# medivhna/TF_Face_Toolbox

Hardware: AMD Instinct MI355X
Metric: images/sec (whole node), SphereFaceNet-20 112x112 bs512 (higher is better)
Workload: dtype f32; 1 GPU; SphereFaceNet-20 + A-softmax training step, 112x112x3, global batch 512, 10575 classes, Momentum, fp32; global_batch=512, per_gpu_batch=512, parallelism=dp1

## Files before the change

### include/fte.h

```cpp
#ifndef FTE_H_
#define FTE_H_

#include <stddef.h>
#include <stdint.h>

#ifdef __cplusplus
extern "C" {
#endif

#define FTE_OK 0
#define FTE_EINVAL (-1)
#define FTE_EWORKSPACE (-2)

const char* fte_version(void);

#define FTE_MFMA_F32 0
#define FTE_MFMA_BF16 1
int fte_set_mfma_dtype(int dtype);
int fte_get_mfma_dtype(void);

#define FTE_CONV_DIRECT 0
#define FTE_CONV_WINOGRAD 1
#define FTE_CONV_AUTO 2
int fte_set_conv_algo(int algo);
int fte_get_conv_algo(void);
int fte_conv3x3_algo(int n, int h, int wd, int cin, int cout, int stride, int op);
size_t fte_wino_pack_bytes(int n, int h, int wd, int c);

int fte_prof_enable(int on);
int fte_prof_count(void);
int fte_prof_get(int i, int* sig, double* flops, float* ms);
int fte_prof_get_shape(int i, int* mnk, double* bytes);
int fte_prof_get_name(int i, char* buf, int buflen);


int fte_conv3x3_fwd(const float* x, const float* w, const float* bias, const float* alpha,
                    const float* res, float* z, float* y,
                    int n, int h, int wd, int cin, int cout, int stride,
                    void* ws, size_t ws_bytes, void* stream);
size_t fte_conv3x3_fwd_ws_bytes(int n, int h, int wd, int cin, int cout, int stride);
int fte_conv3x3_fwd_keep(const float* x, const float* w, const float* bias, const float* alpha,
                         const float* res, float* z, float* y,
                         int n, int h, int wd, int cin, int cout, int stride, float* vpack,
                         void* ws, size_t ws_bytes, void* stream);

int fte_conv3x3_dgrad(const float* dz, const float* w, const float* addin,
                      const float* zprev, const float* alpha_prev,
                      float* raw, float* dzprev, float* dalpha_prev, float* dbias_prev,
                      int n, int h, int wd, int cin, int cout, int stride,
                      void* ws, size_t ws_bytes, void* stream);
size_t fte_conv3x3_dgrad_ws_bytes(int n, int h, int wd, int cin, int cout, int stride);

int fte_conv3x3_wgrad(const float* x, const float* dz, float* dw,
                      int n, int h, int wd, int cin, int cout, int stride,
                      void* ws, size_t ws_bytes, void* stream);
size_t fte_conv3x3_wgrad_ws_bytes(int n, int h, int wd, int cin, int cout, int stride);
int fte_conv3x3_wgrad_kept(const float* x, const float* dz, float* dw,
                           int n, int h, int wd, int cin, int cout, int stride, const float* vpack,
                           void* ws, size_t ws_bytes, void* stream);


int fte_conv2d_fwd(const float* x, const float* w, const float* bias, const float* alpha, const float* res,
                   float* z, float* y, int n, int h, int wd, int cin, int cout, int ksize, int stride,
                   void* ws, size_t ws_bytes, void* stream);
size_t fte_conv2d_fwd_ws_bytes(int n, int h, int wd, int cin, int cout, int ksize, int stride);
int fte_conv2d_dgrad(const float* dz, const float* w, const float* addin, const float* zprev,
                     const float* alpha_prev, float* raw, float* dzprev, float* dalpha_prev, float* dbias_prev,
                     int n, int h, int wd, int cin, int cout, int ksize, int stride,
                     void* ws, size_t ws_bytes, void* stream);
size_t fte_conv2d_dgrad_ws_bytes(int n, int h, int wd, int cin, int cout, int ksize, int stride);
int fte_conv2d_wgrad(const float* x, const float* dz, float* dw, int n, int h, int wd, int cin, int cout,
                     int ksize, int stride, void* ws, size_t ws_bytes, void* stream);
size_t fte_conv2d_wgrad_ws_bytes(int n, int h, int wd, int cin, int cout, int ksize, int stride);

int fte_im2col_first(const float* x, float* cols, int n, int h, int wd, int cin, int ksize, int stride,
                     int kpad, void* stream);
int fte_im2col_first_s16(const float* x, uint16_t* cols16, int n, int h, int wd, int cin, int ksize, int stride, int kpad, void* stream);

int fte_preprocess_u8(const uint8_t* slots, float* out, int n, long slot_stride, int channels, int in_h, int in_w, int crop_h, int crop_w,
                      void* stream);
int fte_preprocess_u8_aug(const uint8_t* slots, float* out, int n, long slot_stride, int channels, int in_h, int in_w, int crop_h,
                          int crop_w, void* stream);
size_t fte_preprocess_u8_geo_ws_bytes(int n, int channels, int crop_h, int crop_w);
int fte_preprocess_u8_geo(const uint8_t* slots, float* out, int n, long slot_stride, int channels, int in_h, int in_w, int crop_h,
                          int crop_w, const float* affine_table, void* ws, size_t ws_bytes, void* stream);

size_t fte_bn_ws_bytes(int c);
int fte_bn_train_fwd(const float* z, const float* gamma, const float* beta, const float* res, float* y,
                     float* mean, float* rstd, float* scale, float* shift, float* moving_mean, float* moving_var,
                     long rows, int c, float eps, float decay, int relu, void* ws, size_t ws_bytes, void* stream);
int fte_bn_infer_fwd(const float* z, const float* gamma, const float* beta, const float* moving_mean,
                     const float* moving_var, const float* res, float* y, float* scale, float* shift,
                     long rows, int c, float eps, int relu, void* stream);
int fte_bn_train_bwd(const float* dy, const float* ymask, const float* z, const float* gamma, const float* mean,
                     const float* rstd, float* dz, float* dgamma, float* dbeta, long rows, int c,
                     void* ws, size_t ws_bytes, void* stream);
int fte_bn_train_bwd_zmask(const float* dy, const float* z, const float* gamma, const float* mean, const float* rstd,
                           const float* scale, const float* shift, float* dz, float* dgamma, float* dbeta, long rows, int c,
                           void* ws, size_t ws_bytes, void* stream);
int fte_bn_train_bwd_res(const float* dy, const float* y, const float* z, const float* gamma, const float* mean, const float* rstd,
                         float* g_out, float* dz, float* dgamma, float* dbeta, long rows, int c,
                         void* ws, size_t ws_bytes, void* stream);
int fte_bn_train_stats(const float* z, const float* gamma, const float* beta, float* mean, float* rstd, float* scale, float* shift,
                       float* moving_mean, float* moving_var, long rows, int c, float eps, float decay,
                       void* ws, size_t ws_bytes, void* stream);
int fte_bn_infer_coef(const float* gamma, const float* beta, const float* moving_mean, const float* moving_var,
                      float* scale, float* shift, int c, float eps, void* stream);
size_t fte_bn_prelu_ws_bytes(int c);
int fte_bn_prelu_apply(const float* z, const float* scale, const float* shift, const float* alpha, float* y, long rows, int c,
                       void* stream);
int fte_bn_prelu_infer_fwd(const float* z, const float* gamma, const float* beta, const float* moving_mean, const float* moving_var,
                           const float* alpha, float* y, float* scale, float* shift, long rows, int c, float eps, void* stream);
int fte_bn_prelu_train_bwd(const float* dy, const float* z, const float* gamma, const float* mean, const float* rstd,
                           const float* scale, const float* shift, const float* alpha, float* dz, float* dgamma, float* dbeta,
                           float* dalpha, long rows, int c, void* ws, size_t ws_bytes, void* stream);
int fte_relu_bwd(const float* dy, const float* y, float* g, long n, void* stream);

int fte_maxpool3x3s2_fwd(const float* x, float* y, uint8_t* idx, int n, int h, int wd, int c, void* stream);
int fte_maxpool3x3s2_bwd(const float* dy, const uint8_t* idx, float* dx, int n, int h, int wd, int c, void* stream);
int fte_gap_fwd(const float* x, float* y, int n, int hw, int c, void* stream);
int fte_gap_bwd(const float* dy, float* dx, int n, int hw, int c, void* stream);
int fte_dropout_fwd(const float* x, float* mask, float* y, long n, float keep_prob, uint64_t seed, void* stream);
int fte_dropout_bwd(const float* dy, const float* mask, float* dx, long n, float keep_prob, void* stream);

int fte_gconv3x3_fwd(const float* x, const float* w, float* y, int n, int h, int wd, int c, int groups,
                     int stride, void* stream);
int fte_gconv3x3_pack_bf16(const float* w, uint16_t* wpk_fwd, uint16_t* wpk_dgrad, int c, int groups, void* stream);
int fte_gconv3x3_bf16(const float* x, const uint16_t* wpk, float* y, int n, int h, int wd, int c, int stride, int dgrad, void* stream);
size_t fte_gconv3x3_wgrad_bf16_ws_bytes(int n, int h, int wd, int c, int groups, int stride);
int fte_gconv3x3_wgrad_bf16(const float* x, const float* dz, float* dw, int n, int h, int wd, int c, int groups, int stride,
                            void* ws, size_t ws_bytes, void* stream);
int fte_gconv3x3_dgrad(const float* dz, const float* w, float* dx, int n, int h, int wd, int c, int groups,
                       int stride, void* stream);
int fte_gconv3x3_wgrad(const float* x, const float* dz, float* dw, int n, int h, int wd, int c, int groups,
                       int stride, void* ws, size_t ws_bytes, void* stream);
size_t fte_gconv3x3_wgrad_ws_bytes(int n, int h, int wd, int c, int groups, int stride);

int fte_bcast_add(float* dx, const float* v, int n, int hw, int c, float scale, void* stream);
int fte_dense_small(const float* a, const float* w, const float* bias, const float* mask, float* out, int m, int n, int k,
                    int trans_w, int act, void* stream);
int fte_act_fwd(const float* x, float* y, long n, int kind, void* stream);
int fte_act_bwd(const float* dy, const float* y, float* dx, long n, int kind, void* stream);
int fte_channel_scale_fwd(const float* x, const float* gate, float* y, int n, int hw, int c, void* stream);
int fte_channel_scale_bwd(const float* dy, const float* x, const float* gate, float* dx, float* dgate,
                          int n, int hw, int c, int pre_sigmoid, void* stream);

int fte_to_bf16(const float* x, uint16_t* y16, long n, void* stream);
int fte_pack_weights_bf16(const float* w, uint16_t* w16, uint16_t* w16t, int ksize, int cin, int cout, void* stream);
int fte_pack_weights_bf16_table(const float* params, uint16_t* dst, const int32_t* table, int nconv, long total, int transposed, void* stream);
int fte_conv2d_fwd16(const uint16_t* x16, const uint16_t* w16t, const float* bias, const float* alpha, const float* res,
                     float* z, float* y, uint16_t* y16, int n, int h, int wd, int cin, int cout, int ksize, int stride,
                     void* ws, size_t ws_bytes, void* stream);
int fte_conv2d_dgrad16(const uint16_t* dz16, const uint16_t* w16, const float* addin, const float* zprev,
                       const float* alpha_prev, float* raw, float* dzprev, uint16_t* dzprev16, float* dalpha_prev,
                       float* dbias_prev, int n, int h, int wd, int cin, int cout, int ksize, int stride,
                       void* ws, size_t ws_bytes, void* stream);
int fte_conv2d_wgrad16(const uint16_t* x16, const uint16_t* dz16, float* dw, int n, int h, int wd, int cin, int cout,
                       int ksize, int stride, void* ws, size_t ws_bytes, void* stream);

int fte_conv2d_fwd_s16(const uint16_t* x16, const uint16_t* w16t, const float* bias, const float* alpha, const uint16_t* res16,
                       uint16_t* z16, uint16_t* y16, float* z32, float* y32, int n, int h, int wd, int cin, int cout,
                       int ksize, int stride, void* ws, size_t ws_bytes, void* stream);
int fte_conv2d_dgrad_s16(const uint16_t* dz16, const uint16_t* w16, const uint16_t* addin16, const uint16_t* zprev16,
                         const float* alpha_prev, uint16_t* raw16, uint16_t* dzprev16, float* dalpha_prev, float* dbias_prev,
                         int n, int h, int wd, int cin, int cout, int ksize, int stride, void* ws, size_t ws_bytes, void* stream);
int fte_conv3x3_first_fwd_s16(const float* x, const float* w, const float* bias, const float* alpha, uint16_t* z16, uint16_t* y16,
                              int n, int h, int wd, int cin, int cout, int stride, void* stream);
int fte_conv3x3_first_wgrad_s16(const float* x, const uint16_t* dz16, float* dw, int n, int h, int wd, int cin, int cout, int stride,
                                void* ws, size_t ws_bytes, void* stream);

#define FTE_S16_Z 1
#define FTE_S16_A 2
int fte_bn_train_fwd_s16(const void* z, const float* gamma, const float* beta, const void* res, void* y,
                         float* mean, float* rstd, float* scale, float* shift, float* moving_mean, float* moving_var,
                         long rows, int c, float eps, float decay, int relu, int flags, void* ws, size_t ws_bytes, void* stream);
int fte_bn_infer_fwd_s16(const void* z, const float* gamma, const float* beta, const float* moving_mean, const float* moving_var,
                         const void* res, void* y, float* scale, float* shift, long rows, int c, float eps, int relu, int flags, void* stream);
int fte_bn_train_bwd_s16(const void* dy, const void* y, const void* z, const float* gamma, const float* mean, const float* rstd,
                         const float* scale, const float* shift, void* g_out, void* dz, float* dgamma, float* dbeta,
                         long rows, int c, int flags, void* ws, size_t ws_bytes, void* stream);
int fte_relu_bwd_s16(const uint16_t* dy16, const uint16_t* y16, uint16_t* g16, long n, void* stream);
int fte_maxpool3x3s2_fwd_s16(const uint16_t* x16, uint16_t* y16, uint8_t* idx, int n, int h, int wd, int c, void* stream);
int fte_maxpool3x3s2_bwd_s16(const uint16_t* dy16, const uint8_t* idx, uint16_t* dx16, int n, int h, int wd, int c, void* stream);
int fte_gap_fwd_s16(const uint16_t* x16, float* y, int n, int hw, int c, void* stream);
int fte_gap_bwd_s16(const float* dy, uint16_t* dx16, int n, int hw, int c, void* stream);
int fte_gconv3x3_bf16_s16(const uint16_t* x16, const uint16_t* wpk, uint16_t* y16, int n, int h, int wd, int c, int stride, int dgrad, void* stream);
int fte_gconv3x3_wgrad_bf16_s16(const uint16_t* x16, const uint16_t* dz16, float* dw, int n, int h, int wd, int c, int groups, int stride,
                                void* ws, size_t ws_bytes, void* stream);
size_t fte_conv2d_bn_fwd_ws_bytes(int n, int h, int wd, int cin, int cout, int ksize, int stride);
int fte_conv2d_bn_fwd_folds(int n, int h, int wd, int cin, int cout, int ksize, int stride, int s16);
int fte_conv2d_bn_fwd(const void* x, const void* w, void* z, const float* gamma, const float* beta, float* mean, float* rstd,
                      float* scale, float* shift, float* moving_mean, float* moving_var, float eps, float decay,
                      const float* in_scale, const float* in_shift, void* y_side,
                      int n, int h, int wd, int cin, int cout, int ksize, int stride, int s16, void* ws, size_t ws_bytes, void* stream);
size_t fte_conv2d_dgrad_bn_ws_bytes(int n, int h, int wd, int cin, int cout, int ksize, int stride);
int fte_conv2d_dgrad_bn(const void* dz, const void* w, const void* addin, const void* zbn, const void* ybn,
                        const float* gamma, const float* mean, const float* rstd, const float* bn_scale, const float* bn_shift,
// ... 175 lines not shown
```

### tf_face_toolbox_amd/_lib.py

```python
import ctypes
import os
from ctypes import c_char_p, c_float, c_int, c_long, c_size_t, c_uint64, c_void_p

_HERE = os.path.dirname(os.path.abspath(__file__))
LIB_PATH = os.environ.get('FTE_LIB') or os.path.join(_HERE, 'libfte.so')


class FteError(RuntimeError):
    pass


_P = c_void_p
_SIGS = {
    'fte_version': (c_char_p, []),
    'fte_prof_enable': (c_int, [c_int]),
    'fte_prof_count': (c_int, []),
    'fte_prof_get': (c_int, [c_int, _P, _P, _P]),
    'fte_prof_get_shape': (c_int, [c_int, _P, _P]),
    'fte_prof_get_name': (c_int, [c_int, _P, c_int]),
    'fte_conv3x3_fwd': (c_int, [_P] * 7 + [c_int] * 6 + [_P, c_size_t, _P]),
    'fte_conv3x3_fwd_ws_bytes': (c_size_t, [c_int] * 6),
    'fte_conv3x3_dgrad': (c_int, [_P] * 9 + [c_int] * 6 + [_P, c_size_t, _P]),
    'fte_conv3x3_dgrad_ws_bytes': (c_size_t, [c_int] * 6),
    'fte_conv3x3_wgrad': (c_int, [_P] * 3 + [c_int] * 6 + [_P, c_size_t, _P]),
    'fte_conv3x3_wgrad_ws_bytes': (c_size_t, [c_int] * 6),
    'fte_conv2d_fwd': (c_int, [_P] * 7 + [c_int] * 7 + [_P, c_size_t, _P]),
    'fte_conv2d_fwd_ws_bytes': (c_size_t, [c_int] * 7),
    'fte_conv2d_dgrad': (c_int, [_P] * 9 + [c_int] * 7 + [_P, c_size_t, _P]),
    'fte_conv2d_dgrad_ws_bytes': (c_size_t, [c_int] * 7),
    'fte_conv2d_wgrad': (c_int, [_P] * 3 + [c_int] * 7 + [_P, c_size_t, _P]),
    'fte_conv2d_wgrad_ws_bytes': (c_size_t, [c_int] * 7),
    'fte_im2col_first': (c_int, [_P] * 2 + [c_int] * 7 + [_P]),
    'fte_im2col_first_s16': (c_int, [_P] * 2 + [c_int] * 7 + [_P]),
    'fte_preprocess_u8': (c_int, [_P] * 2 + [c_int, c_long] + [c_int] * 5 + [_P]),
    'fte_preprocess_u8_aug': (c_int, [_P] * 2 + [c_int, c_long] + [c_int] * 5 + [_P]),
    'fte_preprocess_u8_geo_ws_bytes': (c_size_t, [c_int] * 4),
    'fte_preprocess_u8_geo': (c_int, [_P] * 2 + [c_int, c_long] + [c_int] * 5 + [_P, _P, c_size_t, _P]),
    'fte_bn_ws_bytes': (c_size_t, [c_int]),
    'fte_bn_train_fwd': (c_int, [_P] * 11 + [c_long, c_int, c_float, c_float, c_int, _P, c_size_t, _P]),
    'fte_bn_infer_fwd': (c_int, [_P] * 9 + [c_long, c_int, c_float, c_int, _P]),
    'fte_bn_train_bwd': (c_int, [_P] * 9 + [c_long, c_int, _P, c_size_t, _P]),
    'fte_bn_train_bwd_zmask': (c_int, [_P] * 10 + [c_long, c_int, _P, c_size_t, _P]),
    'fte_bn_train_bwd_res': (c_int, [_P] * 10 + [c_long, c_int, _P, c_size_t, _P]),
    'fte_bn_train_stats': (c_int, [_P] * 9 + [c_long, c_int, c_float, c_float, _P, c_size_t, _P]),
    'fte_bn_infer_coef': (c_int, [_P] * 6 + [c_int, c_float, _P]),
    'fte_bn_prelu_ws_bytes': (c_size_t, [c_int]),
    'fte_bn_prelu_apply': (c_int, [_P] * 5 + [c_long, c_int, _P]),
    'fte_bn_prelu_infer_fwd': (c_int, [_P] * 9 + [c_long, c_int, c_float, _P]),
    'fte_bn_prelu_train_bwd': (c_int, [_P] * 12 + [c_long, c_int, _P, c_size_t, _P]),
    'fte_relu_bwd': (c_int, [_P] * 3 + [c_long, _P]),
    'fte_maxpool3x3s2_fwd': (c_int, [_P] * 3 + [c_int] * 4 + [_P]),
    'fte_maxpool3x3s2_bwd': (c_int, [_P] * 3 + [c_int] * 4 + [_P]),
    'fte_gap_fwd': (c_int, [_P] * 2 + [c_int] * 3 + [_P]),
    'fte_gap_bwd': (c_int, [_P] * 2 + [c_int] * 3 + [_P]),
    'fte_dropout_fwd': (c_int, [_P] * 3 + [c_long, c_float, c_uint64, _P]),
    'fte_dropout_bwd': (c_int, [_P] * 3 + [c_long, c_float, _P]),
    'fte_gconv3x3_fwd': (c_int, [_P] * 3 + [c_int] * 6 + [_P]),
    'fte_gconv3x3_pack_bf16': (c_int, [_P] * 3 + [c_int, c_int, _P]),
    'fte_gconv3x3_bf16': (c_int, [_P] * 3 + [c_int] * 6 + [_P]),
    'fte_gconv3x3_wgrad_bf16_ws_bytes': (c_size_t, [c_int] * 6),
    'fte_gconv3x3_wgrad_bf16': (c_int, [_P] * 3 + [c_int] * 6 + [_P, c_size_t, _P]),
    'fte_gconv3x3_dgrad': (c_int, [_P] * 3 + [c_int] * 6 + [_P]),
    'fte_gconv3x3_wgrad': (c_int, [_P] * 3 + [c_int] * 6 + [_P, c_size_t, _P]),
    'fte_gconv3x3_wgrad_ws_bytes': (c_size_t, [c_int] * 6),
    'fte_bcast_add': (c_int, [_P] * 2 + [c_int] * 3 + [c_float, _P]),
    'fte_act_fwd': (c_int, [_P] * 2 + [c_long, c_int, _P]),
    'fte_act_bwd': (c_int, [_P] * 3 + [c_long, c_int, _P]),
    'fte_channel_scale_fwd': (c_int, [_P] * 3 + [c_int] * 3 + [_P]),
    'fte_channel_scale_bwd': (c_int, [_P] * 5 + [c_int] * 4 + [_P]),
    'fte_to_bf16': (c_int, [_P, _P, c_long, _P]),
    'fte_pack_weights_bf16': (c_int, [_P, _P, _P, c_int, c_int, c_int, _P]),
    'fte_pack_weights_bf16_table': (c_int, [_P, _P, _P, c_int, c_long, c_int, _P]),
    'fte_conv2d_fwd16': (c_int, [_P] * 8 + [c_int] * 7 + [_P, c_size_t, _P]),
    'fte_conv2d_dgrad16': (c_int, [_P] * 10 + [c_int] * 7 + [_P, c_size_t, _P]),
    'fte_conv2d_wgrad16': (c_int, [_P] * 3 + [c_int] * 7 + [_P, c_size_t, _P]),
    'fte_conv2d_fwd_s16': (c_int, [_P] * 9 + [c_int] * 7 + [_P, c_size_t, _P]),
    'fte_conv2d_dgrad_s16': (c_int, [_P] * 9 + [c_int] * 7 + [_P, c_size_t, _P]),
    'fte_conv3x3_first_fwd_s16': (c_int, [_P] * 6 + [c_int] * 6 + [_P]),
    'fte_conv3x3_first_wgrad_s16': (c_int, [_P] * 3 + [c_int] * 6 + [_P, c_size_t, _P]),
    'fte_bn_train_fwd_s16': (c_int, [_P] * 11 + [c_long, c_int, c_float, c_float, c_int, c_int, _P, c_size_t, _P]),
    'fte_bn_infer_fwd_s16': (c_int, [_P] * 9 + [c_long, c_int, c_float, c_int, c_int, _P]),
    'fte_bn_train_bwd_s16': (c_int, [_P] * 12 + [c_long, c_int, c_int, _P, c_size_t, _P]),
    'fte_relu_bwd_s16': (c_int, [_P] * 3 + [c_long, _P]),
    'fte_maxpool3x3s2_fwd_s16': (c_int, [_P] * 3 + [c_int] * 4 + [_P]),
    'fte_maxpool3x3s2_bwd_s16': (c_int, [_P] * 3 + [c_int] * 4 + [_P]),
    'fte_gap_fwd_s16': (c_int, [_P] * 2 + [c_int] * 3 + [_P]),
    'fte_gap_bwd_s16': (c_int, [_P] * 2 + [c_int] * 3 + [_P]),
    'fte_gconv3x3_bf16_s16': (c_int, [_P] * 3 + [c_int] * 6 + [_P]),
    'fte_gconv3x3_wgrad_bf16_s16': (c_int, [_P] * 3 + [c_int] * 6 + [_P, c_size_t, _P]),
    'fte_channel_scale_fwd_s16': (c_int, [_P] * 3 + [c_int] * 3 + [_P]),
    'fte_channel_scale_bwd_s16': (c_int, [_P] * 4 + [c_int] * 4 + [_P]),
    'fte_channel_scale_bwd_apply_s16': (c_int, [_P] * 4 + [c_int] * 3 + [c_float, _P]),
    'fte_dense_small': (c_int, [_P] * 5 + [c_int] * 5 + [_P]),
    'fte_se_squeeze': (c_int, [_P] * 7 + [c_int] * 4 + [_P]),
    'fte_se_apply_fwd': (c_int, [_P] * 6 + [c_int] * 4 + [_P]),
    'fte_se_bwd_gate': (c_int, [_P] * 12 + [c_int] * 4 + [_P]),
    'fte_se_bn_bwd_coef': (c_int, [_P] * 11 + [c_int] * 3 + [_P]),
    'fte_se_bn_bwd_apply': (c_int, [_P] * 6 + [c_int] * 4 + [_P]),
    'fte_dwconv3x3_fwd_s16': (c_int, [_P] * 3 + [c_int] * 5 + [_P]),
    'fte_dwconv3x3_dgrad_s16': (c_int, [_P] * 3 + [c_int] * 5 + [_P]),
    'fte_dwconv3x3_wgrad_s16': (c_int, [_P] * 3 + [c_int] * 5 + [_P, c_size_t, _P]),
    'fte_channel_gather_s16': (c_int, [_P] * 4 + [c_long] + [c_int] * 3 + [_P]),
    'fte_channel_gather_affine_s16': (c_int, [_P] * 4 + [c_int, _P, _P, c_int, c_long, c_int, c_int, _P, _P, c_int, _P, _P, c_int, _P]),
    'fte_bn_train_stats_s16': (c_int, [_P] * 9 + [c_long, c_int, c_float, c_float, c_int, _P, c_size_t, _P]),
    'fte_conv2d_bn_fwd_ws_bytes': (c_size_t, [c_int] * 7),
    'fte_conv2d_bn_fwd': (c_int, [_P] * 11 + [c_float, c_float] + [_P] * 3 + [c_int] * 8 + [_P, c_size_t, _P]),
    'fte_conv2d_bn_fwd_folds': (c_int, [c_int] * 8),
    'fte_conv2d_dgrad_bn_ws_bytes': (c_size_t, [c_int] * 7),
    'fte_conv2d_dgrad_bn': (c_int, [_P] * 14 + [c_int] * 8 + [_P, c_size_t, _P]),
    'fte_bn_apply': (c_int, [_P] * 5 + [c_long, c_int, c_int, c_int, _P]),
    'fte_bn_bwd_apply': (c_int, [_P] * 4 + [c_long, c_int, c_int, _P]),
    'fte_gconv3x3_bn_ws_bytes': (c_size_t, [c_int] * 5),
    'fte_gconv3x3_bn_fwd_bf16_s16': (c_int, [_P] * 11 + [c_float, c_float] + [_P] * 3 + [c_int] * 5 + [_P, c_size_t, _P]),
    'fte_gconv3x3_dgrad_bn_bf16_s16': (c_int, [_P] * 12 + [c_int] * 5 + [_P, c_size_t, _P]),
    'fte_set_mfma_dtype': (c_int, [c_int]),
    'fte_get_mfma_dtype': (c_int, []),
    'fte_set_conv_algo': (c_int, [c_int]),
    'fte_conv3x3_algo': (c_int, [c_int] * 7),
    'fte_wino_pack_bytes': (c_size_t, [c_int] * 4),
    'fte_conv3x3_fwd_keep': (c_int, [_P] * 7 + [c_int] * 6 + [_P, _P, c_size_t, _P]),
    'fte_conv3x3_wgrad_kept': (c_int, [_P] * 3 + [c_int] * 6 + [_P, _P, c_size_t, _P]),
    'fte_get_conv_algo': (c_int, []),
    'fte_l2_normalize_rows': (c_int, [_P] * 3 + [c_int] * 2 + [_P]),
    'fte_pair_scores': (c_int, [_P] * 4 + [c_int] * 3 + [_P]),
    'fte_topk_search_ws_bytes': (c_size_t, [c_int] * 4),
    'fte_topk_search': (c_int, [_P] * 2 + [c_int] * 7 + [_P] * 3 + [c_size_t, _P]),
    'fte_topk_merge': (c_int, [_P] * 2 + [c_int] * 3 + [_P] * 3),
    'fte_score_histograms': (c_int, [_P, _P, c_int, _P, _P] + [c_int] * 4 + [_P] * 3),
    'fte_template_pool': (c_int, [_P, _P, c_int, c_int, _P, c_int, _P, c_int, _P, c_int, _P, _P]),
    'fte_set_pair_scores': (c_int, [_P, c_int, c_int, _P, c_int, _P, c_int, _P, c_int, _P, _P, c_int, _P, c_int, _P, _P]),
    'fte_megaface_pair_scores': (c_int, [_P, c_int, _P, c_int, c_int, _P, _P, c_int, _P, _P]),
    'fte_megaface_scan_ws_bytes': (c_size_t, [c_int] * 2),
    'fte_megaface_scan': (c_int, [_P, c_int, _P, c_int, c_int, _P, _P, c_int, c_int, _P, _P, _P, c_size_t, _P]),
    'fte_pfc_sample_ws_bytes': (c_size_t, [c_int]),
    'fte_pfc_sample': (c_int, [_P] + [c_int] * 5 + [_P] * 4 + [c_size_t, _P]),
    'fte_pfc_gather_cols': (c_int, [_P] * 3 + [c_int] * 5 + [_P]),
    'fte_pfc_scatter_cols': (c_int, [_P] * 3 + [c_int] * 5 + [_P]),
    'fte_pfc_momentum_update_cols': (c_int, [_P] * 4 + [c_int] * 5 + [c_float] * 4 + [_P]),
    'fte_pfc_adam_update_cols': (c_int, [_P] * 5 + [c_int] * 5 + [c_float] * 6 + [c_int, _P]),
    'fte_knn_links_threshold': (c_int, [_P] * 2 + [c_int] * 2 + [c_float, c_int, _P, _P]),
    'fte_knn_links_rank_order': (c_int, [_P] * 2 + [c_int] * 2 + [c_float] * 2 + [_P, _P]),
    'fte_components': (c_int, [_P] * 2 + [c_int] * 2 + [_P] * 3),
    'fte_dwconv3x3_fwd': (c_int, [_P] * 3 + [c_int] * 5 + [_P]),
    'fte_dwconv3x3_dgrad': (c_int, [_P] * 3 + [c_int] * 5 + [_P]),
    'fte_dwconv3x3_wgrad': (c_int, [_P] * 3 + [c_int] * 5 + [_P, c_size_t, _P]),
    'fte_dwconv3x3_wgrad_ws_bytes': (c_size_t, [c_int] * 5),
    'fte_channel_gather': (c_int, [_P] * 4 + [c_long] + [c_int] * 3 + [_P]),
    'fte_channel_gather_affine': (c_int, [_P] * 4 + [c_int, _P, _P, c_int, c_long, c_int, c_int, _P, _P, c_int, _P, _P, c_int, _P]),
    'fte_conv3x3_first_fwd': (c_int, [_P] * 6 + [c_int] * 6 + [_P]),
    'fte_conv3x3_first_wgrad': (c_int, [_P] * 3 + [c_int] * 6 + [_P, c_size_t, _P]),
    'fte_conv3x3_first_wgrad_ws_bytes': (c_size_t, [c_int] * 6),
    'fte_gemm_nn': (c_int, [_P] * 4 + [c_int] * 3 + [_P, c_size_t, _P]),
    'fte_gemm_nn_act': (c_int, [_P] * 4 + [c_int] * 4 + [_P, c_size_t, _P]),
    'fte_gemm_nt': (c_int, [_P] * 4 + [c_int] + [_P] * 3 + [c_int] * 3 + [_P, c_size_t, _P]),
    'fte_gemm_tn': (c_int, [_P] * 3 + [c_int] * 3 + [_P, c_size_t, _P]),
    'fte_gemm_ws_bytes': (c_size_t, [c_int] * 3),
    'fte_softmax_ce_fwd_bwd': (c_int, [_P] * 4 + [c_int] * 3 + [c_float, _P]),
    'fte_focal_loss_fwd_bwd': (c_int, [_P] * 4 + [c_int] * 3 + [c_float] * 3 + [_P]),
    'fte_asoftmax_fwd_bwd': (c_int, [_P] * 4 + [c_float] + [_P] * 4 + [c_int] * 3 + [c_float, _P]),
    'fte_asoftmax_colcoef': (c_int, [_P] * 4 + [c_int] * 3 + [_P]),
    'fte_margin_softmax_fwd_bwd': (c_int, [_P] * 4 + [c_float] * 3 + [_P] * 4 + [c_int] * 3 + [c_float, _P]),
    'fte_margin_softmax_rows_fwd_bwd': (c_int, [_P] * 4 + [c_float] + [_P] * 6 + [c_int] * 3 + [c_float, _P]),
    'fte_subcenter_margin_softmax_fwd_bwd': (c_int, [_P] * 4 + [c_int] + [c_float] * 3 + [_P] * 4 + [c_int] * 3 + [c_float, _P]),
    'fte_subcenter_colcoef': (c_int, [_P] * 4 + [c_int] * 4 + [_P]),
    'fte_subcenter_assign': (c_int, [_P] * 3 + [c_int] + [_P] * 2 + [c_int] * 3 + [_P]),
    'fte_adaface_margins': (c_int, [_P, c_int] + [c_float] * 3 + [c_int] + [_P] * 4),
    'fte_row_norms': (c_int, [_P] * 2 + [c_int] * 3 + [_P]),
    'fte_col_norms': (c_int, [_P] * 2 + [c_int] * 3 + [_P]),
    'fte_add_scaled_rows_cols': (c_int, [_P] * 4 + [c_int] * 3 + [_P]),
    'fte_flip_width': (c_int, [_P] * 2 + [c_int] * 4 + [_P]),
    'fte_axpby': (c_int, [c_float, _P, c_float, _P, _P, c_long, _P]),
    'fte_center_loss_fwd_bwd_update': (c_int, [_P] * 5 + [c_int] * 3 + [c_float] * 2 + [_P, c_size_t, _P]),
    'fte_center_scatter_update': (c_int, [_P] * 3 + [c_int] * 3 + [c_float, _P]),
    'fte_batch_hard_triplet_fwd_bwd': (c_int, [_P] * 2 + [c_float, c_int, c_float] + [_P] * 2 + [c_int] * 2 + [_P, c_size_t, _P]),
    'fte_reduce_rows': (c_int, [_P] * 3 + [c_int, c_long, c_long, c_int, c_float, _P]),
    'fte_sumsq': (c_int, [_P, c_long, c_float, _P, _P, c_size_t, _P]),
    'fte_sum': (c_int, [_P, c_long, c_float, _P, _P, c_size_t, _P]),
    'fte_momentum_update': (c_int, [_P] * 3 + [c_long] + [c_float] * 4 + [_P]),
    'fte_adam_update': (c_int, [_P] * 4 + [c_long] + [c_float] * 6 + [c_int, _P]),
}

_lib = None


def exported_names():
    return sorted(_SIGS)


_CODES = {-1: 'FTE_EINVAL -- a null pointer, a shape the kernel family does not tile (channel multiples, stride, '
              'ksize) or a tensor of 2 GiB or more (buffer-load range)',
          -2: 'FTE_EWORKSPACE -- workspace missing or smaller than the matching *_ws_bytes() query'}

MFMA_DTYPES = {'f32': 0, 'fp32': 0, 'float32': 0, 'bf16': 1, 'bfloat16': 1, 'bf16s': 1}
_storage16 = False


def load():
    global _lib
    if _lib is not None:
        return _lib
    if not os.path.exists(LIB_PATH):
        raise FteError('libfte.so not found at %s -- build it with `python -c "import __graft_entry__ as g; g.build()"` '
                       '(or tf_face_toolbox_amd/csrc/build.sh). There is no CPU fallback.' % LIB_PATH)
    lib = ctypes.CDLL(LIB_PATH)
    for name, (res, args) in _SIGS.items():
        fn = getattr(lib, name)
        fn.restype = res
        fn.argtypes = args
    _lib = lib
    env = os.environ.get('FTE_MFMA_DTYPE')
    if env:
        if env not in MFMA_DTYPES:
            raise FteError('FTE_MFMA_DTYPE=%r: expected f32, bf16 or bf16s' % env)
        lib.fte_set_mfma_dtype(MFMA_DTYPES[env])
        global _storage16
        _storage16 = env == 'bf16s'
    return lib


def _ptr(t):
    if t is None:
        return None
    if isinstance(t, int):
        return t
    return t.data_ptr()


_FN = {}
_Tensor = None


def call(name, *args):
    global _Tensor
    fn = _FN.get(name)
    if fn is None:
        fn = _FN[name] = getattr(load(), name)
        if _Tensor is None:
            import torch
            _Tensor = torch.Tensor
    T = _Tensor
    r = fn(*[a.data_ptr() if type(a) is T else (a.data_ptr() if hasattr(a, 'data_ptr') else a) for a in args])
    if r != 0:
        what = _CODES.get(r, 'hipError_t %d (see hip_runtime_api.h)' % r if r > 0 else 'unknown')
        raise FteError('%s failed with code %d: %s' % (name, r, what))


def query(name, *args):
    return getattr(load(), name)(*args)


def version():
    return load().fte_version().decode()


def source_stamp():
    v = version()
    return v.split('src:', 1)[1] if 'src:' in v else ''


def set_mfma_dtype(name):
    if name not in MFMA_DTYPES:
        raise ValueError('unknown MFMA dtype %r (f32 | bf16 | bf16s)' % (name,))
    global _storage16
    call('fte_set_mfma_dtype', MFMA_DTYPES[name])
    _storage16 = name == 'bf16s'


def get_mfma_dtype():
    return 'bf16' if query('fte_get_mfma_dtype') == 1 else 'f32'


def bf16_storage():
    return _storage16 and query('fte_get_mfma_dtype') == 1
# ... 32 lines not shown
```

### tf_face_toolbox_amd/csrc/api.hip

```cpp
#include <hip/hip_runtime.h>
#include <stdio.h>
#include <stdlib.h>
#include <string.h>

#include <initializer_list>

#include "../../include/fte.h"
#include "igemm.h"
#include "wgrad16.h"
#include "pw16.h"
#include "kernels.h"
#include "layers.h"
#include "wino.h"
#include "search.h"
#include "partial_fc.h"
#include "cluster.h"
#include "iresnet.h"

namespace {

struct Pads { int out, before; };
inline Pads same_pads(int in, int k, int stride) {
    const int out = (in + stride - 1) / stride;
    int total = (out - 1) * stride + k - in;
// ... 196 lines not shown
    hipError_t e = hipSuccess;
    if (rp.tail_mode == 3) {
        int bm, bn;
        igemm_tile_dims(rp.main_tile, &bm, &bn);
        const long T = rp.main_mtiles * (p.N / bn), iters = T * (p.K / 32);
        p.m_base = 0; p.prow0 = (int)prow0;
        p.sk_workers = rp.sk_workers; p.sk_base = (int)(iters / rp.sk_workers); p.sk_rem = (int)(iters % rp.sk_workers);
        p.SKW = pw; p.SKF = reinterpret_cast<unsigned*>(pw + (size_t)rp.sk_workers * bm * bn);
        return igemm_launch(p, al, bl, epi, rp.main_tile, 1, st);
    }
    if (rp.main_rows > 0) {
        p.m_base = 0; p.M = (int)rp.main_rows; p.prow0 = (int)prow0;
        e = igemm_launch(p, al, bl, epi, rp.main_tile, 1, st);
        if (e != hipSuccess) return e;
    }
    if (rp.tail_mode == 0) return e;
    p.m_base = (int)rp.main_rows; p.M = M; p.prow0 = (int)(prow0 + rp.main_mtiles);
    if (rp.tail_mode == 1) return igemm_launch(p, al, bl, epi, rp.tail_tile, 1, st);
    p.PW = pw; p.kchunk = rp.tail_kchunk;
    e = igemm_launch(p, al, bl, epi, rp.tail_tile, rp.tail_splits, st);
    if (e != hipSuccess) return e;
    return igemm_fixup(p, epi, rp.tail_tile, rp.tail_splits, st);
}

template <class F>
size_t both_modes(F f) {
    size_t a, b, c;
    { PlanMode m(false); a = f(); }
    { PlanMode m(true); b = f(); }
    {
        Plan16 guard;
        PlanS16 storage(true);
        c = f();
    }
    return a > b ? (a > c ? a : c) : (b > c ? b : c);
}

inline int wino_min_c() {
    static const int v = getenv("FTE_WINO_MIN_C") ? atoi(getenv("FTE_WINO_MIN_C")) : 128;
    return v;
}
inline bool wino_fwd_small_tiles() {
    static const int tpb = getenv("FTE_WINO_FWD_TPB") ? atoi(getenv("FTE_WINO_FWD_TPB")) : 256;
    return tpb != 512;
}
inline bool wino_shape_ok(int n, int h, int wd, int cin, int cout, int ksize, int stride) {
    if (ksize != 3 || stride != 1 || cin % 64 || cout % 64 || n <= 0 || h < 2 || wd < 2) return false;
    const size_t lim = (size_t)1 << 31;
    return (size_t)n * h * wd * cin * 4 < lim && (size_t)n * h * wd * cout * 4 < lim;
}
inline bool wino_sized(int n, int h, int wd, int cin, int cout, int ksize, int stride, int op) {
    const int algo = wino_get_algo();
    if (algo == 0 || !wino_shape_ok(n, h, wd, cin, cout, ksize, stride)) return false;
    if (op == 2 && !wino_wgrad_splits(cin, cout)) return false;
    if (algo == 1) return true;
    static const int ops = getenv("FTE_WINO_OPS") ? atoi(getenv("FTE_WINO_OPS")) : 7;
    static const int ops64 = getenv("FTE_WINO_OPS64") ? atoi(getenv("FTE_WINO_OPS64")) : 5;
    const int cmin = cin < cout ? cin : cout;
    if (cmin < wino_min_c()) return cmin >= 64 && (ops64 & (1 << op)) != 0;
    return (ops & (1 << op)) != 0;
}
inline bool wino_wanted(int n, int h, int wd, int cin, int cout, int ksize, int stride, int op) {
    return !plan_bf16() && !g_plan_bn && wino_sized(n, h, wd, cin, cout, ksize, stride, op);
}
inline bool aligned16(std::initializer_list<const void*> ptrs) {
    uintptr_t v = 0;
    for (const void* q : ptrs) v |= (uintptr_t)q;
    return (v & 15) == 0;
}
struct WinoWs { size_t v_off, u_off, slab_off, total; };
inline WinoWs wino_ws(int n, int h, int wd, int cin, int cout, int op, size_t head) {
    const WinoGeom g = wino_geom(n, h, wd);
    WinoWs w;
    w.v_off = align_up(head);
    if (op == 0) {
        w.u_off = w.v_off + align_up(wino_pack_floats(g.M, cin) * 4);
        w.slab_off = w.total = w.u_off + align_up((size_t)16 * cin * cout * 4);
    } else if (op == 1) {
        w.u_off = w.v_off + align_up(wino_pack_floats(g.M, cout) * 4);
        w.slab_off = w.total = w.u_off + align_up((size_t)16 * cin * cout * 4);
    } else {
        w.u_off = w.v_off + align_up(wino_pack_floats(g.M, cin) * 4);
        w.slab_off = w.u_off;
        w.total = w.slab_off + align_up((size_t)wino_wgrad_splits(cin, cout) * 16 * cin * cout * 4);
    }
    return w;
}
}

extern "C" {

#ifndef FTE_SRC_SHA
#define FTE_SRC_SHA "unstamped"
#endif
const char* fte_version(void) { return "fte 0.2 gfx950 fp32-mfma src:" FTE_SRC_SHA; }

int fte_to_bf16(const float* x, uint16_t* y, long n, void* stream) {
    if (!x || !y || n <= 0 || n % 4) return FTE_EINVAL;
    return rc(k_to_bf16(x, y, n, (hipStream_t)stream));
}
int fte_pack_weights_bf16(const float* w, uint16_t* w16, uint16_t* w16t, int ksize, int cin, int cout, void* stream) {
    if (!w || (!w16 && !w16t) || ksize <= 0 || cin <= 0 || cout <= 0) return FTE_EINVAL;
    return rc(k_pack_weights_bf16(w, w16, w16t, ksize * ksize, cin, cout, (hipStream_t)stream));
}

int fte_pack_weights_bf16_table(const float* params, uint16_t* dst, const int32_t* table, int nconv, long total, int transposed, void* stream) {
    if (!params || !dst || !table || nconv <= 0 || nconv > 64 || total <= 0 || total % 4) return FTE_EINVAL;
    return rc(k_pack_weights_table(params, dst, table, nconv, total, transposed, (hipStream_t)stream));
}

int fte_set_mfma_dtype(int dtype) {
    if (dtype != FTE_MFMA_F32 && dtype != FTE_MFMA_BF16) return FTE_EINVAL;
    igemm_set_bf16(dtype == FTE_MFMA_BF16);
    return FTE_OK;
}
int fte_get_mfma_dtype(void) { return igemm_get_bf16() ? FTE_MFMA_BF16 : FTE_MFMA_F32; }

int fte_set_conv_algo(int algo) {
    if (algo < FTE_CONV_DIRECT || algo > FTE_CONV_AUTO) return FTE_EINVAL;
    wino_set_algo(algo);
    return FTE_OK;
}
int fte_get_conv_algo(void) { return wino_get_algo(); }

int fte_prof_enable(int on) { igemm_prof_enable(on != 0, on == 1); return FTE_OK; }
int fte_prof_count(void) { return igemm_prof_count(); }
int fte_prof_get_shape(int i, int* mnk, double* bytes) {
    if (!mnk || !bytes) return FTE_EINVAL;
    return rc(igemm_prof_get_shape(i, mnk, bytes));
}
int fte_prof_get_name(int i, char* buf, int buflen) {
    if (!buf || buflen <= 0) return FTE_EINVAL;
    return rc(igemm_prof_get_name(i, buf, buflen));
}
int fte_prof_get(int i, int* sig, double* flops, float* ms) {
    if (!sig || !flops || !ms) return FTE_EINVAL;
    return rc(igemm_prof_get(i, sig, flops, ms));
}

size_t fte_conv2d_fwd_ws_bytes(int n, int h, int wd, int cin, int cout, int ksize, int stride) {
    if (n <= 0 || cin <= 0 || cin % 32 || cout <= 0 || cout % 64) return 0;
    const Pads ph = same_pads(h, ksize, stride), pw = same_pads(wd, ksize, stride);
    size_t need = both_modes([&] { return plan_rows((long)n * ph.out * pw.out, cout, (long)ksize * ksize * cin, true, false, EPI_FWD).pw_bytes; });
    if (wino_sized(n, h, wd, cin, cout, ksize, stride, 0)) {
        const size_t wn = wino_ws(n, h, wd, cin, cout, 0, 0).total;
        if (wn > need) need = wn;
    }
    return need;
}

static int conv2d_fwd_impl(const void* x, const void* w, bool src16, const float* bias, const float* alpha, const float* res,
                           float* z, float* y, uint16_t* y16, int n, int h, int wd, int cin, int cout, int ksize, int stride,
                           void* ws, size_t ws_bytes, void* stream, const uint16_t* res16 = nullptr, uint16_t* z16 = nullptr,
                           float* stat_part = nullptr, int* stat_rows = nullptr, float* vpack = nullptr) {
    if (!x || !w || (!y && !(src16 && y16)) || n <= 0 || cin % 32 || cout % 64 || (stride != 1 && stride != 2) || (ksize != 1 && ksize != 3))
        return FTE_EINVAL;
    const Pads ph = same_pads(h, ksize, stride), pw = same_pads(wd, ksize, stride);
    IgemmParams p;
    zero_params(&p);
    p.M = n * ph.out * pw.out; p.N = cout; p.K = ksize * ksize * cin; p.kchunk = p.K;
    p.a_OH = ph.out; p.a_OW = pw.out; p.a_IH = h; p.a_IW = wd; p.a_stride = stride;
    p.a_ld = cin; p.a_KC = cin; p.a_NT = ksize * ksize;
    for (int r = 0; r < ksize; ++r)
        for (int s = 0; s < ksize; ++s) { p.a_dh[r * ksize + s] = r - ph.before; p.a_dw[r * ksize + s] = s - pw.before; }
    p.A = (const float*)x;
    p.B = (const float*)w;
    p.c_ld = cout;
    p.Y = y; p.Z = z; p.R = res; p.bias = bias; p.alpha = alpha; p.Y16 = y16;
    p.R16 = res16; p.Z16 = z16;
    int bl = BL_KN;
    if (src16) {
        p.src16 = 1; p.b_ld = cin; bl = BL_NK;
        for (int t = 0; t < ksize * ksize; ++t) p.b_tapoff[t] = t * cout * cin;
    } else {
        p.b_ld = cout;
    }
    if (!set_bytes(&p, (size_t)n * h * wd * cin, (size_t)ksize * ksize * cin * cout, src16 ? 2 : 4)) return FTE_EINVAL;
    if (!src16 && !stat_part && y && wino_wanted(n, h, wd, cin, cout, ksize, stride, 0)) {
        WinoWs wl = wino_ws(n, h, wd, cin, cout, 0, 0);
        if (vpack) { wl.u_off = 0; wl.total = align_up((size_t)16 * cin * cout * 4); }
        if (ws && ws_bytes >= wl.total) {
            if (!aligned16({x, w, bias, alpha, res, z, y, ws, vpack})) return FTE_EINVAL;
            float* V = vpack ? vpack : (float*)((char*)ws + wl.v_off);
            float* U = (float*)((char*)ws + wl.u_off);
            hipError_t e = wino_transform_filter((const float*)w, U, cin, cout, 0, (hipStream_t)stream);
            if (e != hipSuccess) return (int)e;
            e = wino_transform_tiles((const float*)x, V, n, h, wd, cin, 0, (hipStream_t)stream, wino_fwd_small_tiles());
            if (e != hipSuccess) return (int)e;
            WinoMMParams q;
            memset(&q, 0, sizeof(q));
            q.V = V; q.U = U; q.K = cin; q.N = cout; q.g = wino_geom(n, h, wd);
            q.Y = y; q.Z = z; q.R = res; q.bias = bias; q.alpha = alpha;
            return rc(wino_mm(q, EPI_FWD, (hipStream_t)stream));
        }
    }
    if (vpack) return FTE_EWORKSPACE;
    RowPlan rp = plan_rows(p.M, p.N, p.K, ws != nullptr, false, EPI_FWD);
    if (rp.tail_mode >= 2 && ws_bytes < rp.pw_bytes) rp = plan_rows(p.M, p.N, p.K, false);
    if (stat_part) {
        if (rp.tail_mode == 2) return FTE_EINVAL;
        p.SP = stat_part;
        *stat_rows = (int)(rp.main_mtiles + rp.tail_mtiles);
    }
    return rc(launch_rows(p, rp, AL_MK, bl, EPI_FWD, 0, (float*)ws, (hipStream_t)stream));
}
int fte_conv2d_fwd(const float* x, const float* w, const float* bias, const float* alpha, const float* res,
                   float* z, float* y, int n, int h, int wd, int cin, int cout, int ksize, int stride,
                   void* ws, size_t ws_bytes, void* stream) {
    return conv2d_fwd_impl(x, w, false, bias, alpha, res, z, y, nullptr, n, h, wd, cin, cout, ksize, stride, ws, ws_bytes, stream);
}
int fte_conv2d_fwd16(const uint16_t* x16, const uint16_t* w16t, const float* bias, const float* alpha, const float* res,
                     float* z, float* y, uint16_t* y16, int n, int h, int wd, int cin, int cout, int ksize, int stride,
                     void* ws, size_t ws_bytes, void* stream) {
    Plan16 guard;
    return conv2d_fwd_impl(x16, w16t, true, bias, alpha, res, z, y, y16, n, h, wd, cin, cout, ksize, stride, ws, ws_bytes, stream);
}

int fte_conv2d_fwd_s16(const uint16_t* x16, const uint16_t* w16t, const float* bias, const float* alpha, const uint16_t* res16,
                       uint16_t* z16, uint16_t* y16, float* z32, float* y32, int n, int h, int wd, int cin, int cout, int ksize, int stride,
                       void* ws, size_t ws_bytes, void* stream) {
    if (!y16 || (res16 && ((uintptr_t)res16 & 15))) return FTE_EINVAL;
    Plan16 guard;
    PlanS16 storage(!z32 && !y32);
    return conv2d_fwd_impl(x16, w16t, true, bias, alpha, nullptr, z32, y32, y16, n, h, wd, cin, cout, ksize, stride, ws, ws_bytes, stream, res16, z16);
}

size_t fte_conv3x3_fwd_ws_bytes(int n, int h, int wd, int cin, int cout, int stride) {
    return fte_conv2d_fwd_ws_bytes(n, h, wd, cin, cout, 3, stride);
}
int fte_conv3x3_fwd(const float* x, const float* w, const float* bias, const float* alpha, const float* res,
                    float* z, float* y, int n, int h, int wd, int cin, int cout, int stride,
                    void* ws, size_t ws_bytes, void* stream) {
    return fte_conv2d_fwd(x, w, bias, alpha, res, z, y, n, h, wd, cin, cout, 3, stride, ws, ws_bytes, stream);
}
int fte_conv3x3_fwd_keep(const float* x, const float* w, const float* bias, const float* alpha, const float* res,
                         float* z, float* y, int n, int h, int wd, int cin, int cout, int stride, float* vpack,
                         void* ws, size_t ws_bytes, void* stream) {
    if (vpack && ((uintptr_t)vpack & 15)) return FTE_EINVAL;
    return conv2d_fwd_impl(x, w, false, bias, alpha, res, z, y, nullptr, n, h, wd, cin, cout, 3, stride, ws, ws_bytes, stream,
                           nullptr, nullptr, nullptr, nullptr, vpack);
}
int fte_conv3x3_algo(int n, int h, int wd, int cin, int cout, int stride, int op) {
    if (op < 0 || op > 2) return FTE_EINVAL;
    return (!igemm_get_bf16() && wino_sized(n, h, wd, cin, cout, 3, stride, op)) ? FTE_CONV_WINOGRAD : FTE_CONV_DIRECT;
}
size_t fte_wino_pack_bytes(int n, int h, int wd, int c) {
    if (n <= 0 || h < 2 || wd < 2 || c <= 0 || c % 64) return 0;
    return wino_pack_floats(wino_geom(n, h, wd).M, c) * sizeof(float);
}

namespace {
struct DgradClass { int ph, pw, hq, wq, ntap, dh[9], dw[9], wt[9]; RowPlan rp; long mtiles; };
int dgrad_classes(int n, int h, int wd, int cin, int cout, int ksize, int stride, DgradClass* cls) {
    const Pads ph = same_pads(h, ksize, stride), pw = same_pads(wd, ksize, stride);
    int nc = 0;
    for (int a = 0; a < stride; ++a)
        for (int b = 0; b < stride; ++b) {
            DgradClass& c = cls[nc];
            c.ph = a; c.pw = b;
            c.hq = (h - a + stride - 1) / stride;
            c.wq = (wd - b + stride - 1) / stride;
            c.ntap = 0;
            if (c.hq <= 0 || c.wq <= 0) continue;
            for (int r = 0; r < ksize; ++r) {
                if ((a + ph.before - r) % stride) continue;
                for (int s = 0; s < ksize; ++s) {
                    if ((b + pw.before - s) % stride) continue;
                    c.dh[c.ntap] = (a + ph.before - r) / stride;
                    c.dw[c.ntap] = (b + pw.before - s) / stride;
                    c.wt[c.ntap] = r * ksize + s;
                    ++c.ntap;
                }
            }
            const long M = (long)n * c.hq * c.wq;
            static const bool cls_big = getenv("FTE_DGRAD_CLS_BIG") && atoi(getenv("FTE_DGRAD_CLS_BIG")) == 1;
            c.rp = plan_rows(M, cin, (long)c.ntap * cout, true, stride != 1 && !cls_big, EPI_DGRAD);
            c.mtiles = c.rp.main_mtiles + c.rp.tail_mtiles;
            ++nc;
        }
    return nc;
}
static bool dgrad_merged16() {
    static const bool on = getenv("FTE_DGRAD_MERGED16") && atoi(getenv("FTE_DGRAD_MERGED16")) == 1;
    return on && plan_bf16();
}
bool dgrad_mergeable(const DgradClass* cls, int nc, int n, int cin) {
    static const char* mode = getenv("FTE_DGRAD_CLASSES");
    if (nc != 4 || (mode && mode[0] == 's')) return false;
    for (int i = 0; i < nc; ++i)
        if (cls[i].hq != cls[0].hq || cls[i].wq != cls[0].wq || cls[i].ntap < 1) return false;
    if ((mode && mode[0] == 'm') || dgrad_merged16()) return true;
    const long tiles = (((long)n * cls[0].hq * cls[0].wq + 63) / 64) * (cin / 64);
    return tiles < SLOTS;
}
static int dgrad_merged_tile(int cin) {
    if (!dgrad_merged16()) return TILE_64x64;
    return cin % 128 == 0 ? TILE_128x128 : TILE_128x64;
}
long dgrad_merged_rows(const DgradClass* cls, int nc, int n, int cin) {
    if (!dgrad_mergeable(cls, nc, n, cin)) return 0;
    int bm, bn;
    igemm_tile_dims(dgrad_merged_tile(cin), &bm, &bn);
    return (long)nc * (((long)n * cls[0].hq * cls[0].wq + bm - 1) / bm);
}
int dgrad_merged_plan(const DgradClass* cls, int nc, int n, int cin, int* order) {
    for (int i = 0; i < nc; ++i) order[i] = i;
    for (int i = 0; i < nc; ++i)
        for (int j = i + 1; j < nc; ++j)
            if (cls[order[j]].ntap > cls[order[i]].ntap) { const int t = order[i]; order[i] = order[j]; order[j] = t; }
    (void)n;
    return dgrad_merged_tile(cin);
}
}

size_t fte_conv2d_dgrad_ws_bytes(int n, int h, int wd, int cin, int cout, int ksize, int stride) {
    if (n <= 0 || cin <= 0 || cin % 64 || cout % 32) return 0;
    size_t need = both_modes([&] {
        DgradClass cls[4];
        const int nc = dgrad_classes(n, h, wd, cin, cout, ksize, stride, cls);
        long rows = 0;
        size_t pw = 0;
        for (int i = 0; i < nc; ++i) { rows += cls[i].mtiles; if (cls[i].rp.pw_bytes > pw) pw = cls[i].rp.pw_bytes; }
        const long merged_rows = dgrad_merged_rows(cls, nc, n, cin);
        if (merged_rows > rows) rows = merged_rows;
        return 2 * align_up((size_t)rows * cin * sizeof(float)) + SCRATCH_BYTES + pw;
    });
    if (wino_sized(n, h, wd, cin, cout, ksize, stride, 1)) {
        const WinoGeom g = wino_geom(n, h, wd);
        const size_t wn = wino_ws(n, h, wd, cin, cout, 1, 2 * align_up((size_t)g.MB * cin * sizeof(float)) + SCRATCH_BYTES).total;
        if (wn > need) need = wn;
    }
    return need;
}

struct DgradBn {
    const void* zbn; const void* ybn;
    const float* gamma; const float* mean; const float* rstd; const float* scale; const float* shift;
    float* dgamma; float* dbeta; float* coef;
};
static int conv2d_dgrad_impl(const void* dz, const void* w, bool src16, const float* addin, const float* zprev,
                             const float* alpha_prev, float* raw, float* dzprev, uint16_t* dzprev16, float* dalpha_prev, float* dbias_prev,
                             int n, int h, int wd, int cin, int cout, int ksize, int stride, void* ws, size_t ws_bytes, void* stream,
                             const uint16_t* addin16 = nullptr, const uint16_t* zprev16 = nullptr, uint16_t* raw16 = nullptr,
                             const DgradBn* bn = nullptr) {
    const float* zx = nullptr;
    const uint16_t* zx16 = nullptr;
    if (bn) {
        const void* msk = (!bn->scale && bn->ybn) ? bn->ybn : bn->zbn;
        const void* zb = (!bn->scale && bn->ybn) ? bn->zbn : nullptr;
        if (src16) { zprev16 = (const uint16_t*)msk; zx16 = (const uint16_t*)zb; }
        else { zprev = (const float*)msk; zx = (const float*)zb; }
        alpha_prev = bn->gamma;
        dalpha_prev = bn->dgamma; dbias_prev = bn->dbeta;
    }
    if (zprev16 && !zprev) zprev = reinterpret_cast<const float*>(zprev16);
    const bool z16only = zprev16 != nullptr;
    if (!dz || !w || (!dzprev && !(src16 && dzprev16)) || n <= 0 || cout % 32 || cin % 64 || (stride != 1 && stride != 2) || (ksize != 1 && ksize != 3)) return FTE_EINVAL;
    if (zprev && !alpha_prev) return FTE_EINVAL;
    const Pads pho = same_pads(h, ksize, stride), pwo = same_pads(wd, ksize, stride);
    if (!src16 && !bn && dzprev && !dzprev16 && !addin16 && !zprev16 && !raw16 && wino_wanted(n, h, wd, cin, cout, ksize, stride, 1)) {
        const WinoGeom g = wino_geom(n, h, wd);
        const size_t half_w = align_up((size_t)g.MB * cin * sizeof(float));
        const WinoWs wl = wino_ws(n, h, wd, cin, cout, 1, 2 * half_w + SCRATCH_BYTES);
        if (ws && ws_bytes >= wl.total) {
            if (!aligned16({dz, w, addin, zprev, alpha_prev, raw, dzprev, ws})) return FTE_EINVAL;
            const bool part = zprev && (dalpha_prev || dbias_prev);
            float* V = (float*)((char*)ws + wl.v_off);
            float* U = (float*)((char*)ws + wl.u_off);
            hipError_t e = wino_transform_filter((const float*)w, U, cin, cout, 1, (hipStream_t)stream);
            if (e != hipSuccess) return (int)e;
            e = wino_transform_tiles((const float*)dz, V, n, h, wd, cout, 0, (hipStream_t)stream);
            if (e != hipSuccess) return (int)e;
            WinoMMParams q;
            memset(&q, 0, sizeof(q));
            q.V = V; q.U = U; q.K = cout; q.N = cin; q.g = g;
            q.ADD = addin; q.RAW = raw; q.Zin = zprev; q.alpha = alpha_prev; q.amod = cin; q.DZ = dzprev;
            q.PA = part ? (float*)ws : nullptr; q.PB = part ? (float*)((char*)ws + half_w) : nullptr;
            e = wino_mm(q, EPI_DGRAD, (hipStream_t)stream);
            if (e != hipSuccess) return (int)e;
            if (part) {
                float* scratch = (float*)((char*)ws + 2 * half_w);
                if (dalpha_prev && dbias_prev) return rc(k_reduce_rows2(q.PA, dalpha_prev, q.PB, dbias_prev, nullptr, 1, g.MB, cin, 1, 1.f, scratch, (hipStream_t)stream));
                if (dalpha_prev) return rc(k_reduce_rows(q.PA, dalpha_prev, nullptr, 1, g.MB, cin, 1, 1.f, scratch, (hipStream_t)stream));
                return rc(k_reduce_rows(q.PB, dbias_prev, nullptr, 1, g.MB, cin, 1, 1.f, scratch, (hipStream_t)stream));
            }
            return FTE_OK;
        }
    }
    DgradClass cls[4];
    const int nc = dgrad_classes(n, h, wd, cin, cout, ksize, stride, cls);
    const bool merged = dgrad_mergeable(cls, nc, n, cin);
    long rows = 0;
    for (int i = 0; i < nc; ++i) rows += cls[i].mtiles;
// ... 17 lines not shown
        p.M = n * c0.hq * c0.wq; p.N = cin; p.a_KC = cout;
        p.A = (const float*)dz; p.a_OH = c0.hq; p.a_OW = c0.wq; p.a_IH = pho.out; p.a_IW = pwo.out; p.a_stride = 1; p.a_ld = cout;
        p.ncls = nc;
        int t = 0;
        for (int k = 0; k < nc; ++k) {
            const DgradClass& c = cls[order[k]];
            p.cls_tap0[k] = t; p.cls_ph[k] = c.ph; p.cls_pw[k] = c.pw;
            for (int j = 0; j < c.ntap; ++j, ++t) { p.a_dh[t] = c.dh[j]; p.a_dw[t] = c.dw[j]; p.b_tapoff[t] = c.wt[j] * cin * cout; }
        }
        p.cls_tap0[nc] = t;
        p.a_NT = t; p.K = t * cout; p.kchunk = p.K;
        p.B = (const float*)w; p.b_ld = cout;
        p.c_OH = c0.hq; p.c_OW = c0.wq; p.c_FH = h; p.c_FW = wd; p.c_step = stride; p.c_ld = cin;
        p.ADD = addin; p.RAW = raw; p.Zin = z16only ? nullptr : zprev; p.alpha = alpha_prev; p.amod = cin; p.DZ = dzprev;
        p.ADD16 = addin16; p.Zin16 = zprev16; p.RAW16 = raw16;
        p.PA = PA; p.PB = PB; p.prow0 = 0;
        if (bn) { p.bn_mu = bn->mean; p.bn_rs = bn->rstd; p.bn_sc = bn->scale; p.bn_sh = bn->shift; p.Zx = zx; p.Zx16 = zx16; }
        p.src16 = src16 ? 1 : 0; p.DZ16 = dzprev16;
        if (!set_bytes(&p, (size_t)n * pho.out * pwo.out * cout, (size_t)ksize * ksize * cin * cout, src16 ? 2 : 4)) return FTE_EINVAL;
        hipError_t e = igemm_launch(p, AL_MK, BL_NK, EPI_DGRAD, tile, 1, (hipStream_t)stream);
        if (e != hipSuccess) return (int)e;
    } else {
    long prow = 0;
    for (int i = 0; i < nc; ++i) {
        const DgradClass& c = cls[i];
        IgemmParams p;
        zero_params(&p);
        p.M = n * c.hq * c.wq; p.N = cin; p.K = c.ntap * cout; p.kchunk = p.K;
        p.A = (const float*)dz; p.a_OH = c.hq; p.a_OW = c.wq; p.a_IH = pho.out; p.a_IW = pwo.out; p.a_stride = 1;
        p.a_ld = cout; p.a_KC = cout; p.a_NT = c.ntap;
        for (int t = 0; t < c.ntap; ++t) {
            p.a_dh[t] = c.dh[t]; p.a_dw[t] = c.dw[t];
            p.b_tapoff[t] = c.wt[t] * cin * cout;
        }
        p.B = (const float*)w; p.b_ld = cout;
        p.src16 = src16 ? 1 : 0; p.DZ16 = dzprev16;
        if (stride == 1) { p.c_OH = 0; }
        else { p.c_OH = c.hq; p.c_OW = c.wq; p.c_FH = h; p.c_FW = wd; p.c_step = stride; p.c_ph = c.ph; p.c_pw = c.pw; }
        p.c_ld = cin;
        p.ADD = addin; p.RAW = raw; p.Zin = z16only ? nullptr : zprev; p.alpha = alpha_prev; p.amod = cin; p.DZ = dzprev;
        p.ADD16 = addin16; p.Zin16 = zprev16; p.RAW16 = raw16;
        p.PA = PA; p.PB = PB;
        if (bn) { p.bn_mu = bn->mean; p.bn_rs = bn->rstd; p.bn_sc = bn->scale; p.bn_sh = bn->shift; p.Zx = zx; p.Zx16 = zx16; }
        if (!set_bytes(&p, (size_t)n * pho.out * pwo.out * cout, (size_t)ksize * ksize * cin * cout, src16 ? 2 : 4)) return FTE_EINVAL;
        hipError_t e = launch_rows(p, c.rp, AL_MK, BL_NK, EPI_DGRAD, prow, pwbuf, (hipStream_t)stream);
        if (e != hipSuccess) return (int)e;
        prow += c.mtiles;
    }
    }
    if (bn)
        return rc(l_bn_bwd_finalize(PB, PA, cin, (int)rows, (long)n * h * wd, cin, bn->gamma, bn->mean, bn->rstd, bn->dgamma, bn->dbeta,
                                    bn->coef, (hipStream_t)stream));
    if (want_part) {
        if (dalpha_prev && dbias_prev) {
            hipError_t e = k_reduce_rows2(PA, dalpha_prev, PB, dbias_prev, nullptr, 1, rows, cin, 1, 1.f, scratch, (hipStream_t)stream);
            if (e != hipSuccess) return (int)e;
        } else {
            if (dalpha_prev) { hipError_t e = k_reduce_rows(PA, dalpha_prev, nullptr, 1, rows, cin, 1, 1.f, scratch, (hipStream_t)stream); if (e != hipSuccess) return (int)e; }
            if (dbias_prev) { hipError_t e = k_reduce_rows(PB, dbias_prev, nullptr, 1, rows, cin, 1, 1.f, scratch, (hipStream_t)stream); if (e != hipSuccess) return (int)e; }
        }
    }
    return FTE_OK;
}

int fte_conv2d_dgrad(const float* dz, const float* w, const float* addin, const float* zprev,
                     const float* alpha_prev, float* raw, float* dzprev, float* dalpha_prev, float* dbias_prev,
                     int n, int h, int wd, int cin, int cout, int ksize, int stride, void* ws, size_t ws_bytes, void* stream) {
    return conv2d_dgrad_impl(dz, w, false, addin, zprev, alpha_prev, raw, dzprev, nullptr, dalpha_prev, dbias_prev,
                             n, h, wd, cin, cout, ksize, stride, ws, ws_bytes, stream);
}
int fte_conv2d_dgrad16(const uint16_t* dz16, const uint16_t* w16, const float* addin, const float* zprev,
                       const float* alpha_prev, float* raw, float* dzprev, uint16_t* dzprev16, float* dalpha_prev, float* dbias_prev,
                       int n, int h, int wd, int cin, int cout, int ksize, int stride, void* ws, size_t ws_bytes, void* stream) {
    Plan16 guard;
    return conv2d_dgrad_impl(dz16, w16, true, addin, zprev, alpha_prev, raw, dzprev, dzprev16, dalpha_prev, dbias_prev,
                             n, h, wd, cin, cout, ksize, stride, ws, ws_bytes, stream);
}

int fte_conv2d_dgrad_s16(const uint16_t* dz16, const uint16_t* w16, const uint16_t* addin16, const uint16_t* zprev16,
                         const float* alpha_prev, uint16_t* raw16, uint16_t* dzprev16, float* dalpha_prev, float* dbias_prev,
                         int n, int h, int wd, int cin, int cout, int ksize, int stride, void* ws, size_t ws_bytes, void* stream) {
    if (!dzprev16) return FTE_EINVAL;
    Plan16 guard;
    PlanS16 storage(true);
    return conv2d_dgrad_impl(dz16, w16, true, nullptr, nullptr, alpha_prev, nullptr, nullptr, dzprev16, dalpha_prev, dbias_prev,
                             n, h, wd, cin, cout, ksize, stride, ws, ws_bytes, stream, addin16, zprev16, raw16);
}

size_t fte_conv3x3_dgrad_ws_bytes(int n, int h, int wd, int cin, int cout, int stride) {
    return fte_conv2d_dgrad_ws_bytes(n, h, wd, cin, cout, 3, stride);
}
int fte_conv3x3_dgrad(const float* dz, const float* w, const float* addin, const float* zprev,
                      const float* alpha_prev, float* raw, float* dzprev, float* dalpha_prev, float* dbias_prev,
                      int n, int h, int wd, int cin, int cout, int stride, void* ws, size_t ws_bytes, void* stream) {
    return fte_conv2d_dgrad(dz, w, addin, zprev, alpha_prev, raw, dzprev, dalpha_prev, dbias_prev,
                            n, h, wd, cin, cout, 3, stride, ws, ws_bytes, stream);
}

namespace {
inline bool wgrad_split_major() {
    static const bool on = !getenv("FTE_WGRAD_SPLIT_MAJOR") || atoi(getenv("FTE_WGRAD_SPLIT_MAJOR")) != 0;
    return on;
}
void wgrad_plan(int n, int h, int wd, int cin, int cout, int ksize, int stride, int* tile, int* splits, int* kchunk, int* K) {
    const Pads ph = same_pads(h, ksize, stride), pw = same_pads(wd, ksize, stride);
    *K = n * ph.out * pw.out;
    const long M = (long)ksize * ksize * cin;
    static const int wg_tile = getenv("FTE_WGRAD_TILE") ? atoi(getenv("FTE_WGRAD_TILE")) : -1;
    const int narrow = (M % 192 == 0 && M % 128 != 0) ? TILE_192x64 : TILE_128x64;
    const bool tiny = ksize == 1 && M * cout <= 256L * 256;
    *tile = wg_tile >= 0 ? wg_tile : (tiny ? TILE_64x64 : (cout % 128 == 0) ? TILE_128x128 : narrow);
    plan_splits(tiles_of(*tile, M, cout), *K, splits, kchunk, false);
    if (wg_tile < 0 && *tile != TILE_64x64 && *splits > 1 && *kchunk < 1024) {
        *tile = TILE_64x64;
        plan_splits(tiles_of(*tile, M, cout), *K, splits, kchunk, false);
    }
}
}

size_t fte_conv2d_wgrad_ws_bytes(int n, int h, int wd, int cin, int cout, int ksize, int stride) {
    if (n <= 0 || cin <= 0 || cin % 4 || cout <= 0 || cout % 64) return 0;
    int tile, splits, kchunk, K;
    wgrad_plan(n, h, wd, cin, cout, ksize, stride, &tile, &splits, &kchunk, &K);
    size_t need = splits > 1 ? (size_t)splits * ksize * ksize * cin * cout * sizeof(float) : 0;
    if (ksize == 3 && stride == 1) {
        Wgrad16Params g;
        int cfg = 0;
        if (wgrad16_plan(n, h, wd, cin, cout, &g, &cfg) && g.S > 1) {
            const size_t gneed = (size_t)g.S * g.slab * sizeof(float);
            if (gneed > need) need = gneed;
        }
    }
    if (ksize == 1 && stride == 1) {
        Wgrad16Params g;
        int cfg = 0;
        if (wgrad16p_plan(n, h, wd, cin, cout, &g, &cfg) && g.S > 1) {
            const size_t gneed = (size_t)g.S * g.slab * sizeof(float);
            if (gneed > need) need = gneed;
        }
    }
    if (wino_sized(n, h, wd, cin, cout, ksize, stride, 2)) {
        const size_t wn = wino_ws(n, h, wd, cin, cout, 2, 0).total;
        if (wn > need) need = wn;
    }
    return need + SCRATCH_BYTES;
}
size_t fte_conv3x3_wgrad_ws_bytes(int n, int h, int wd, int cin, int cout, int stride) {
    return fte_conv2d_wgrad_ws_bytes(n, h, wd, cin, cout, 3, stride);
}

static int conv2d_wgrad_impl(const void* x, const void* dz, bool src16, float* dw, int n, int h, int wd, int cin, int cout, int ksize, int stride,
                             void* ws, size_t ws_bytes, void* stream, const float* vpack = nullptr) {
    if (src16 && (cin % 8 || cout % 8)) return FTE_EINVAL;
    if (!x || !dz || !dw || n <= 0 || cin % 4 || cout % 64 || (stride != 1 && stride != 2) || (ksize != 1 && ksize != 3)) return FTE_EINVAL;
    const Pads ph = same_pads(h, ksize, stride), pw = same_pads(wd, ksize, stride);
    {
        const size_t lim = (size_t)1 << 31, es = src16 ? 2 : 4;
        if ((size_t)n * h * wd * cin * es >= lim || (size_t)n * ph.out * pw.out * cout * es >= lim) return FTE_EINVAL;
    }
    int tile, splits, kchunk, K;
    wgrad_plan(n, h, wd, cin, cout, ksize, stride, &tile, &splits, &kchunk, &K);
    if (!src16 && wino_wanted(n, h, wd, cin, cout, ksize, stride, 2)) {
        WinoWs wl = wino_ws(n, h, wd, cin, cout, 2, 0);
        if (vpack) {
            const size_t vsz = wl.u_off - wl.v_off;
            wl.u_off -= vsz; wl.slab_off -= vsz; wl.total -= vsz;
        }
        if (ws && ws_bytes >= wl.total) {
            if (!aligned16({x, dz, dw, ws, vpack})) return FTE_EINVAL;
            const float* V = vpack ? vpack : (float*)((char*)ws + wl.v_off);
            float* slabs = (float*)((char*)ws + wl.slab_off);
            hipError_t e = hipSuccess;
            if (!vpack) e = wino_transform_tiles((const float*)x, (float*)((char*)ws + wl.v_off), n, h, wd, cin, 0, (hipStream_t)stream);
            if (e != hipSuccess) return (int)e;
            return rc(wino_wgrad(V, (const float*)dz, slabs, dw, wino_geom(n, h, wd), cin, cout, (hipStream_t)stream));
        }
    }
    if (vpack) return FTE_EWORKSPACE;
    if (src16 && ksize == 3 && stride == 1) {
        Wgrad16Params g;
        int cfg = 0;
        if (wgrad16_plan(n, h, wd, cin, cout, &g, &cfg)) {
            const size_t gneed = g.S > 1 ? (size_t)g.S * g.slab * sizeof(float) : 0;
            const size_t xb = (size_t)n * h * wd * cin * 2, db = (size_t)n * h * wd * cout * 2;
            if ((!gneed || (ws && ws_bytes >= gneed)) && xb < (1ull << 31) && db < (1ull << 31)) {
                g.x = (const unsigned short*)x; g.dz = (const unsigned short*)dz;
                g.out = g.S > 1 ? (float*)ws : dw;
                g.x_bytes = (unsigned)xb; g.dz_bytes = (unsigned)db;
                for (int r = 0; r < 3; ++r)
                    for (int s2 = 0; s2 < 3; ++s2) { g.dh[r * 3 + s2] = r - 1; g.dw[r * 3 + s2] = s2 - 1; }
                const int sig[5] = {AL_KM, BL_KN, EPI_FWD, 7, g.S};
                const double rows = 9.0 * cin;
                const int h = igemm_prof_begin(sig, (int)rows, cout, K, 2.0 * rows * cout * (double)K, (double)xb + (double)db + (double)g.S * g.slab * 4.0,
                                               (hipStream_t)stream);
                hipError_t e = wgrad16_launch(g, cfg, (hipStream_t)stream);
                igemm_prof_end(h, cfg == 0 ? "wgrad16_kernel<32,256,3,128>" : cfg == 1 ? "wgrad16_kernel<64,128,3,128>" : "wgrad16_kernel<64,64,3,192>", (hipStream_t)stream);
                if (e != hipSuccess) return (int)e;
                if (g.S > 1) return rc(k_reduce_rows((const float*)ws, dw, nullptr, 1, g.S, g.slab, 1, 1.f, nullptr, (hipStream_t)stream));
                return FTE_OK;
            }
        }
    }
    if (src16 && ksize == 1 && stride == 1) {
        Wgrad16Params g;
        int cfg = 0;
        if (wgrad16p_plan(n, h, wd, cin, cout, &g, &cfg)) {
            const size_t gneed = g.S > 1 ? (size_t)g.S * g.slab * sizeof(float) : 0;
            const size_t xb = (size_t)n * h * wd * cin * 2, db = (size_t)n * h * wd * cout * 2;
            if ((!gneed || (ws && ws_bytes >= gneed)) && xb < (1ull << 31) && db < (1ull << 31)) {
                g.x = (const unsigned short*)x; g.dz = (const unsigned short*)dz;
                g.out = g.S > 1 ? (float*)ws : dw;
                g.x_bytes = (unsigned)xb; g.dz_bytes = (unsigned)db;
                const int sig[5] = {AL_KM, BL_KN, EPI_FWD, 7, g.S};
                const int hr = igemm_prof_begin(sig, cin, cout, K, 2.0 * cin * cout * (double)K, (double)xb + (double)db + (double)g.S * g.slab * 4.0,
                                                (hipStream_t)stream);
                hipError_t e = wgrad16p_launch(g, cfg, (hipStream_t)stream);
                static const char* const psym[7] = {"wgrad16p_kernel<128,256,2,4>", "wgrad16p_kernel<256,128,4,2>", "wgrad16p_kernel<128,128,2,4>", "wgrad16p_kernel<64,256,1,8>",
                                                   "wgrad16p_kernel<256,64,8,1>", "wgrad16p_kernel<64,128,2,4>", "wgrad16p_kernel<128,64,4,2>"};
                igemm_prof_end(hr, psym[cfg], (hipStream_t)stream);
                if (e != hipSuccess) return (int)e;
                if (g.S > 1) return rc(k_reduce_rows((const float*)ws, dw, nullptr, 1, g.S, g.slab, 1, 1.f, nullptr, (hipStream_t)stream));
                return FTE_OK;
            }
        }
    }
    const size_t need = splits > 1 ? (size_t)splits * ksize * ksize * cin * cout * sizeof(float) : 0;
    if (need && (!ws || ws_bytes < need)) return FTE_EWORKSPACE;
    IgemmParams p;
    zero_params(&p);
    p.M = ksize * ksize * cin; p.N = cout; p.K = K; p.kchunk = kchunk;
    p.A = (const float*)x; p.a_OH = ph.out; p.a_OW = pw.out; p.a_IH = h; p.a_IW = wd; p.a_stride = stride;
    p.a_ld = cin; p.a_KC = cin; p.a_NT = ksize * ksize;
    for (int r = 0; r < ksize; ++r)
        for (int s = 0; s < ksize; ++s) { p.a_dh[r * ksize + s] = r - ph.before; p.a_dw[r * ksize + s] = s - pw.before; }
    p.B = (const float*)dz; p.b_ld = cout;
    p.c_ld = cout;
    p.slab = (long)p.M * p.N;
    p.Y = splits > 1 ? (float*)ws : dw;
    p.split_major = (wgrad_split_major() && splits > 1) ? splits : 0;
    p.src16 = src16 ? 1 : 0;
    if (!set_bytes(&p, (size_t)n * h * wd * cin, (size_t)K * cout, src16 ? 2 : 4)) return FTE_EINVAL;
    hipError_t e = igemm_launch(p, AL_KM, BL_KN, EPI_FWD, tile, splits, (hipStream_t)stream);
    if (e != hipSuccess) return (int)e;
    if (splits > 1) return rc(k_reduce_rows((const float*)ws, dw, nullptr, 1, splits, p.slab, 1, 1.f, nullptr, (hipStream_t)stream));
    return FTE_OK;
}
int fte_conv2d_wgrad(const float* x, const float* dz, float* dw, int n, int h, int wd, int cin, int cout, int ksize, int stride,
                     void* ws, size_t ws_bytes, void* stream) {
    return conv2d_wgrad_impl(x, dz, false, dw, n, h, wd, cin, cout, ksize, stride, ws, ws_bytes, stream);
}
int fte_conv2d_wgrad16(const uint16_t* x16, const uint16_t* dz16, float* dw, int n, int h, int wd, int cin, int cout, int ksize, int stride,
                       void* ws, size_t ws_bytes, void* stream) {
    return conv2d_wgrad_impl(x16, dz16, true, dw, n, h, wd, cin, cout, ksize, stride, ws, ws_bytes, stream);
}
int fte_conv3x3_wgrad(const float* x, const float* dz, float* dw, int n, int h, int wd, int cin, int cout, int stride,
                      void* ws, size_t ws_bytes, void* stream) {
    return fte_conv2d_wgrad(x, dz, dw, n, h, wd, cin, cout, 3, stride, ws, ws_bytes, stream);
}
int fte_conv3x3_wgrad_kept(const float* x, const float* dz, float* dw, int n, int h, int wd, int cin, int cout, int stride,
                           const float* vpack, void* ws, size_t ws_bytes, void* stream) {
    if (vpack && ((uintptr_t)vpack & 15)) return FTE_EINVAL;
    return conv2d_wgrad_impl(x, dz, false, dw, n, h, wd, cin, cout, 3, stride, ws, ws_bytes, stream, vpack);
}

int fte_conv3x3_first_fwd(const float* x, const float* w, const float* bias, const float* alpha, float* z, float* y,
                          int n, int h, int wd, int cin, int cout, int stride, void* stream) {
    if (!x || !w || !y || (cout != 64 && cout != 32) || (cin != 1 && cin != 3)) return FTE_EINVAL;
    const Pads ph = same_pads(h, 3, stride), pw = same_pads(wd, 3, stride);
    return rc(k_conv_first_fwd(x, w, bias, alpha, z, y, nullptr, nullptr, n, h, wd, cin, cout, ph.out, pw.out, stride, ph.before, pw.before, (hipStream_t)stream));
}
int fte_conv3x3_first_fwd_s16(const float* x, const float* w, const float* bias, const float* alpha, uint16_t* z16, uint16_t* y16,
                              int n, int h, int wd, int cin, int cout, int stride, void* stream) {
    if (!x || !w || !y16 || (cout != 64 && cout != 32) || (cin != 1 && cin != 3)) return FTE_EINVAL;
    const Pads ph = same_pads(h, 3, stride), pw = same_pads(wd, 3, stride);
    return rc(k_conv_first_fwd(x, w, bias, alpha, nullptr, nullptr, z16, y16, n, h, wd, cin, cout, ph.out, pw.out, stride, ph.before, pw.before, (hipStream_t)stream));
}

size_t fte_conv3x3_first_wgrad_ws_bytes(int n, int h, int wd, int cin, int cout, int stride) {
    const Pads ph = same_pads(h, 3, stride), pw = same_pads(wd, 3, stride);
    return align_up((size_t)k_conv_first_wgrad_blocks((long)n * ph.out * pw.out) * 9 * cin * cout * sizeof(float)) + SCRATCH_BYTES;
}

static int conv_first_wgrad_impl(const float* x, const float* dz, const uint16_t* dz16, float* dw, int n, int h, int wd, int cin, int cout, int stride,
                                 void* ws, size_t ws_bytes, void* stream) {
    if (!x || (!dz && !dz16) || !dw || (cout != 64 && cout != 32) || (cin != 1 && cin != 3)) return FTE_EINVAL;
    const Pads ph = same_pads(h, 3, stride), pw = same_pads(wd, 3, stride);
    const int blocks = k_conv_first_wgrad_blocks((long)n * ph.out * pw.out);
    const size_t need = align_up((size_t)blocks * 9 * cin * cout * sizeof(float));
    if (!ws || ws_bytes < need + SCRATCH_BYTES) return FTE_EWORKSPACE;
    hipError_t e = k_conv_first_wgrad(x, dz, dz16, (float*)ws, n, h, wd, cin, cout, ph.out, pw.out, stride, ph.before, pw.before, blocks, (hipStream_t)stream);
    if (e != hipSuccess) return (int)e;
    return rc(k_reduce_rows((const float*)ws, dw, nullptr, 1, blocks, 9L * cin * cout, 1, 1.f, (float*)((char*)ws + need), (hipStream_t)stream));
}
int fte_conv3x3_first_wgrad(const float* x, const float* dz, float* dw, int n, int h, int wd, int cin, int cout, int stride,
                            void* ws, size_t ws_bytes, void* stream) {
    return conv_first_wgrad_impl(x, dz, nullptr, dw, n, h, wd, cin, cout, stride, ws, ws_bytes, stream);
}
int fte_conv3x3_first_wgrad_s16(const float* x, const uint16_t* dz16, float* dw, int n, int h, int wd, int cin, int cout, int stride,
                                void* ws, size_t ws_bytes, void* stream) {
    return conv_first_wgrad_impl(x, nullptr, dz16, dw, n, h, wd, cin, cout, stride, ws, ws_bytes, stream);
}

namespace {
size_t dense_slab_bytes(int tile, long rows, long cols, int red) {
    int splits = 1, kchunk = red;
    if (tiles_of(tile, rows, cols) < 256) plan_splits(tiles_of(tile, rows, cols), red, &splits, &kchunk);
    return splits > 1 ? (size_t)splits * rows * cols * sizeof(float) : 0;
// ... 939 lines not shown
```

### tf_face_toolbox_amd/csrc/wino.h

```cpp
#pragma once
#include <hip/hip_runtime.h>
#include <stddef.h>

struct WinoGeom {
    int n, h, w, th, tw;
    long M;
    int MB;
};
WinoGeom wino_geom(int n, int h, int w);

inline size_t wino_pack_floats(long rows, int c) { return (size_t)((rows + 63) / 64) * 64 * (size_t)c * 16; }

hipError_t wino_transform_tiles(const float* x, float* pack, int n, int h, int w, int c, int mode, hipStream_t st, bool small = false);
hipError_t wino_transform_filter(const float* w, float* pack, int cin, int cout, int dgrad, hipStream_t st);

struct WinoMMParams {
    const float* V;
    const float* U;
    int K, N;
    WinoGeom g;
    float* Y; float* Z; const float* R; const float* bias; const float* alpha;
    const float* ADD; float* RAW; const float* Zin; float* DZ; float* PA; float* PB;
    int amod;
};
hipError_t wino_mm(const WinoMMParams& p, int epi, hipStream_t st);

int wino_wgrad_splits(int cin, int cout);
hipError_t wino_wgrad(const float* V, const float* dz, float* slabs, float* dw, const WinoGeom& g, int cin, int cout, hipStream_t st);

void wino_set_algo(int a);
int wino_get_algo();
```

### tf_face_toolbox_amd/csrc/wino.hip

```cpp
#include <hip/hip_runtime.h>
#include <stdint.h>
#include <stdio.h>
#include <stdlib.h>
#include <string.h>

#include <atomic>

#include "igemm.h"
#include "igemm_dev.h"
#include "wino.h"

#ifdef FTE_WINO_STAMP
__device__ unsigned long long* g_wino_stamp = nullptr;
extern "C" int fte_debug_set_wino_stamp(void* buf) {
    return (int)hipMemcpyToSymbol(HIP_SYMBOL(g_wino_stamp), &buf, sizeof(buf));
}
#endif

namespace {

using namespace igemm_dev;

typedef __attribute__((address_space(3))) void lds_void;
__device__ __forceinline__ void dma16(const __amdgpu_buffer_rsrc_t& r, char* lds, unsigned voff, unsigned soff) {
    __builtin_amdgcn_raw_ptr_buffer_load_lds(r, (lds_void*)lds, 16, voff, soff, 0, 0);
}

constexpr unsigned OOB = 0x80000000u;
#ifndef WMM_ABL
#define WMM_ABL 0
#endif
constexpr int SLAB_F = 16 * 64 * 8;
constexpr int SLAB_B = SLAB_F * 4;

template <int MODE, int TPB>
__global__ __launch_bounds__(TPB) void wino_tiles_kernel(const float* __restrict__ x, float* __restrict__ pack, int H, int W, int C,
                                                         int TH, int TW, long M, int MB, unsigned x_bytes) {
    constexpr int P = MODE == 0 ? 4 : 2;
    constexpr int SUB = 512 / TPB;
    const int tid = threadIdx.x;
    const int c4 = tid & 7;
    const int per = (MB + 7) >> 3;
    const int slot = blockIdx.x >> 3;
    const int mb = (blockIdx.x & 7) * per + slot / SUB, KS = C >> 3;
    if (mb >= MB) return;
    const int r = (slot % SUB) * (64 / SUB) + (tid >> 3);
    const long m = (long)mb * 64 + r;
    const int tpi = TH * TW;
    int n = 0, ty = 0, tx = 0;
    const bool mv = m < M;
    if (mv) { n = (int)(m / tpi); const int rem = (int)(m - (long)n * tpi); ty = rem / TW; tx = rem - ty * TW; }
    const int y0 = 2 * ty - (MODE == 0 ? 1 : 0), x0 = 2 * tx - (MODE == 0 ? 1 : 0);
    const __amdgpu_buffer_rsrc_t rs = __builtin_amdgcn_make_buffer_rsrc(const_cast<float*>(x), 0, x_bytes, 0x00020000);
    const unsigned choff = (unsigned)(blockIdx.y * 32 + c4 * 4) * 4u;
    f32x4 d[P][P];
#pragma unroll
    for (int i = 0; i < P; ++i)
#pragma unroll
        for (int j = 0; j < P; ++j) {
            const int yy = y0 + i, xx = x0 + j;
            const bool ok = mv && yy >= 0 && yy < H && xx >= 0 && xx < W;
            d[i][j] = __builtin_bit_cast(f32x4, __builtin_amdgcn_raw_buffer_load_b128(rs, ok ? (unsigned)(((n * H + yy) * W + xx) * C) * 4u + choff : OOB, 0, 0));
        }
    const int ks = blockIdx.y * 4 + (c4 >> 1), sw = (r >> 4) & 1;
    float* o = pack + (((size_t)mb * KS + ks) * 16 * 64 + r) * 8 + (((c4 & 1) ^ sw) << 2);
    if constexpr (MODE == 0) {
#pragma unroll
        for (int i = 0; i < 4; ++i) {
            f32x4 w[4];
#pragma unroll
            for (int j = 0; j < 4; ++j)
                w[j] = i == 0 ? d[0][j] - d[2][j] : i == 1 ? d[1][j] + d[2][j] : i == 2 ? d[2][j] - d[1][j] : d[1][j] - d[3][j];
            *reinterpret_cast<f32x4*>(o + (size_t)(4 * i + 0) * 512) = w[0] - w[2];
            *reinterpret_cast<f32x4*>(o + (size_t)(4 * i + 1) * 512) = w[1] + w[2];
            *reinterpret_cast<f32x4*>(o + (size_t)(4 * i + 2) * 512) = w[2] - w[1];
            *reinterpret_cast<f32x4*>(o + (size_t)(4 * i + 3) * 512) = w[1] - w[3];
        }
    } else {
#pragma unroll
        for (int i = 0; i < 4; ++i) {
            f32x4 u[2];
#pragma unroll
            for (int j = 0; j < 2; ++j)
                u[j] = i == 0 ? d[0][j] : i == 1 ? 0.5f * (d[0][j] + d[1][j]) : i == 2 ? 0.5f * (d[0][j] - d[1][j]) : d[1][j];
            *reinterpret_cast<f32x4*>(o + (size_t)(4 * i + 0) * 512) = u[0];
            *reinterpret_cast<f32x4*>(o + (size_t)(4 * i + 1) * 512) = 0.5f * (u[0] + u[1]);
            *reinterpret_cast<f32x4*>(o + (size_t)(4 * i + 2) * 512) = 0.5f * (u[0] - u[1]);
            *reinterpret_cast<f32x4*>(o + (size_t)(4 * i + 3) * 512) = u[1];
        }
    }
}

__global__ __launch_bounds__(256) void wino_filter_kernel(const float* __restrict__ w, float* __restrict__ pack, int cin, int cout, int dgrad) {
    const int K = dgrad ? cout : cin, NR = dgrad ? cin : cout;
    const int idx = blockIdx.x * 256 + threadIdx.x;
    if (idx >= K * NR) return;
    int k, row;
    if (dgrad) { k = idx % K; row = idx / K; }
    else { row = idx % NR; k = idx / NR; }
    float g[3][3];
#pragma unroll
    for (int a = 0; a < 3; ++a)
#pragma unroll
        for (int b = 0; b < 3; ++b)
            g[a][b] = dgrad ? w[(((2 - a) * 3 + (2 - b)) * (size_t)cin + row) * cout + k] : w[((a * 3 + b) * (size_t)cin + k) * cout + row];
    float p[4][3];
#pragma unroll
    for (int b = 0; b < 3; ++b) {
        p[0][b] = g[0][b];
        p[1][b] = 0.5f * (g[0][b] + g[1][b] + g[2][b]);
        p[2][b] = 0.5f * (g[0][b] - g[1][b] + g[2][b]);
        p[3][b] = g[2][b];
    }
    const int KS = K >> 3, rb = row >> 6, r = row & 63, c8 = k & 7;
    float* o = pack + ((((size_t)rb * KS + (k >> 3)) * 16) * 64 + r) * 8 + (((c8 >> 2) ^ ((r >> 4) & 1)) << 2) + (c8 & 3);
#pragma unroll
    for (int i = 0; i < 4; ++i) {
        o[(size_t)(4 * i + 0) * 512] = p[i][0];
        o[(size_t)(4 * i + 1) * 512] = 0.5f * (p[i][0] + p[i][1] + p[i][2]);
        o[(size_t)(4 * i + 2) * 512] = 0.5f * (p[i][0] - p[i][1] + p[i][2]);
        o[(size_t)(4 * i + 3) * 512] = p[i][2];
    }
}

template <int EPI, int NWN>
__global__ __launch_bounds__(256 * NWN, 1) void wino_mm_kernel(const WinoMMParams p, int NBX, int GRP, int vid0, int nvirt) {
    constexpr int NW = 4 * NWN;
    constexpr int BSTG = NWN * (SLAB_B / 2);
    constexpr int STG = SLAB_B + BSTG;
    extern __shared__ __attribute__((aligned(16))) char wsm[];
    const int tid = threadIdx.x;
    const int lane = tid & 63;
    const int wid = __builtin_amdgcn_readfirstlane(tid >> 6);
    const int q = wid & 1, mi = (wid >> 1) & 1, ni = NWN == 2 ? wid >> 2 : 0;
    const int hb = NWN == 2 ? 0 : (int)(blockIdx.x & 1);
    const int li = lane & 31, lh = lane >> 5;
    const int KS = p.K >> 3, NB = p.N >> 6;
    auto decode = [&](int vid, int& mb, int& nb) -> bool {
        if (GRP > 0) {
            const int xcd = vid & 7, slot = vid >> 3;
            const int grp = xcd % GRP, cls = xcd / GRP, C = 8 / GRP;
            mb = (slot / NBX) * C + cls;
            nb = grp * NBX + slot % NBX;
        } else {
            mb = vid / NB; nb = vid - mb * NB;
        }
        return mb < p.g.MB;
    };
    auto next_valid = [&](int vid, int& mb, int& nb) -> int {
        if constexpr (NWN == 2) {
            for (; vid < nvirt; vid += (int)gridDim.x)
                if (decode(vid, mb, nb)) return vid;
        } else if (vid == vid0) {
            int c = 0;
            for (int v = vid0; v < nvirt; ++v)
                if (decode(v, mb, nb)) {
                    if (c == (int)(blockIdx.x >> 1)) return v;
                    ++c;
                }
        }
        return nvirt;
    };
    const unsigned voff = (unsigned)lane * 16u;
    auto issue = [&](int mb, int nb, int s, int stage) {
        const __amdgpu_buffer_rsrc_t rsA = __builtin_amdgcn_make_buffer_rsrc(const_cast<float*>(p.V + (size_t)mb * KS * SLAB_F), 0, (unsigned)KS * SLAB_B, 0x00020000);
        const __amdgpu_buffer_rsrc_t rsB = __builtin_amdgcn_make_buffer_rsrc(const_cast<float*>(p.U + (size_t)nb * KS * SLAB_F), 0, (unsigned)KS * SLAB_B, 0x00020000);
        char* base = wsm + stage * STG;
#pragma unroll
        for (int i = 0; i < 32 / NW; ++i) {
            const int piece = wid + NW * i;
            dma16(rsA, base + piece * 1024, voff, (unsigned)(s * SLAB_B + piece * 1024));
        }
#pragma unroll
        for (int i = 0; i < 4; ++i) {
            const int piece = wid + NW * i;
            dma16(rsB, base + SLAB_B + piece * 1024, voff, (unsigned)(s * SLAB_B + (NWN == 2 ? piece : 2 * piece + hb) * 1024));
        }
    };
    constexpr int BPL = NWN * 1024;
    const int a_off = ((8 * q) * 64 + 32 * mi + li) * 32 + ((lh ^ ((li >> 4) & 1)) << 4);
    const int b_off = (8 * q) * BPL + (32 * ni + li) * 32 + ((lh ^ ((li >> 4) & 1)) << 4);
    float* xb = reinterpret_cast<float*>(wsm + STG);
    int* rowpix = reinterpret_cast<int*>(wsm + 2 * STG);
    int* rowflag = rowpix + 64;
    float* red = reinterpret_cast<float*>(rowflag + 64);

    int mb = 0, nb = 0;
    int vid = next_valid(NWN == 2 ? vid0 + (int)blockIdx.x : vid0, mb, nb);
    if (vid >= nvirt) return;
    f32x4 xa[4], xb4[4], ya[4], yb[4];
    auto read_frags = [&](int stage, int half, f32x4 (&fa)[4], f32x4 (&fb)[4], int t) {
        const char* As = wsm + stage * STG;
        fa[t] = *reinterpret_cast<const f32x4*>(As + a_off + (4 * half + t) * 2048);
        fb[t] = *reinterpret_cast<const f32x4*>(As + SLAB_B + b_off + (4 * half + t) * BPL);
    };
    auto dma_piece = [&](const __amdgpu_buffer_rsrc_t& rsA, const __amdgpu_buffer_rsrc_t& rsB, int s, int stage, int i) {
        char* base = wsm + stage * STG;
        if constexpr (NWN == 2) {
            const int piece = wid + 8 * (i >> 1);
            if (i & 1) dma16(rsB, base + SLAB_B + piece * 1024, voff, (unsigned)(s * SLAB_B + piece * 1024));
            else dma16(rsA, base + piece * 1024, voff, (unsigned)(s * SLAB_B + piece * 1024));
        } else {
            const int piece = wid + 4 * (i & 7);
            if (i >= 8) dma16(rsB, base + SLAB_B + piece * 1024, voff, (unsigned)(s * SLAB_B + (2 * piece + hb) * 1024));
            else dma16(rsA, base + piece * 1024, voff, (unsigned)(s * SLAB_B + piece * 1024));
        }
    };
    constexpr int NDMA = NWN == 2 ? 8 : 12;
    issue(mb, nb, 0, 0);
    issue(mb, nb, 1, 1);
    asm volatile("s_waitcnt vmcnt(0)\n\ts_barrier" ::: "memory");
#pragma unroll
    for (int t = 0; t < 4; ++t) read_frags(0, 0, xa, xb4, t);
    bool first = true;
    while (vid < nvirt) {
        int mb2 = 0, nb2 = 0;
        const int vid2 = NWN == 2 ? next_valid(vid + (int)gridDim.x, mb2, nb2) : nvirt;
        const bool has_next = vid2 < nvirt;
#ifdef FTE_WINO_STAMP
        unsigned long long st0 = 0, sr0 = 0, st1 = 0;
        if (g_wino_stamp) { st0 = __builtin_amdgcn_s_memtime(); sr0 = __builtin_amdgcn_s_memrealtime(); __builtin_amdgcn_s_waitcnt(0xC07F); }
#endif
        f32x16 acc[8];
#pragma unroll
        for (int t = 0; t < 8; ++t)
#pragma unroll
            for (int r = 0; r < 16; ++r) acc[t][r] = 0.f;
        for (int s = 0; s < KS; ++s) {
            const int st = s & 1;
            __builtin_amdgcn_sched_barrier(0);
            static_for<0, 16>([&](auto ic) {
                constexpr int idx = decltype(ic)::value, j = idx >> 2, t = idx & 3;
                acc[t] = __builtin_amdgcn_mfma_f32_32x32x2f32(xa[t][j], xb4[t][j], acc[t], 0, 0, 0);
                if constexpr (idx < 4 && !(WMM_ABL & 2)) read_frags(st, 1, ya, yb, idx);
                __builtin_amdgcn_sched_barrier(0);
            });
            if constexpr (WMM_ABL & 4) asm volatile("s_waitcnt vmcnt(0) lgkmcnt(0)" ::: "memory");
            else if (s == 0 && !first) asm volatile("s_waitcnt vmcnt(16) lgkmcnt(0)\n\ts_barrier" ::: "memory");
            else asm volatile("s_waitcnt vmcnt(0) lgkmcnt(0)\n\ts_barrier" ::: "memory");
            const bool same = s + 2 < KS;
            const bool dma = same || (has_next && s + 2 == KS);
            const int dmb = same ? mb : mb2, dnb = same ? nb : nb2, ds = same ? s + 2 : 0;
            const __amdgpu_buffer_rsrc_t rsA = __builtin_amdgcn_make_buffer_rsrc(const_cast<float*>(p.V + (size_t)dmb * KS * SLAB_F), 0, dma ? (unsigned)KS * SLAB_B : 0u, 0x00020000);
            const __amdgpu_buffer_rsrc_t rsB = __builtin_amdgcn_make_buffer_rsrc(const_cast<float*>(p.U + (size_t)dnb * KS * SLAB_F), 0, dma ? (unsigned)KS * SLAB_B : 0u, 0x00020000);
            if (s == 0 && tid < 64) {
                const int m = mb * 64 + tid;
                int pix = -1, fl = 0;
                if (m < (int)p.g.M) {
                    const int tpi = p.g.th * p.g.tw;
                    const int n = m / tpi, rem = m - n * tpi;
                    const int ty = rem / p.g.tw, tx = rem - ty * p.g.tw;
                    pix = (n * p.g.h + 2 * ty) * p.g.w + 2 * tx;
                    fl = ((2 * ty + 1 < p.g.h) ? 1 : 0) | ((2 * tx + 1 < p.g.w) ? 2 : 0);
                }
                rowpix[tid] = pix; rowflag[tid] = fl;
            }
            __builtin_amdgcn_sched_barrier(0);
            static_for<0, 16>([&](auto ic) {
                constexpr int idx = decltype(ic)::value, j = idx >> 2, t = idx & 3;
                acc[4 + t] = __builtin_amdgcn_mfma_f32_32x32x2f32(ya[t][j], yb[t][j], acc[4 + t], 0, 0, 0);
                if constexpr (idx < 4 && !(WMM_ABL & 2)) read_frags(st ^ 1, 0, xa, xb4, idx);
                if constexpr (idx >= 4 && idx < 4 + NDMA && !(WMM_ABL & 1)) dma_piece(rsA, rsB, ds, st, idx - 4);
                __builtin_amdgcn_sched_barrier(0);
            });
        }
#ifdef FTE_WINO_STAMP
        if (g_wino_stamp) { st1 = __builtin_amdgcn_s_memtime(); __builtin_amdgcn_s_waitcnt(0xC07F); }
#endif
        asm volatile("s_waitcnt vmcnt(0) lgkmcnt(0)\n\ts_barrier" ::: "memory");

        int lane_e = lane;
        asm volatile("" : "+v"(lane_e));
        const int li_e = lane_e & 31, lh_e = lane_e >> 5;
        float keep[16][2];
#pragma unroll
        for (int r = 0; r < 16; ++r) {
            const float p00 = acc[0][r] + acc[1][r] + acc[2][r], p01 = acc[1][r] - acc[2][r] - acc[3][r];
            const float p10 = acc[4][r] + acc[5][r] + acc[6][r], p11 = acc[5][r] - acc[6][r] - acc[7][r];
            float s0, s1;
            if (q == 0) { keep[r][0] = p00 + p10; keep[r][1] = p01 + p11; s0 = p10; s1 = p11; }
            else { keep[r][0] = -p00 - p10; keep[r][1] = -p01 - p11; s0 = p00; s1 = p01; }
            xb[(wid * 32 + 2 * r) * 64 + lane_e] = s0;
            xb[(wid * 32 + 2 * r + 1) * 64 + lane_e] = s1;
        }
        __builtin_amdgcn_sched_barrier(0);
        const int prw = lane_e >> 3, pc4 = lane_e & 7;
        const int ch0 = nb * 64 + 32 * (NWN == 2 ? ni : hb) + 4 * pc4;
        unsigned off[2][2][2];
#pragma unroll
        for (int h2 = 0; h2 < 2; ++h2)
#pragma unroll
            for (int j = 0; j < 2; ++j) {
                const int rr = 32 * mi + 16 * h2 + prw + 8 * j;
                const int pix = rowpix[rr], fl = rowflag[rr];
                const bool rowok = pix >= 0 && (q == 0 || (fl & 1));
                const unsigned o = (unsigned)((pix + q * p.g.w) * p.N + ch0) * 4u;
                off[0][h2][j] = rowok ? o : OOB;
                off[1][h2][j] = (rowok && (fl & 2)) ? o + (unsigned)p.N * 4u : OOB;
            }
        const unsigned tbytes = (unsigned)((size_t)p.g.n * p.g.h * p.g.w * p.N * 4);
        auto rsrc_of = [&](const float* q_) { return __builtin_amdgcn_make_buffer_rsrc(const_cast<float*>(q_), 0, q_ ? tbytes : 0u, 0x00020000); };
        auto ld4 = [&](const __amdgpu_buffer_rsrc_t& r_, unsigned o) { return __builtin_bit_cast(f32x4, __builtin_amdgcn_raw_buffer_load_b128(r_, o, 0, 0)); };
        auto st4 = [&](const __amdgpu_buffer_rsrc_t& r_, unsigned o, const f32x4& v) { __builtin_amdgcn_raw_buffer_store_b128(__builtin_bit_cast(u32x4, v), r_, o, 0, 0); };
        f32x4 in0[2][2][2], in1[2][2][2];
        f32x4 bias4 = {0.f, 0.f, 0.f, 0.f}, al4 = {1.f, 1.f, 1.f, 1.f};
        bool act = false;
        if constexpr (EPI == EPI_FWD) {
            const __amdgpu_buffer_rsrc_t rsR = rsrc_of(p.R);
#pragma unroll
            for (int b = 0; b < 2; ++b)
#pragma unroll
                for (int h2 = 0; h2 < 2; ++h2)
#pragma unroll
                    for (int j = 0; j < 2; ++j) in0[b][h2][j] = ld4(rsR, off[b][h2][j]);
            if (p.bias) bias4 = *reinterpret_cast<const f32x4*>(p.bias + ch0);
            act = p.alpha != nullptr;
            if (act) al4 = *reinterpret_cast<const f32x4*>(p.alpha + ch0);
        } else {
            const __amdgpu_buffer_rsrc_t rsA = rsrc_of(p.ADD), rsZ = rsrc_of(p.Zin);
#pragma unroll
            for (int b = 0; b < 2; ++b)
#pragma unroll
                for (int h2 = 0; h2 < 2; ++h2)
#pragma unroll
                    for (int j = 0; j < 2; ++j) { in0[b][h2][j] = ld4(rsA, off[b][h2][j]); in1[b][h2][j] = ld4(rsZ, off[b][h2][j]); }
            act = p.Zin != nullptr;
            if (act) al4 = *reinterpret_cast<const f32x4*>(p.alpha + ch0 % p.amod);
        }
        asm volatile("s_waitcnt lgkmcnt(0)\n\ts_barrier" ::: "memory");
#pragma unroll
        for (int r = 0; r < 16; ++r)
#pragma unroll
            for (int b = 0; b < 2; ++b) keep[r][b] += xb[((wid ^ 1) * 32 + 2 * r + b) * 64 + lane_e];
        asm volatile("s_waitcnt lgkmcnt(0)\n\ts_barrier" ::: "memory");
        if (has_next) issue(mb2, nb2, 1, 1);
        float* patch = reinterpret_cast<float*>(wsm + 2 * STG + 2560) + wid * (16 * 36);
        f32x4 sa4 = {0.f, 0.f, 0.f, 0.f}, sb4 = {0.f, 0.f, 0.f, 0.f};
        const __amdgpu_buffer_rsrc_t rsO0 = rsrc_of(EPI == EPI_FWD ? p.Z : p.RAW), rsO1 = rsrc_of(EPI == EPI_FWD ? p.Y : p.DZ);
#pragma unroll
        for (int b = 0; b < 2; ++b)
#pragma unroll
            for (int h2 = 0; h2 < 2; ++h2) {
                __builtin_amdgcn_wave_barrier();
#pragma unroll
                for (int r8 = 0; r8 < 8; ++r8) patch[((r8 & 3) + 8 * (r8 >> 2) + 4 * lh_e) * 36 + li_e] = keep[8 * h2 + r8][b];
                __builtin_amdgcn_fence(__ATOMIC_RELEASE, "wavefront");
                __builtin_amdgcn_wave_barrier();
#pragma unroll
                for (int j = 0; j < 2; ++j) {
                    f32x4 v = *reinterpret_cast<const f32x4*>(patch + (prw + 8 * j) * 36 + 4 * pc4);
                    const unsigned o = off[b][h2][j];
                    if constexpr (EPI == EPI_FWD) {
                        v += bias4;
                        st4(rsO0, o, v);
#pragma unroll
                        for (int e = 0; e < 4; ++e) v[e] = v[e] > 0.f ? v[e] : al4[e] * v[e];
                        v += in0[b][h2][j];
                        st4(rsO1, o, v);
                    } else {
                        v += in0[b][h2][j];
                        st4(rsO0, o, v);
                        const bool in = o != OOB;
#pragma unroll
                        for (int e = 0; e < 4; ++e) {
                            const float z = act ? in1[b][h2][j][e] : 1.f;
                            sa4[e] += in ? v[e] * fminf(z, 0.f) : 0.f;
                            v[e] *= prelu_slope(z, al4[e]);
                            sb4[e] += in ? v[e] : 0.f;
                        }
                        st4(rsO1, o, v);
                    }
                }
            }
        if constexpr (EPI == EPI_DGRAD) {
            if (p.PA) {
#pragma unroll
                for (int e = 0; e < 4; ++e) {
                    float a_ = sa4[e], b_ = sb4[e];
                    a_ += __shfl_xor(a_, 8); b_ += __shfl_xor(b_, 8);
                    a_ += __shfl_xor(a_, 16); b_ += __shfl_xor(b_, 16);
                    a_ += __shfl_xor(a_, 32); b_ += __shfl_xor(b_, 32);
                    if (prw == 0) { red[wid * 32 + 4 * pc4 + e] = a_; red[(NW + wid) * 32 + 4 * pc4 + e] = b_; }
                }
                asm volatile("s_waitcnt lgkmcnt(0)\n\ts_barrier" ::: "memory");
                if (tid < 32 * NWN) {
                    const int n2 = tid >> 5, l2 = tid & 31;
                    float a = 0.f, b = 0.f;
#pragma unroll
                    for (int k = 0; k < 4; ++k) { a += red[(4 * n2 + k) * 32 + l2]; b += red[(NW + 4 * n2 + k) * 32 + l2]; }
                    const size_t o = (size_t)mb * p.N + nb * 64 + (NWN == 2 ? tid : 32 * hb + tid);
                    p.PA[o] = a;
                    if (p.PB) p.PB[o] = b;
                }
            }
        }
#ifdef FTE_WINO_STAMP
        if (g_wino_stamp && tid == 0) {
            const unsigned long long t2 = __builtin_amdgcn_s_memtime(), r2 = __builtin_amdgcn_s_memrealtime();
            unsigned long long* o = g_wino_stamp + 8 * (size_t)vid;
            o[0] = st1 - st0; o[1] = t2 - st1; o[2] = t2 - st0; o[3] = r2 - sr0; o[4] = sr0; o[5] = (unsigned long long)KS; o[6] = blockIdx.x; o[7] = r2;
        }
#endif
        if (has_next) {
#pragma unroll
            for (int t = 0; t < 4; ++t) read_frags(0, 0, xa, xb4, t);
        }
        vid = vid2; mb = mb2; nb = nb2;
        first = false;
    }
}

#ifndef WG_ABL
#define WG_ABL 0
#endif
constexpr int WG_KSTRIDE = 4096 + 32;
constexpr int WG_OP = 8 * WG_KSTRIDE;
__global__ __launch_bounds__(512, 1) void wino_wgrad_kernel(const float* __restrict__ V, const float* __restrict__ dz, float* __restrict__ slabs,
                                                            int cin, int cout, WinoGeom g, int S, unsigned dz_bytes) {
    extern __shared__ __attribute__((aligned(16))) char wsm[];
    const int tid = threadIdx.x;
    const int lane = tid & 63;
    const int wid = __builtin_amdgcn_readfirstlane(tid >> 6);
    const int li = lane & 31, lh = lane >> 5;
    const int KSa = cin >> 3, CB = cin >> 6, NB2 = cout >> 6, P = CB * NB2, MB = g.MB;
    const int L = (blockIdx.x & 7) * (gridDim.x >> 3) + (blockIdx.x >> 3);
    const int split = L / P, pair = L - split * P;
    const int cb = pair / NB2, nb = pair - cb * NB2;
    const int mb0 = (int)((long)split * MB / S), mb1 = (int)((long)(split + 1) * MB / S);
    const int nsteps = (mb1 - mb0) * 8;
    const unsigned voff = (unsigned)((lane >> 4) * 2048 + (lane & 15) * 16);
    const __amdgpu_buffer_rsrc_t rsD = __builtin_amdgcn_make_buffer_rsrc(const_cast<float*>(dz), 0, dz_bytes, 0x00020000);
    const int q8 = 8 / g.tw, r8 = 8 - q8 * g.tw;
    int pn, pty, ptx;
    {
        const int m = mb0 * 64 + wid, tpi = g.th * g.tw;
        pn = m / tpi;
        const int rem = m - pn * tpi;
        pty = rem / g.tw; ptx = rem - pty * g.tw;
    }
    int ps = 0;
    float e[2][2];
    auto load_dz = [&]() {
        const bool mv = ps < nsteps && pn < g.n;
        const int base = ((pn * g.h + 2 * pty) * g.w + 2 * ptx) * cout + nb * 64;
#pragma unroll
        for (int a_ = 0; a_ < 2; ++a_)
#pragma unroll
            for (int b_ = 0; b_ < 2; ++b_) {
                const bool ok = mv && 2 * pty + a_ < g.h && 2 * ptx + b_ < g.w;
                const unsigned so = ok ? (unsigned)(base + (a_ * g.w + b_) * cout) * 4u : 0u;
                e[a_][b_] = __builtin_bit_cast(float, __builtin_amdgcn_raw_buffer_load_b32(rsD, ok ? (unsigned)lane * 4u : OOB, so, 0));
            }
        ++ps;
        ptx += r8; pty += q8;
        if (ptx >= g.tw) { ptx -= g.tw; ++pty; }
        while (pty >= g.th) { pty -= g.th; ++pn; }
    };
    const unsigned up_base = (unsigned)(WG_OP + (lane >> 3) * WG_KSTRIDE + wid * 32 + (lane & 7) * 4);
    auto store_up_row = [&](int stage, int i) {
        const float c0 = i == 0 ? e[0][0] : i == 1 ? e[0][0] + e[1][0] : i == 2 ? e[0][0] - e[1][0] : e[1][0];
        const float c1 = i == 0 ? e[0][1] : i == 1 ? e[0][1] + e[1][1] : i == 2 ? e[0][1] - e[1][1] : e[1][1];
        char* base = wsm + stage * (2 * WG_OP) + up_base + (4 * i) * 256;
        *reinterpret_cast<float*>(base) = c0;
        *reinterpret_cast<float*>(base + 256) = c0 + c1;
        *reinterpret_cast<float*>(base + 512) = c0 - c1;
        *reinterpret_cast<float*>(base + 768) = c1;
    };
    auto store_up = [&](int stage) {
#pragma unroll
        for (int i = 0; i < 4; ++i) store_up_row(stage, i);
    };
    f32x16 acc[2][2][2];
#pragma unroll
    for (int t = 0; t < 2; ++t)
#pragma unroll
        for (int i = 0; i < 2; ++i)
#pragma unroll
            for (int j = 0; j < 2; ++j)
#pragma unroll
                for (int r = 0; r < 16; ++r) acc[t][i][j][r] = 0.f;
    const unsigned lbase = (unsigned)(unsigned long long)(const __attribute__((address_space(3))) char*)wsm;
    const unsigned a_lo = lbase + (unsigned)((li >> 3) * WG_KSTRIDE + (2 * wid) * 256 + lh * 128 + ((li & 7) << 2));
    const unsigned a_hi = lbase + (unsigned)((li >> 3) * WG_KSTRIDE + (2 * wid) * 256 + lh * 128 + (((li & 7) ^ 4) << 2));
    const unsigned b_b = lbase + (unsigned)(WG_OP + (li >> 3) * WG_KSTRIDE + (2 * wid) * 256 + lh * 128 + ((li & 7) << 2));
    float xa[2][2][2], xb[2][2][2], ya[2][2][2], yb[2][2][2];
    auto read_frag = [&](unsigned abase, unsigned bbase, int half, float (&fa)[2][2][2], float (&fb)[2][2][2], int idx) {
        const int t = idx >> 2, i = (idx >> 1) & 1, jj = idx & 1;
        const unsigned so = (unsigned)(i * 4 * WG_KSTRIDE + t * 256 + (2 * half + jj) * 32);
        fa[t][i][jj] = *(const __attribute__((address_space(3))) float*)(unsigned long long)(abase + so);
        fb[t][i][jj] = *(const __attribute__((address_space(3))) float*)(unsigned long long)(bbase + so);
    };
    auto a_base = [&](int s_) { return ((((s_ & 7) >> 1) & 1) ? a_hi : a_lo) + (unsigned)((s_ & 1) * (2 * WG_OP)); };
    auto b_base = [&](int s_) { return b_b + (unsigned)((s_ & 1) * (2 * WG_OP)); };
    auto dma_piece = [&](int s_, int i) {
        const int mb = mb0 + (s_ >> 3), o = s_ & 7;
        const __amdgpu_buffer_rsrc_t rsA = __builtin_amdgcn_make_buffer_rsrc(const_cast<float*>(V + (size_t)(s_ < nsteps ? mb : mb0) * KSa * SLAB_F), 0,
                                                                             s_ < nsteps ? (unsigned)KSa * SLAB_B : 0u, 0x00020000);
        const int piece = wid + 8 * i, ks = piece >> 2, t4 = piece & 3;
        dma16(rsA, wsm + (s_ & 1) * (2 * WG_OP) + ks * WG_KSTRIDE + t4 * 1024, voff, (unsigned)(((8 * cb + ks) * 16 + 4 * t4) * 2048 + o * 256));
    };
    if (nsteps > 0) {
#pragma unroll
        for (int i = 0; i < 4; ++i) { dma_piece(0, i); dma_piece(1, i); }
        load_dz(); store_up(0);
        load_dz(); store_up(1);
        load_dz();
        asm volatile("s_waitcnt vmcnt(4) lgkmcnt(0)\n\ts_barrier" ::: "memory");
        const unsigned pa = a_base(0), pb = b_base(0);
#pragma unroll
        for (int idx = 0; idx < 8; ++idx) read_frag(pa, pb, 0, xa, xb, idx);
    }
    for (int s = 0; s < nsteps; ++s) {
        const unsigned ca = a_base(s), cbb = b_base(s), na = a_base(s + 1), nbb = b_base(s + 1);
        __builtin_amdgcn_sched_barrier(0);
        static_for<0, 16>([&](auto ic) {
            constexpr int idx = decltype(ic)::value, jj = idx >> 3, t = (idx >> 2) & 1, i = (idx >> 1) & 1, k = idx & 1;
            acc[t][i][k] = __builtin_amdgcn_mfma_f32_32x32x2f32(xa[t][i][jj], xb[t][k][jj], acc[t][i][k], 0, 0, 0);
            if constexpr (idx < 8 && !(WG_ABL & 4)) read_frag(ca, cbb, 1, ya, yb, idx);
            __builtin_amdgcn_sched_barrier(0);
        });
        asm volatile("s_waitcnt vmcnt(4) lgkmcnt(0)\n\ts_barrier" ::: "memory");
        __builtin_amdgcn_sched_barrier(0);
        static_for<0, 16>([&](auto ic) {
            constexpr int idx = decltype(ic)::value, jj = idx >> 3, t = (idx >> 2) & 1, i = (idx >> 1) & 1, k = idx & 1;
            acc[t][i][k] = __builtin_amdgcn_mfma_f32_32x32x2f32(ya[t][i][jj], yb[t][k][jj], acc[t][i][k], 0, 0, 0);
            if constexpr (idx < 8 && !(WG_ABL & 4)) read_frag(na, nbb, 0, xa, xb, idx);
            if constexpr (idx >= 8 && idx < 12 && !(WG_ABL & 1)) dma_piece(s + 2, idx - 8);
            if constexpr (idx >= 12 && !(WG_ABL & 2)) {
                store_up_row(s & 1, idx - 12);
                if constexpr (idx == 15) load_dz();
            }
            __builtin_amdgcn_sched_barrier(0);
        });
    }
    asm volatile("s_waitcnt vmcnt(0)" ::: "memory");
    const size_t plane = (size_t)cin * cout;
#pragma unroll
    for (int t = 0; t < 2; ++t)
#pragma unroll
        for (int i = 0; i < 2; ++i)
#pragma unroll
            for (int k = 0; k < 2; ++k) {
                float* o = slabs + ((size_t)split * 16 + 2 * wid + t) * plane + (size_t)(cb * 64 + 32 * i + 4 * lh) * cout + nb * 64 + 32 * k + li;
#pragma unroll
                for (int r = 0; r < 16; ++r) o[(size_t)((r & 3) + 8 * (r >> 2)) * cout] = acc[t][i][k][r];
            }
}

__global__ __launch_bounds__(256) void wino_wgrad_finish_kernel(const float* __restrict__ slabs, float* __restrict__ dw, int S, long plane) {
    const long idx = (long)blockIdx.x * 256 + threadIdx.x;
    if (idx >= plane) return;
    float m[16];
#pragma unroll
    for (int t = 0; t < 16; ++t) m[t] = 0.f;
    for (int s = 0; s < S; ++s)
#pragma unroll
        for (int t = 0; t < 16; ++t) m[t] += slabs[((size_t)s * 16 + t) * plane + idx];
#pragma unroll
    for (int t = 0; t < 16; ++t) {
        const float sc = (((t >> 2) == 1 || (t >> 2) == 2) ? 0.5f : 1.f) * (((t & 3) == 1 || (t & 3) == 2) ? 0.5f : 1.f);
        m[t] *= sc;
    }
    float pr[3][4];
#pragma unroll
    for (int j = 0; j < 4; ++j) {
        pr[0][j] = m[0 + j] + m[4 + j] + m[8 + j];
        pr[1][j] = m[4 + j] - m[8 + j];
        pr[2][j] = m[4 + j] + m[8 + j] - m[12 + j];
    }
#pragma unroll
    for (int a = 0; a < 3; ++a) {
        dw[(size_t)(a * 3 + 0) * plane + idx] = pr[a][0] + pr[a][1] + pr[a][2];
        dw[(size_t)(a * 3 + 1) * plane + idx] = pr[a][1] - pr[a][2];
        dw[(size_t)(a * 3 + 2) * plane + idx] = pr[a][1] + pr[a][2] - pr[a][3];
    }
}

int g_algo = -1;

}

WinoGeom wino_geom(int n, int h, int w) {
    WinoGeom g;
    g.n = n; g.h = h; g.w = w; g.th = (h + 1) / 2; g.tw = (w + 1) / 2;
    g.M = (long)n * g.th * g.tw;
    g.MB = (int)((g.M + 63) / 64);
    return g;
}

hipError_t wino_transform_tiles(const float* x, float* pack, int n, int h, int w, int c, int mode, hipStream_t st, bool small) {
    if (c % 32) return hipErrorInvalidValue;
    const WinoGeom g = wino_geom(n, h, w);
    const size_t xb = (size_t)n * h * w * c * 4;
    if (xb >= ((size_t)1 << 31)) return hipErrorInvalidValue;
    const dim3 grid(8 * ((g.MB + 7) / 8) * (small ? 2 : 1), c / 32);
    if (mode == 0 && small) hipLaunchKernelGGL((wino_tiles_kernel<0, 256>), grid, dim3(256), 0, st, x, pack, h, w, c, g.th, g.tw, g.M, g.MB, (unsigned)xb);
    else if (mode == 0) hipLaunchKernelGGL((wino_tiles_kernel<0, 512>), grid, dim3(512), 0, st, x, pack, h, w, c, g.th, g.tw, g.M, g.MB, (unsigned)xb);
    else hipLaunchKernelGGL((wino_tiles_kernel<1, 512>), grid, dim3(512), 0, st, x, pack, h, w, c, g.th, g.tw, g.M, g.MB, (unsigned)xb);
    return hipGetLastError();
}

hipError_t wino_transform_filter(const float* w, float* pack, int cin, int cout, int dgrad, hipStream_t st) {
    if (cin % 64 || cout % 64) return hipErrorInvalidValue;
    const int total = cin * cout;
    hipLaunchKernelGGL(wino_filter_kernel, dim3((total + 255) / 256), dim3(256), 0, st, w, pack, cin, cout, dgrad);
    return hipGetLastError();
}

namespace {
template <int EPI, int NWN>
hipError_t wino_mm_launch(const WinoMMParams& p, int NBX, int GRP, int vid0, int vid1, int grid, int tiles, hipStream_t st) {
    constexpr int NW = 4 * NWN;
    const size_t lds = 2 * ((size_t)SLAB_B + NWN * (SLAB_B / 2)) + 2560 + (size_t)NW * 16 * 36 * 4;
    static std::atomic<unsigned> attr{0u};
    int dev = 0;
    (void)hipGetDevice(&dev);
    const unsigned bit = 1u << (dev & 31);
    if (!(attr.load(std::memory_order_acquire) & bit)) {
        hipError_t e = hipFuncSetAttribute(reinterpret_cast<const void*>(wino_mm_kernel<EPI, NWN>), hipFuncAttributeMaxDynamicSharedMemorySize, (int)lds);
        if (e != hipSuccess) return e;
        attr.fetch_or(bit, std::memory_order_release);
    }
    const int sig[5] = {AL_MK, BL_NK, EPI, 8, 1};
    const double frac = (double)tiles / ((double)p.g.MB * (p.N / 64));
    const double flops = 2.0 * 16.0 * (double)tiles * 64.0 * 64.0 * p.K;
    const double bytes = frac * ((double)wino_pack_floats(p.g.M, p.K) * 4.0 + 16.0 * p.N * p.K * 4.0 + (double)p.g.n * p.g.h * p.g.w * p.N * 4.0 *
                                 (EPI == EPI_FWD ? (1 + (p.Z ? 1 : 0) + (p.R ? 1 : 0)) : (1 + (p.ADD ? 1 : 0) + (p.RAW ? 1 : 0) + (p.Zin ? 1 : 0))));
    const int h = igemm_prof_begin(sig, (int)((long)tiles * 64 / (p.N / 64)), p.N, 16 * p.K, flops, bytes, st);
    hipLaunchKernelGGL((wino_mm_kernel<EPI, NWN>), dim3(grid), dim3(256 * NWN), lds, st, p, NBX, GRP, vid0, vid1);
    igemm_prof_end(h, EPI == EPI_FWD ? (NWN == 2 ? "wino_mm_kernel<0,2>" : "wino_mm_kernel<0,1>") : (NWN == 2 ? "wino_mm_kernel<1,2>" : "wino_mm_kernel<1,1>"), st);
    return hipGetLastError();
}
}

hipError_t wino_mm(const WinoMMParams& p, int epi, hipStream_t st) {
    if (p.K % 64 || p.N % 64 || p.g.MB <= 0) return hipErrorInvalidValue;
    if ((size_t)p.g.n * p.g.h * p.g.w * p.N >= ((size_t)1 << 31)) return hipErrorInvalidValue;
    const int NB = p.N / 64;
    int NBX = NB < 2 ? NB : 2, GRP = NB / NBX;
    static const int plain = getenv("FTE_WINO_PLAIN_ORDER") ? atoi(getenv("FTE_WINO_PLAIN_ORDER")) : 0;
    int nvirt;
    if (plain || NB % NBX || 8 % GRP) { GRP = 0; nvirt = p.g.MB * NB; }
    else { const int C = 8 / GRP; nvirt = 8 * ((p.g.MB + C - 1) / C) * NBX; }
    static int cus = 0;
    if (!cus) {
        int dev = 0;
        hipDeviceProp_t prop;
        if (hipGetDevice(&dev) != hipSuccess || hipGetDeviceProperties(&prop, dev) != hipSuccess) return hipErrorInvalidDevice;
        cus = prop.multiProcessorCount > 8 ? prop.multiProcessorCount / 8 * 8 : 8;
    }
    const int grid = nvirt < cus ? (nvirt + 7) / 8 * 8 : cus;
    static const int halves = getenv("FTE_WINO_HALF_TILES") ? atoi(getenv("FTE_WINO_HALF_TILES")) : 1;
    auto valid = [&](int vid) {
        if (GRP > 0) { const int xcd = vid & 7, slot = vid >> 3, cls = xcd / GRP, C = 8 / GRP; return (slot / NBX) * C + cls < p.g.MB; }
        return vid / NB < p.g.MB;
    };
    const int rounds = (nvirt + grid - 1) / grid, last = grid * (rounds - 1);
    int L = 0;
    for (int v = last; v < nvirt; ++v) L += valid(v) ? 1 : 0;
    const int total = p.g.MB * NB;
    int tail_base = nvirt;
    if (halves && L > 0 && 2 * L <= cus && (rounds == 1 || halves == 2)) tail_base = last;
    hipError_t e = hipSuccess;
    if (tail_base > 0) {
        e = epi == EPI_FWD ? wino_mm_launch<EPI_FWD, 2>(p, NBX, GRP, 0, tail_base, grid, total - (tail_base < nvirt ? L : 0), st)
                           : wino_mm_launch<EPI_DGRAD, 2>(p, NBX, GRP, 0, tail_base, grid, total - (tail_base < nvirt ? L : 0), st);
        if (e != hipSuccess) return e;
    }
    if (tail_base < nvirt)
        e = epi == EPI_FWD ? wino_mm_launch<EPI_FWD, 1>(p, NBX, GRP, tail_base, nvirt, 2 * L, L, st)
                           : wino_mm_launch<EPI_DGRAD, 1>(p, NBX, GRP, tail_base, nvirt, 2 * L, L, st);
    return e;
}

int wino_wgrad_splits(int cin, int cout) {
    if (cin % 64 || cout % 64) return 0;
    const int P = (cin / 64) * (cout / 64);
    if (P > 256 || 256 % P) return 0;
    return 256 / P;
}

hipError_t wino_wgrad(const float* V, const float* dz, float* slabs, float* dw, const WinoGeom& g, int cin, int cout, hipStream_t st) {
    const int S = wino_wgrad_splits(cin, cout);
    if (!S) return hipErrorInvalidValue;
    const size_t db = (size_t)g.n * g.h * g.w * cout * 4;
    if (db >= ((size_t)1 << 31)) return hipErrorInvalidValue;
    const size_t lds = 4 * (size_t)WG_OP;
    static std::atomic<unsigned> attr{0u};
    int dev = 0;
    (void)hipGetDevice(&dev);
    const unsigned bit = 1u << (dev & 31);
    if (!(attr.load(std::memory_order_acquire) & bit)) {
        hipError_t e = hipFuncSetAttribute(reinterpret_cast<const void*>(wino_wgrad_kernel), hipFuncAttributeMaxDynamicSharedMemorySize, (int)lds);
        if (e != hipSuccess) return e;
        attr.fetch_or(bit, std::memory_order_release);
    }
    const int sig[5] = {AL_KM, BL_KN, EPI_FWD, 8, S};
    const double flops = 2.0 * 16.0 * (double)g.MB * 64.0 * cin * cout;
    const double bytes = (double)wino_pack_floats(g.M, cin) * 4.0 + (double)db + (double)S * 16.0 * cin * cout * 4.0;
    const int h = igemm_prof_begin(sig, 16 * cin, cout, (int)(g.MB * 64), flops, bytes, st);
    hipLaunchKernelGGL(wino_wgrad_kernel, dim3(256), dim3(512), lds, st, V, dz, slabs, cin, cout, g, S, (unsigned)db);
    igemm_prof_end(h, "wino_wgrad_kernel", st);
    hipError_t e = hipGetLastError();
    if (e != hipSuccess) return e;
    const long plane = (long)cin * cout;
    hipLaunchKernelGGL(wino_wgrad_finish_kernel, dim3((unsigned)((plane + 255) / 256)), dim3(256), 0, st, slabs, dw, S, plane);
    return hipGetLastError();
}

void wino_set_algo(int a) { g_algo = a; }
int wino_get_algo() {
    if (g_algo < 0) {
        const char* e = getenv("FTE_CONV_ALGO");
        g_algo = 2;
        if (e) {
            if (!strcmp(e, "direct")) g_algo = 0;
            else if (!strcmp(e, "winograd")) g_algo = 1;
            else if (!strcmp(e, "auto")) g_algo = 2;
        }
    }
    return g_algo;
}
```

### tf_face_toolbox_amd/nets/sphere.py

```python
import math
import os
from collections import OrderedDict

import torch

from .. import _lib, heads
from ..loss import sample_size
from .net_base import NORMALISED_HEADS, Network, adaface_params, adaface_state, margin_params, side_stream

NUM_BLOCKS = (1, 2, 4, 1)
EMBED = 512


def same_pads(in_size, k, stride):
    out = -(-in_size // stride)
    total = max((out - 1) * stride + k - in_size, 0)
    return out, total // 2, total - total // 2


class _Conv(object):
    __slots__ = ('name', 'stage', 'stride', 'has_bias', 'second', 'cin', 'cout', 'hin', 'win', 'hout', 'wout')


class Variable(object):
# ... 14 lines not shown

    def __init__(self, weight_decay=0.0005, data_format='NCHW', name='SphereNet', seed=0):
        super(SphereNet, self).__init__(weight_decay, data_format, name)
        self.num_outputs = [64, 128, 256, 512]
        self.seed = seed
        self.built = False
        self.bf16_copies = os.environ.get('FTE_BF16_COPIES', '1') != '0'
        self.tower_scale = 1.0
        self.global_step = 0
        self.sub_centers = 1
        self._act_n = None

    def _conv_specs(self, h, w, cin):
        specs = []
        for si, nb in enumerate(NUM_BLOCKS):
            stage = '%s/conv%d' % (self.name, si + 1)
            lst = [(stage + '/Conv', 2, True, None)]
            for b in range(nb):
                blk = stage + ('/resBlock' if nb == 1 else '/Repeat/resBlock_%d' % (b + 1))
                lst += [(blk + '/Conv', 1, False, 0), (blk + '/Conv_1', 1, False, 1)]
            for nm, stride, has_bias, second in lst:
                c = _Conv()
                c.name, c.stage, c.stride, c.has_bias, c.second = nm, si, stride, has_bias, second
                c.cin, c.cout, c.hin, c.win = cin, self.num_outputs[si], h, w
                c.hout, c.wout = same_pads(h, 3, stride)[0], same_pads(w, 3, stride)[0]
                specs.append(c)
                h, w, cin = c.hout, c.wout, c.cout
        return specs

    def build(self, height, width, channels, num_classes, device='cuda'):
        _lib.load()
        self.device = torch.device(device)
        self.in_hwc = (height, width, channels)
        self.num_classes = int(num_classes)
        self.cpad = (self.num_classes + 127) // 128 * 128
        self.convs = self._conv_specs(height, width, channels)
        last = self.convs[-1]
        self.feat_hwc = (last.hout, last.wout, last.cout)
        self.fin = last.hout * last.wout * last.cout
        small, big = [], []
        for c in self.convs:
            if c.has_bias:
                small.append((c.name + '/biases', 'bias', (c.cout,), c.cout))
            small.append((c.name + '/alpha', 'alpha', (c.cout,), c.cout))
            big.append((c.name + '/weights', 'conv_w', (3, 3, c.cin, c.cout), 9 * c.cin * c.cout))
        small.append((self.name + '/fully_connected/biases', 'fc_b', (EMBED,), EMBED))
        big.append((self.name + '/fully_connected/weights', 'fc_w', (self.fin, EMBED), self.fin * EMBED))
        K = self.sub_centers
        big.append(('classifier/fc_classifier/weights', 'cls_w', (EMBED, K * self.num_classes), EMBED * K * self.cpad))
        self.variables = OrderedDict()
        off = 0
        for nm, kind, shape, size in small + big:
            self.variables[nm] = Variable(nm, kind, shape, off, size)
            off += (size + 3) // 4 * 4
        self.small_end = self.variables[big[0][0]].offset
        self.cls_start = self.variables['classifier/fc_classifier/weights'].offset
        self.fc_start = self.variables[self.name + '/fully_connected/weights'].offset
        self._stage_first = [min(self.variables[c.name + '/weights'].offset for c in self.convs if c.stage == st_)
                             for st_ in sorted(set(c.stage for c in self.convs))]
        self.arena_size = off
        dev = self.device
        self.params = torch.zeros(off, dtype=torch.float32, device=dev)
        self.grads = torch.zeros(off + 4, dtype=torch.float32, device=dev)
        self.loss_slots = self.grads[off:off + 4]
        self.state = self._make_state()
        self._init_params()
        self.built = True
        return self

    def _make_state(self):
        return OrderedDict()

    def view(self, name, arena=None):
        v = self.variables[name]
        a = self.params if arena is None else arena
        return a[v.offset:v.offset + v.size]

    def _init_params(self):
        g = torch.Generator().manual_seed(self.seed)
        for c in self.convs:
            if c.has_bias:
                lim = (6.0 / (9 * c.cin + 9 * c.cout)) ** 0.5
                w = (torch.rand(3, 3, c.cin, c.cout, generator=g) * 2 - 1) * lim
            else:
                w = torch.randn(3, 3, c.cin, c.cout, generator=g) * 0.01
            self.view(c.name + '/weights').copy_(w.reshape(-1))
            self.view(c.name + '/alpha').fill_(0.25)
        lim = (6.0 / (self.fin + EMBED)) ** 0.5
        w = (torch.rand(self.fin, EMBED, generator=g) * 2 - 1) * lim
        self.view(self.name + '/fully_connected/weights').copy_(w.reshape(-1))
        K = self.sub_centers
        wc = torch.zeros(EMBED, K, self.cpad)
        wc[:, :, :self.num_classes] = (torch.randn(EMBED, K * self.num_classes, generator=g) * 0.001).reshape(EMBED, K, self.num_classes)
        self.view('classifier/fc_classifier/weights').copy_(wc.reshape(-1))

    def _fc_perm(self, t, to_internal):
        if self.data_format == 'NHWC':
            return t
        h, w, c = self.feat_hwc
        if to_internal:
            return t.reshape(c, h, w, EMBED).permute(1, 2, 0, 3).reshape(self.fin, EMBED)
        return t.reshape(h, w, c, EMBED).permute(2, 0, 1, 3).reshape(self.fin, EMBED)

    def get_variable(self, name, arena=None):
        if name in self.state:
            return self.state[name].clone()
        v = self.variables[name]
        t = self.view(name, arena)
        if v.kind == 'cls_w':
            return t.reshape(EMBED, self.sub_centers, self.cpad)[:, :, :self.num_classes].reshape(v.ref_shape).clone()
        if v.kind == 'fc_w':
            return self._fc_perm(t.reshape(self.fin, EMBED), False).contiguous()
        return t.reshape(v.ref_shape).clone()

    def set_variable(self, name, value, arena=None):
        if name in self.state:
            self.state[name].copy_(torch.as_tensor(value, dtype=torch.float32).reshape(self.state[name].shape))
            return
        v = self.variables[name]
        t = torch.as_tensor(value, dtype=torch.float32).to(self.device)
        assert tuple(t.shape) == v.ref_shape, (name, tuple(t.shape), v.ref_shape)
        if v.kind == 'cls_w':
            buf = torch.zeros(EMBED, self.sub_centers, self.cpad, device=self.device)
            buf[:, :, :self.num_classes] = t.reshape(EMBED, self.sub_centers, self.num_classes)
            t = buf
        elif v.kind == 'fc_w':
            t = self._fc_perm(t, True)
        self.view(name, arena).copy_(t.reshape(-1))

    def load_params(self, params):
        for k, val in params.items():
            self.set_variable(k, val)

    def _storage16(self):
        return _lib.bf16_storage()

    def _alloc_acts(self, n):
        s16 = self._storage16()
        key = (s16, _lib.get_mfma_dtype(), _lib.query('fte_get_conv_algo'))
        if self._act_n == n and getattr(self, '_act_key', None) == key:
            return
        self._act_key = key
        dev = self.device
        f32 = dict(dtype=torch.float32, device=dev)
        i16 = dict(dtype=torch.int16, device=dev)
        self._act_s16 = s16
        self.y16 = None
        self.z, self.y = [], []
        last = len(self.convs) - 1
        for l, c in enumerate(self.convs):
            keep32 = not s16 or l == last
            self.z.append(torch.empty(n, c.hout, c.wout, c.cout, **f32) if keep32 else None)
            self.y.append(torch.empty(n, c.hout, c.wout, c.cout, **f32) if keep32 else None)
        if s16:
            self.z16 = [torch.empty(n, c.hout, c.wout, c.cout, **i16) for c in self.convs]
        self.emb = torch.empty(n, EMBED, **f32)
        hw = self._head_width()
        self.s_raw = torch.empty(n, hw, **f32)
        self.G = torch.empty(n, hw, **f32)
        self.logits_buf = torch.empty(n, hw // self.sub_centers, **f32) if self.head == 'asoftmax' or self.head in NORMALISED_HEADS else self.s_raw
        self.loss_rows = torch.empty(n, **f32)
        self.xn = torch.empty(n, **f32)
        self.wn = torch.empty(hw, **f32)
        self.rowcoef = torch.empty(n, **f32)
        self.colcoef = torch.empty(hw, **f32)
        self.demb = torch.empty(n, EMBED, **f32)
        self.bwd = {}
        for si in range(4):
            c = [q for q in self.convs if q.stage == si][0]
            shp = (n, c.hout, c.wout, c.cout)
            if s16:
                one = [torch.empty(shp, **f32)] if si == 3 else []
                self.bwd[si] = dict(dz=one, raw=list(one and [torch.empty(shp, **f32)]), dzi=0, rawi=0,
                                    dz16=[torch.empty(shp, **i16) for _ in range(self._dz_buffers())],
                                    raw16=[torch.empty(shp, **i16), torch.empty(shp, **i16)])
            else:
                self.bwd[si] = dict(dz=[torch.empty(shp, **f32) for _ in range(self._dz_buffers())],
                                    raw=[torch.empty(shp, **f32), torch.empty(shp, **f32)], dzi=0, rawi=0)
        need = 4096
        q = _lib.query
        self.vpack = [None] * len(self.convs)
        if not s16 and os.environ.get('FTE_WINO_KEEP', '1') != '0':
            for l, c in enumerate(self.convs):
                if l > 0 and c.stride == 1 and q('fte_conv3x3_algo', n, c.hin, c.win, c.cin, c.cout, 1, 0) == 1 \
                        and q('fte_conv3x3_algo', n, c.hin, c.win, c.cin, c.cout, 1, 2) == 1:
                    self.vpack[l] = torch.empty(q('fte_wino_pack_bytes', n, c.hin, c.win, c.cin) // 4, **f32)
        for c in self.convs[1:]:
            need = max(need, q('fte_conv3x3_fwd_ws_bytes', n, c.hin, c.win, c.cin, c.cout, c.stride),
                       q('fte_conv3x3_wgrad_ws_bytes', n, c.hin, c.win, c.cin, c.cout, c.stride),
                       q('fte_conv3x3_dgrad_ws_bytes', n, c.hin, c.win, c.cin, c.cout, c.stride))
        c0 = self.convs[0]
        need = max(need, q('fte_conv3x3_first_wgrad_ws_bytes', n, c0.hin, c0.win, c0.cin, c0.cout, c0.stride),
                   q('fte_gemm_ws_bytes', n, EMBED, self.fin), q('fte_gemm_ws_bytes', n, hw, EMBED))
        self.ws = torch.empty((need + 3) // 4 + 1024, **f32)
        self.ws_bytes = self.ws.numel() * 4
        self.side = side_stream(self.device) if os.environ.get('FTE_SIDE_STREAM', '1') != '0' else None
        self.ws_side = torch.empty_like(self.ws) if self.side is not None else self.ws
        self._alloc_head(n)
        self._act_n = n
        self.y16 = None

    def _head_width(self):
        return self.sub_centers * self.cpad

    def _alloc_head(self, n):
        """further head buffers of a subclass, sized with the activations"""

    def _use_copies(self):
        return self.bf16_copies and _lib.get_mfma_dtype() == 'bf16'

    def _alloc_copies(self):
        if self.y16 is not None and self.y16[0].shape[0] == self._act_n:
            return
        i16 = dict(dtype=torch.int16, device=self.device)
        n = self._act_n
        self.y16 = [torch.empty(n, c.hout, c.wout, c.cout, **i16) for c in self.convs]
        for si in range(4):
            b = self.bwd[si]
            if 'dz16' not in b:
                b['dz16'] = [torch.empty(b['dz'][0].shape, **i16) for _ in b['dz']]
        if getattr(self, 'packs', None) is None:
            from ._packs import FilterPacks
            self.packs = FilterPacks([(c.name, self.variables[c.name + '/weights'].offset, 3, c.cin, c.cout) for c in self.convs[1:]], self.device)
            self.w16, self.w16t = self.packs.w16, self.packs.w16t

    def _pack_weights(self, st):
        self.packs.refresh(self.params, st)

    def prelu(self, x, name='prelu'):
        raise RuntimeError('PReLU is fused into the conv epilogue (fte_conv3x3_fwd); it is not a separate op here.')

    def _check_images(self, images):
        if not (isinstance(images, torch.Tensor) and images.is_cuda and images.dtype == torch.float32):
            raise TypeError('images must be a float32 CUDA tensor in NHWC (data.py:275-279 layout)')
        if not images.is_contiguous():
            images = images.contiguous()
        return images

    def _fwd_split(self, n, copies):
        env = os.environ.get('FTE_FWD_HALVES', 'auto')
        if env == '0' or copies or self.side is None or n < 2 or getattr(self, 'one_stream', False):
            return 0
        key = (n, getattr(self, '_act_key', None))
        if getattr(self, '_split_key', None) != key:
            q = _lib.query
            gran = 1
            for l, c in enumerate(self.convs):
                if self.vpack[l] is not None:
                    tpi = ((c.hin + 1) // 2) * ((c.win + 1) // 2)
                    gran = max(gran, 64 // math.gcd(64, tpi))
            a = int(os.environ.get('FTE_FWD_SPLIT', (n // 2) // gran * gran))
            ok, any_w = 0 < a < n, False
            for l, c in enumerate(self.convs):
                if l == 0 or c.stride != 1 or not ok:
                    continue
                algo = [q('fte_conv3x3_algo', m, c.hin, c.win, c.cin, c.cout, 1, 0) for m in (n, a, n - a)]
                any_w = any_w or algo[0] == 1
                if algo[1] != algo[0] or algo[2] != algo[0]:
                    ok = False
                if self.vpack[l] is not None and (a * ((c.hin + 1) // 2) * ((c.win + 1) // 2)) % 64:
                    ok = False
            self._split_key, self._split = key, (a if ok and any_w else 0)
        if not self._split:
            return 0
        return self._split if env == '1' or n >= int(os.environ.get('FTE_FWD_HALVES_MIN', '128')) else 0

    def _fwd_halves(self, n, copies):
        return self._fwd_split(n, copies) > 0

    def backbone(self, inputs, is_training=False, reuse=None):
        x = self._check_images(inputs)
        n, h, w, ch = x.shape
        if not self.built:
            raise RuntimeError('call build() or forward(..., num_classes=) with is_training=True first')
        assert (h, w, ch) == self.in_hwc, ((h, w, ch), self.in_hwc)
        self._alloc_acts(n)
        st = _stream()
        call = _lib.call
        keep = is_training
        self._images = x
        s16 = self._storage16()
        copies = self._use_copies() or s16
        self._copies_live = copies and keep
        self._s16_live = s16 and keep
        self._vpack_live = keep and not copies
        if copies:
            self._alloc_copies()
            self._pack_weights(st)
        def layer(l, c, lo, hi, ws, st):
            m = hi - lo
            wv = self.view(c.name + '/weights')
            bv = self.view(c.name + '/biases') if c.has_bias else None
            av = self.view(c.name + '/alpha')
            zz = self.z[l][lo:hi] if keep and self.z[l] is not None else None
            if s16:
                z16 = self.z16[l][lo:hi] if keep else None
                if l == 0:
                    call('fte_conv3x3_first_fwd_s16', x[lo:hi], wv, bv, av, z16, self.y16[0][lo:hi], m, c.hin, c.win, c.cin, c.cout, c.stride, st)
                else:
                    call('fte_conv2d_fwd_s16', self.y16[l - 1][lo:hi], self.w16t[c.name], bv, av, self.y16[l - 2][lo:hi] if c.second == 1 else None,
                         z16, self.y16[l][lo:hi], zz, self.y[l][lo:hi] if self.y[l] is not None else None, m, c.hin, c.win, c.cin, c.cout, 3, c.stride,
                         ws, self.ws_bytes, st)
            elif l == 0:
                call('fte_conv3x3_first_fwd', x[lo:hi], wv, bv, av, zz, self.y[0][lo:hi], m, c.hin, c.win, c.cin, c.cout, c.stride, st)
                if copies:
                    call('fte_to_bf16', self.y[0][lo:hi], self.y16[0][lo:hi], self.y[0][lo:hi].numel(), st)
            else:
                res = self.y[l - 2][lo:hi] if c.second == 1 else None
                if copies:
                    call('fte_conv2d_fwd16', self.y16[l - 1][lo:hi], self.w16t[c.name], bv, av, res, zz, self.y[l][lo:hi], self.y16[l][lo:hi],
                         m, c.hin, c.win, c.cin, c.cout, 3, c.stride, ws, self.ws_bytes, st)
                elif keep and self.vpack[l] is not None:
                    vp = self.vpack[l]
                    if m != n:
                        per = ((c.hin + 1) // 2) * ((c.win + 1) // 2) * c.cin * 16
                        vp = vp[lo * per:hi * per] if hi < n else vp[lo * per:]
                    call('fte_conv3x3_fwd_keep', self.y[l - 1][lo:hi], wv, bv, av, res, zz, self.y[l][lo:hi],
                         m, c.hin, c.win, c.cin, c.cout, c.stride, vp, ws, self.ws_bytes, st)
                else:
                    call('fte_conv3x3_fwd', self.y[l - 1][lo:hi], wv, bv, av, res, zz, self.y[l][lo:hi],
                         m, c.hin, c.win, c.cin, c.cout, c.stride, ws, self.ws_bytes, st)

        split = self._fwd_split(n, copies)
        if split:
            main, side = torch.cuda.current_stream(), self.side
            side.wait_stream(main)
            for l, c in enumerate(self.convs):
                layer(l, c, 0, split, self.ws, st)
                layer(l, c, split, n, self.ws_side, side.cuda_stream)
            main.wait_stream(side)
        else:
            for l, c in enumerate(self.convs):
                layer(l, c, 0, n, self.ws, st)
        call('fte_gemm_nn', self.y[-1], self.view(self.name + '/fully_connected/weights'),
             self.view(self.name + '/fully_connected/biases'), self.emb, n, EMBED, self.fin, self.ws, self.ws_bytes, st)
        return self.emb

    def _head_cols(self):
        cls = 'classifier/fc_classifier/weights'
        return self.view(cls), self.view(cls, self.grads), self.num_classes, self.cpad

    def _classifier_raw(self, n):
        W, _, _, ld = self._head_cols()
        _lib.call('fte_gemm_nn', self.emb, W, None, self.s_raw, n, self.sub_centers * ld, EMBED, self.ws, self.ws_bytes, _stream())

    def _ensure_built(self, images, num_classes):
        if not self.built:
            n, h, w, ch = images.shape
            self.build(h, w, ch, num_classes, images.device)
        else:
            assert num_classes == self.num_classes, 'num_classes changed after the variables were created'

    def forward(self, images, num_classes=None, is_training=True):
        if is_training:
            assert num_classes is not None, 'num_classes must be given when is_training=True'
            self._ensure_built(images, num_classes)
            self.backbone(images, is_training=True)
            self._classifier_raw(images.shape[0])
            return {'logits': self.s_raw[:, :self.num_classes]}
        return self._eval_features(images)

    def _eval_features(self, images):
        images = self._check_images(images)
        n, h, w, ch = images.shape
        st = _stream()
        out = torch.empty(n, EMBED, dtype=torch.float32, device=images.device)
        f1 = self.backbone(images, is_training=False)
        _lib.call('fte_axpby', 0.5, f1, 0.0, f1, out, n * EMBED, st)
        flipped = torch.empty_like(images)
        _lib.call('fte_flip_width', images, flipped, n, h, w, ch, st)
        f2 = self.backbone(flipped, is_training=False)
        _lib.call('fte_axpby', 1.0, out, 0.5, f2, out, n * EMBED, st)
        return out

    def _grad_scale(self, n):
        return self.tower_scale / n

    def _finish_losses(self, n):
        st = _stream()
        _lib.call('fte_sum', self.loss_rows, n, self.tower_scale / n, self.loss_slots[0:1], self.ws, self.ws_bytes, st)
        nreg = self.arena_size - self.small_end
        _lib.call('fte_sumsq', self.params[self.small_end:], nreg, 0.5 * self.weight_decay * self.tower_scale,
                  self.loss_slots[1:2], self.ws, self.ws_bytes, st)

    def loss_function(self, scope, labels, **logits):
        n = labels.shape[0]
        labels = heads.check_labels(labels)
        self._labels = labels
        _lib.call('fte_softmax_ce_fwd_bwd', self.s_raw, labels, self.loss_rows, self.G, n, self.num_classes, self.cpad,
                  self._grad_scale(n), _stream())
        self._finish_losses(n)
        return [self.loss_slots[0], self.loss_slots[1]], ['cross_entropy', 'reg_loss'], OrderedDict()

    def _head_backward(self, n, st):
        W, dW, _, ld = self._head_cols()
        ld *= self.sub_centers
        norm = self.head != 'softmax'
        heads.classifier_dw(self, self.emb, W, dW, n, EMBED, ld, self.ws, self.ws_bytes, st, norm)
        self._scatter_dw(st)
        heads.classifier_dx(self, self.emb, W, self.demb, n, EMBED, ld, self.ws, self.ws_bytes, st, norm)

    def _scatter_dw(self, st):
        """what a head on a subset of the columns does with its dW before the input side runs; nothing for all columns"""

    def backward_head(self):
        n = self._act_n
        st = _stream()
        call = _lib.call
        g = self.grads
        self._head_backward(n, st)
        fcw = self.name + '/fully_connected/weights'
        call('fte_reduce_rows', self.demb, self.view(self.name + '/fully_connected/biases', g), None, 1, n, EMBED, 1, 1.0, st)
        call('fte_gemm_tn', self.y[-1], self.demb, self.view(fcw, g), n, EMBED, self.fin, self.ws, self.ws_bytes, st)

    def backward(self):
        for stage in self.backward_stages():
            stage()

    def backward_stages(self):
        it = self._body_walk()
        return [self.backward_head] + [lambda it=it: next(it) for _ in range(len(self._stage_first))]

    @staticmethod
    def _dz_buffers():
        return max(2, int(os.environ.get('FTE_DZ_BUFFERS', '3')))

    def _side_stream(self, n):
        if self.side is None or getattr(self, 'one_stream', False):
            return None
        if os.environ.get('FTE_SIDE_STREAM') == '1':
            return self.side
        return self.side if (n <= 256 or _lib.get_mfma_dtype() == 'bf16' or _lib.query('fte_get_conv_algo') != 0) else None

    def backward_body(self):
        for _ in self._body_walk():
            pass

    def _body_walk(self):
        n = self._act_n
        st = _stream()
        call = _lib.call
        g = self.grads
        fcw = self.name + '/fully_connected/weights'
        L = self.convs
        last = len(L) - 1
        b4 = self.bwd[L[last].stage]
        d_out, dz_cur = b4['raw'][0], b4['dz'][0]
        b4['rawi'], b4['dzi'] = 0, 0
        call('fte_gemm_nt', self.demb, self.view(fcw), self.z[last], self.view(L[last].name + '/alpha'), L[last].cout,
             d_out, dz_cur, self.view(L[last].name + '/alpha', g), n, EMBED, self.fin, self.ws, self.ws_bytes, st)
        s16 = getattr(self, '_s16_live', False) and self._storage16()
        copies = s16 or (getattr(self, '_copies_live', False) and self._use_copies())
        dz16_cur = None
        d16_out = None
        if copies:
            dz16_cur = b4['dz16'][0]
            call('fte_to_bf16', dz_cur, dz16_cur, dz_cur.numel(), st)
        if s16:
            d16_out = b4['raw16'][0]
            call('fte_to_bf16', d_out, d16_out, d_out.numel(), st)
        trace = getattr(self, '_trace_dz', None)
        main, side = torch.cuda.current_stream(), self._side_stream(n)
        wst, wws = (side.cuda_stream, self.ws_side) if side is not None else (st, self.ws)
        readers = {}
        last_w = None
        for l in range(last, -1, -1):
            c = L[l]
            if trace is not None:
                trace[c.name] = (dz16_cur if s16 else dz_cur).clone()
            gw = self.view(c.name + '/weights', g)
            if l == 0:
                if last_w is not None:
                    main.wait_event(last_w)
                if s16:
                    call('fte_conv3x3_first_wgrad_s16', self._images, dz16_cur, gw, n, c.hin, c.win, c.cin, c.cout, c.stride,
                         self.ws, self.ws_bytes, st)
                else:
                    call('fte_conv3x3_first_wgrad', self._images, dz_cur, gw, n, c.hin, c.win, c.cin, c.cout, c.stride,
                         self.ws, self.ws_bytes, st)
                break
            if side is not None:
                side.wait_event(main.record_event())
            if copies:
                call('fte_conv2d_wgrad16', self.y16[l - 1], dz16_cur, gw, n, c.hin, c.win, c.cin, c.cout, 3, c.stride,
                     wws, self.ws_bytes, wst)
            elif getattr(self, '_vpack_live', False) and self.vpack[l] is not None:
                call('fte_conv3x3_wgrad_kept', self.y[l - 1], dz_cur, gw, n, c.hin, c.win, c.cin, c.cout, c.stride,
                     self.vpack[l], wws, self.ws_bytes, wst)
            else:
                call('fte_conv3x3_wgrad', self.y[l - 1], dz_cur, gw, n, c.hin, c.win, c.cin, c.cout, c.stride,
                     wws, self.ws_bytes, wst)
            if side is not None:
                last_w = readers[(dz16_cur if s16 else dz_cur).data_ptr()] = side.record_event()
            p = L[l - 1]
            bp = self.bwd[p.stage]
            if s16:
                if p.stage != c.stage:
                    bp['dzi'], bp['rawi'] = 0, 0
                    raw16_t = bp['raw16'][0]
                else:
                    bp['dzi'] = (bp['dzi'] + 1) % len(bp['dz16'])
                    raw16_t = bp['raw16'][bp['rawi'] ^ 1]
                dz16_prev = bp['dz16'][bp['dzi']]
                raw16 = raw16_t if p.second == 1 else None
                ev = readers.pop(dz16_prev.data_ptr(), None)
                if ev is not None:
                    main.wait_event(ev)
                call('fte_conv2d_dgrad_s16', dz16_cur, self.w16[c.name], d16_out if c.second == 0 else None, self.z16[l - 1],
                     self.view(p.name + '/alpha'), raw16, dz16_prev, self.view(p.name + '/alpha', g),
                     self.view(p.name + '/biases', g) if p.has_bias else None,
                     n, c.hin, c.win, c.cin, c.cout, 3, c.stride, self.ws, self.ws_bytes, st)
                if raw16 is not None:
                    d16_out = raw16
                    if p.stage == c.stage:
                        bp['rawi'] ^= 1
                dz16_cur = dz16_prev
                if p.stage != c.stage:
                    if last_w is not None:
                        main.wait_event(last_w)
                        last_w = None
                        readers.clear()
                    yield
                continue
            addin = d_out if c.second == 0 else None
            if p.stage != c.stage:
                bp['dzi'], bp['rawi'] = 0, 0
                dz_prev, raw_t = bp['dz'][0], bp['raw'][0]
            else:
                bp['dzi'] = (bp['dzi'] + 1) % len(bp['dz'])
                dz_prev = bp['dz'][bp['dzi']]
                raw_t = bp['raw'][bp['rawi'] ^ 1]
            raw = raw_t if p.second == 1 else None
            ev = readers.pop(dz_prev.data_ptr(), None)
            if ev is not None:
                main.wait_event(ev)
            if copies:
                dz16_prev = bp['dz16'][bp['dzi']]
                call('fte_conv2d_dgrad16', dz16_cur, self.w16[c.name], addin, self.z[l - 1],
                     self.view(p.name + '/alpha'), raw, dz_prev, dz16_prev, self.view(p.name + '/alpha', g),
                     self.view(p.name + '/biases', g) if p.has_bias else None,
                     n, c.hin, c.win, c.cin, c.cout, 3, c.stride, self.ws, self.ws_bytes, st)
                dz16_cur = dz16_prev
            else:
                call('fte_conv3x3_dgrad', dz_cur, self.view(c.name + '/weights'), addin, self.z[l - 1],
                     self.view(p.name + '/alpha'), raw, dz_prev, self.view(p.name + '/alpha', g),
                     self.view(p.name + '/biases', g) if p.has_bias else None,
                     n, c.hin, c.win, c.cin, c.cout, c.stride, self.ws, self.ws_bytes, st)
            if raw is not None:
                d_out = raw
                if p.stage == c.stage:
                    bp['rawi'] ^= 1
            dz_cur = dz_prev
            if p.stage != c.stage:
                if last_w is not None:
                    main.wait_event(last_w)
                    last_w = None
                    readers.clear()
                yield
        yield

    def param_list(self, is_training, trainable, scope=None):
        bb = [v for k, v in self.variables.items() if k.startswith(self.name + '/')]
        if is_training:
            return [bb, [self.variables['classifier/fc_classifier/weights']]]
        return [bb]

    def pretrained_param(self, scope=None):
        return [v for grp in self.param_list(is_training=False, trainable=False, scope=scope) for v in grp
                if self.name in v.name]

    def arena_groups(self):
        return [(0, self.small_end, False, 0), (self.small_end, self.cls_start, True, 0),
                (self.cls_start, self.arena_size, True, 1)]

    def grad_buckets(self):
        firsts = self._stage_first
        ends = firsts[1:] + [self.fc_start]
        buckets = [(self.fc_start, self.arena_size + 4)]
        for i in range(len(firsts) - 1, 0, -1):
            buckets.append((firsts[i], ends[i]))
        buckets.append((0, ends[0]))
        return buckets


class SphereNetMargin(SphereNet):
    head = 'asoftmax'
    needs_labels = True

    def __init__(self, weight_decay=0.0005, data_format='NCHW', name='SphereNet', seed=0,
                 lambda_base=1000.0, gamma=0.12, power=1.0, lambda_min=5.0):
        super(SphereNetMargin, self).__init__(weight_decay, data_format, name, seed)
        self.lambda_base, self.gamma, self.power, self.lambda_min = lambda_base, gamma, power, lambda_min

    def current_lambda(self):
        return max(self.lambda_min, self.lambda_base * (1.0 + self.gamma * self.global_step) ** (-self.power))

    def forward(self, images, labels=None, num_classes=None, is_training=True):
        if not is_training:
            return self._eval_features(images)
        assert num_classes is not None, 'num_classes must be given when is_training=True'
        assert labels is not None, 'margin nets take labels in forward (data_parallel.py:220)'
        self._ensure_built(images, num_classes)
        n = images.shape[0]
        self._check_sample(n)
        labels = heads.check_labels(labels)
        self._labels = labels
        st = _stream()
        self.backbone(images, is_training=True)
        labels, extra = self._sample_classes(labels, n, st)
        self._classifier_raw(n)
        W, _, c, ld = self._head_cols()
        heads.margin_forward(self, self.emb, W, self.s_raw, labels, self.logits_buf, self._head_spec(), n, EMBED, c, ld,
                             self._grad_scale(n), st)
        return dict({'logits': self.logits_buf[:, :c]}, **extra)

    def _check_sample(self, n):
        """a sampled-class head refuses a batch its sample cannot hold"""

    def _sample_classes(self, labels, n, st):
        return labels, {}

    def _head_spec(self):
        self.lam = self.current_lambda()
        return ('asoftmax', self.lam)

    def _others(self):
        others = OrderedDict()
        others['lambda'] = self.lam
        return others

    def loss_function(self, scope, labels, **logits):
        n = labels.shape[0]
        self._finish_losses(n)
        return [self.loss_slots[0], self.loss_slots[1]], ['cross_entropy', 'reg_loss'], self._others()


class SphereNetAdditiveMargin(SphereNetMargin):

    def __init__(self, weight_decay=0.0005, data_format='NCHW', name='SphereNet', seed=0, head='arcface',
                 scale=None, margin=None, margin_cos=None, sample_rate=None, sample_seed=0, sub_centers=1):
# ... 126 lines not shown
```

Before: 15230 images/sec.

## Fuse PReLU into Winograd input transform and skip materializing intermediate activations

For residual pairs where both convs use kept Winograd packs, the first conv now writes only its pre-activation z. The second conv applies PReLU inside the Winograd tile transform, so the intermediate y tensor is never written or read. A LEAN variant of the wino_mm kernel drops the residual load and the activated-output store, with a shallower vmcnt wait. The wgrad finish kernel is also restructured so 16 thread rows split the slab reduction and combine through shared memory. This cuts activation memory traffic and allocations, at the cost of more template variants and an extra alpha load in the tile transform.

```diff
diff --git a/include/fte.h b/include/fte.h
--- a/include/fte.h
+++ b/include/fte.h
@@ -43,6 +43,10 @@
                          const float* res, float* z, float* y,
                          int n, int h, int wd, int cin, int cout, int stride, float* vpack,
                          void* ws, size_t ws_bytes, void* stream);
+int fte_conv3x3_fwd_keep_act(const float* x, const float* xalpha, const float* w, const float* bias, const float* alpha,
+                             const float* res, float* z, float* y,
+                             int n, int h, int wd, int cin, int cout, int stride, float* vpack,
+                             void* ws, size_t ws_bytes, void* stream);
 
 int fte_conv3x3_dgrad(const float* dz, const float* w, const float* addin,
                       const float* zprev, const float* alpha_prev,
diff --git a/tf_face_toolbox_amd/_lib.py b/tf_face_toolbox_amd/_lib.py
--- a/tf_face_toolbox_amd/_lib.py
+++ b/tf_face_toolbox_amd/_lib.py
@@ -119,6 +119,7 @@
     'fte_conv3x3_algo': (c_int, [c_int] * 7),
     'fte_wino_pack_bytes': (c_size_t, [c_int] * 4),
     'fte_conv3x3_fwd_keep': (c_int, [_P] * 7 + [c_int] * 6 + [_P, _P, c_size_t, _P]),
+    'fte_conv3x3_fwd_keep_act': (c_int, [_P] * 8 + [c_int] * 6 + [_P, _P, c_size_t, _P]),
     'fte_conv3x3_wgrad_kept': (c_int, [_P] * 3 + [c_int] * 6 + [_P, _P, c_size_t, _P]),
     'fte_get_conv_algo': (c_int, []),
     'fte_l2_normalize_rows': (c_int, [_P] * 3 + [c_int] * 2 + [_P]),
diff --git a/tf_face_toolbox_amd/csrc/api.hip b/tf_face_toolbox_amd/csrc/api.hip
--- a/tf_face_toolbox_amd/csrc/api.hip
+++ b/tf_face_toolbox_amd/csrc/api.hip
@@ -372,8 +372,11 @@
 static int conv2d_fwd_impl(const void* x, const void* w, bool src16, const float* bias, const float* alpha, const float* res,
                            float* z, float* y, uint16_t* y16, int n, int h, int wd, int cin, int cout, int ksize, int stride,
                            void* ws, size_t ws_bytes, void* stream, const uint16_t* res16 = nullptr, uint16_t* z16 = nullptr,
-                           float* stat_part = nullptr, int* stat_rows = nullptr, float* vpack = nullptr) {
-    if (!x || !w || (!y && !(src16 && y16)) || n <= 0 || cin % 32 || cout % 64 || (stride != 1 && stride != 2) || (ksize != 1 && ksize != 3))
+                           float* stat_part = nullptr, int* stat_rows = nullptr, float* vpack = nullptr,
+                           const float* xalpha = nullptr, bool z_only_ok = false) {
+    const bool z_only = z_only_ok && !y && z && vpack;
+    if ((xalpha || z_only_ok) && !vpack) return FTE_EINVAL;
+    if (!x || !w || (!y && !(src16 && y16) && !z_only) || n <= 0 || cin % 32 || cout % 64 || (stride != 1 && stride != 2) || (ksize != 1 && ksize != 3))
         return FTE_EINVAL;
     const Pads ph = same_pads(h, ksize, stride), pw = same_pads(wd, ksize, stride);
     IgemmParams p;
@@ -396,16 +399,16 @@
         p.b_ld = cout;
     }
     if (!set_bytes(&p, (size_t)n * h * wd * cin, (size_t)ksize * ksize * cin * cout, src16 ? 2 : 4)) return FTE_EINVAL;
-    if (!src16 && !stat_part && y && wino_wanted(n, h, wd, cin, cout, ksize, stride, 0)) {
+    if (!src16 && !stat_part && (y || z_only) && wino_wanted(n, h, wd, cin, cout, ksize, stride, 0)) {
         WinoWs wl = wino_ws(n, h, wd, cin, cout, 0, 0);
         if (vpack) { wl.u_off = 0; wl.total = align_up((size_t)16 * cin * cout * 4); }
         if (ws && ws_bytes >= wl.total) {
-            if (!aligned16({x, w, bias, alpha, res, z, y, ws, vpack})) return FTE_EINVAL;
+            if (!aligned16({x, w, bias, alpha, res, z, y, ws, vpack, xalpha})) return FTE_EINVAL;
             float* V = vpack ? vpack : (float*)((char*)ws + wl.v_off);
             float* U = (float*)((char*)ws + wl.u_off);
             hipError_t e = wino_transform_filter((const float*)w, U, cin, cout, 0, (hipStream_t)stream);
             if (e != hipSuccess) return (int)e;
-            e = wino_transform_tiles((const float*)x, V, n, h, wd, cin, 0, (hipStream_t)stream, wino_fwd_small_tiles());
+            e = wino_transform_tiles((const float*)x, V, n, h, wd, cin, 0, (hipStream_t)stream, wino_fwd_small_tiles(), xalpha);
             if (e != hipSuccess) return (int)e;
             WinoMMParams q;
             memset(&q, 0, sizeof(q));
@@ -459,6 +462,13 @@
     if (vpack && ((uintptr_t)vpack & 15)) return FTE_EINVAL;
     return conv2d_fwd_impl(x, w, false, bias, alpha, res, z, y, nullptr, n, h, wd, cin, cout, 3, stride, ws, ws_bytes, stream,
                            nullptr, nullptr, nullptr, nullptr, vpack);
+}
+int fte_conv3x3_fwd_keep_act(const float* x, const float* xalpha, const float* w, const float* bias, const float* alpha, const float* res,
+                             float* z, float* y, int n, int h, int wd, int cin, int cout, int stride, float* vpack,
+                             void* ws, size_t ws_bytes, void* stream) {
+    if (!vpack || ((uintptr_t)vpack & 15) || (!y && !z)) return FTE_EINVAL;
+    return conv2d_fwd_impl(x, w, false, bias, alpha, res, z, y, nullptr, n, h, wd, cin, cout, 3, stride, ws, ws_bytes, stream,
+                           nullptr, nullptr, nullptr, nullptr, vpack, xalpha, true);
 }
 int fte_conv3x3_algo(int n, int h, int wd, int cin, int cout, int stride, int op) {
     if (op < 0 || op > 2) return FTE_EINVAL;
@@ -782,7 +792,7 @@
 static int conv2d_wgrad_impl(const void* x, const void* dz, bool src16, float* dw, int n, int h, int wd, int cin, int cout, int ksize, int stride,
                              void* ws, size_t ws_bytes, void* stream, const float* vpack = nullptr) {
     if (src16 && (cin % 8 || cout % 8)) return FTE_EINVAL;
-    if (!x || !dz || !dw || n <= 0 || cin % 4 || cout % 64 || (stride != 1 && stride != 2) || (ksize != 1 && ksize != 3)) return FTE_EINVAL;
+    if ((!x && !vpack) || !dz || !dw || n <= 0 || cin % 4 || cout % 64 || (stride != 1 && stride != 2) || (ksize != 1 && ksize != 3)) return FTE_EINVAL;
     const Pads ph = same_pads(h, ksize, stride), pw = same_pads(wd, ksize, stride);
     {
         const size_t lim = (size_t)1 << 31, es = src16 ? 2 : 4;
diff --git a/tf_face_toolbox_amd/csrc/wino.h b/tf_face_toolbox_amd/csrc/wino.h
--- a/tf_face_toolbox_amd/csrc/wino.h
+++ b/tf_face_toolbox_amd/csrc/wino.h
@@ -11,7 +11,8 @@
 
 inline size_t wino_pack_floats(long rows, int c) { return (size_t)((rows + 63) / 64) * 64 * (size_t)c * 16; }
 
-hipError_t wino_transform_tiles(const float* x, float* pack, int n, int h, int w, int c, int mode, hipStream_t st, bool small = false);
+hipError_t wino_transform_tiles(const float* x, float* pack, int n, int h, int w, int c, int mode, hipStream_t st, bool small = false,
+                                const float* alpha = nullptr);
 hipError_t wino_transform_filter(const float* w, float* pack, int cin, int cout, int dgrad, hipStream_t st);
 
 struct WinoMMParams {
@@ -24,6 +25,7 @@
     int amod;
 };
 hipError_t wino_mm(const WinoMMParams& p, int epi, hipStream_t st);
+bool wino_lean_enabled();
 
 int wino_wgrad_splits(int cin, int cout);
 hipError_t wino_wgrad(const float* V, const float* dz, float* slabs, float* dw, const WinoGeom& g, int cin, int cout, hipStream_t st);
diff --git a/tf_face_toolbox_amd/csrc/wino.hip b/tf_face_toolbox_amd/csrc/wino.hip
--- a/tf_face_toolbox_amd/csrc/wino.hip
+++ b/tf_face_toolbox_amd/csrc/wino.hip
@@ -33,8 +33,8 @@
 constexpr int SLAB_F = 16 * 64 * 8;
 constexpr int SLAB_B = SLAB_F * 4;
 
-template <int MODE, int TPB>
-__global__ __launch_bounds__(TPB) void wino_tiles_kernel(const float* __restrict__ x, float* __restrict__ pack, int H, int W, int C,
+template <int MODE, int TPB, bool ACT>
+__global__ __launch_bounds__(TPB) void wino_tiles_kernel(const float* __restrict__ x, const float* __restrict__ alpha, float* __restrict__ pack, int H, int W, int C,
                                                          int TH, int TW, long M, int MB, unsigned x_bytes) {
     constexpr int P = MODE == 0 ? 4 : 2;
     constexpr int SUB = 512 / TPB;
@@ -62,6 +62,15 @@
             const bool ok = mv && yy >= 0 && yy < H && xx >= 0 && xx < W;
             d[i][j] = __builtin_bit_cast(f32x4, __builtin_amdgcn_raw_buffer_load_b128(rs, ok ? (unsigned)(((n * H + yy) * W + xx) * C) * 4u + choff : OOB, 0, 0));
         }
+    if constexpr (ACT) {
+        const f32x4 al4 = *reinterpret_cast<const f32x4*>(alpha + blockIdx.y * 32 + c4 * 4);
+#pragma unroll
+        for (int i = 0; i < P; ++i)
+#pragma unroll
+            for (int j = 0; j < P; ++j)
+#pragma unroll
+                for (int e = 0; e < 4; ++e) d[i][j][e] = d[i][j][e] > 0.f ? d[i][j][e] : al4[e] * d[i][j][e];
+    }
     const int ks = blockIdx.y * 4 + (c4 >> 1), sw = (r >> 4) & 1;
     float* o = pack + (((size_t)mb * KS + ks) * 16 * 64 + r) * 8 + (((c4 & 1) ^ sw) << 2);
     if constexpr (MODE == 0) {
@@ -123,9 +132,10 @@
     }
 }
 
-template <int EPI, int NWN>
+template <int EPI, int NWN, bool LEAN>
 __global__ __launch_bounds__(256 * NWN, 1) void wino_mm_kernel(const WinoMMParams p, int NBX, int GRP, int vid0, int nvirt) {
     constexpr int NW = 4 * NWN;
+    constexpr int NST = LEAN ? 8 : 16;
     constexpr int BSTG = NWN * (SLAB_B / 2);
     constexpr int STG = SLAB_B + BSTG;
     extern __shared__ __attribute__((aligned(16))) char wsm[];
@@ -236,7 +246,7 @@
                 __builtin_amdgcn_sched_barrier(0);
             });
             if constexpr (WMM_ABL & 4) asm volatile("s_waitcnt vmcnt(0) lgkmcnt(0)" ::: "memory");
-            else if (s == 0 && !first) asm volatile("s_waitcnt vmcnt(16) lgkmcnt(0)\n\ts_barrier" ::: "memory");
+            else if (s == 0 && !first) asm volatile("s_waitcnt vmcnt(%0) lgkmcnt(0)\n\ts_barrier" ::"n"(NST) : "memory");
             else asm volatile("s_waitcnt vmcnt(0) lgkmcnt(0)\n\ts_barrier" ::: "memory");
             const bool same = s + 2 < KS;
             const bool dma = same || (has_next && s + 2 == KS);
@@ -306,13 +316,15 @@
         f32x4 bias4 = {0.f, 0.f, 0.f, 0.f}, al4 = {1.f, 1.f, 1.f, 1.f};
         bool act = false;
         if constexpr (EPI == EPI_FWD) {
-            const __amdgpu_buffer_rsrc_t rsR = rsrc_of(p.R);
-#pragma unroll
-            for (int b = 0; b < 2; ++b)
-#pragma unroll
-                for (int h2 = 0; h2 < 2; ++h2)
-#pragma unroll
-                    for (int j = 0; j < 2; ++j) in0[b][h2][j] = ld4(rsR, off[b][h2][j]);
+            if constexpr (!LEAN) {
+                const __amdgpu_buffer_rsrc_t rsR = rsrc_of(p.R);
+#pragma unroll
+                for (int b = 0; b < 2; ++b)
+#pragma unroll
+                    for (int h2 = 0; h2 < 2; ++h2)
+#pragma unroll
+                        for (int j = 0; j < 2; ++j) in0[b][h2][j] = ld4(rsR, off[b][h2][j]);
+            }
             if (p.bias) bias4 = *reinterpret_cast<const f32x4*>(p.bias + ch0);
             act = p.alpha != nullptr;
             if (act) al4 = *reinterpret_cast<const f32x4*>(p.alpha + ch0);
@@ -323,7 +335,10 @@
 #pragma unroll
                 for (int h2 = 0; h2 < 2; ++h2)
 #pragma unroll
-                    for (int j = 0; j < 2; ++j) { in0[b][h2][j] = ld4(rsA, off[b][h2][j]); in1[b][h2][j] = ld4(rsZ, off[b][h2][j]); }
+                    for (int j = 0; j < 2; ++j) {
+                        if constexpr (!LEAN) in0[b][h2][j] = ld4(rsA, off[b][h2][j]);
+                        in1[b][h2][j] = ld4(rsZ, off[b][h2][j]);
+                    }
             act = p.Zin != nullptr;
             if (act) al4 = *reinterpret_cast<const f32x4*>(p.alpha + ch0 % p.amod);
         }
@@ -353,13 +368,17 @@
                     if constexpr (EPI == EPI_FWD) {
                         v += bias4;
                         st4(rsO0, o, v);
-#pragma unroll
-                        for (int e = 0; e < 4; ++e) v[e] = v[e] > 0.f ? v[e] : al4[e] * v[e];
-                        v += in0[b][h2][j];
-                        st4(rsO1, o, v);
+                        if constexpr (!LEAN) {
+#pragma unroll
+                            for (int e = 0; e < 4; ++e) v[e] = v[e] > 0.f ? v[e] : al4[e] * v[e];
+                            v += in0[b][h2][j];
+                            st4(rsO1, o, v);
+                        }
                     } else {
-                        v += in0[b][h2][j];
-                        st4(rsO0, o, v);
+                        if constexpr (!LEAN) {
+                            v += in0[b][h2][j];
+                            st4(rsO0, o, v);
+                        }
                         const bool in = o != OOB;
 #pragma unroll
                         for (int e = 0; e < 4; ++e) {
@@ -547,19 +566,27 @@
             }
 }
 
-__global__ __launch_bounds__(256) void wino_wgrad_finish_kernel(const float* __restrict__ slabs, float* __restrict__ dw, int S, long plane) {
-    const long idx = (long)blockIdx.x * 256 + threadIdx.x;
-    if (idx >= plane) return;
+constexpr int WF_E = 32;
+__global__ __launch_bounds__(16 * WF_E) void wino_wgrad_finish_kernel(const float* __restrict__ slabs, float* __restrict__ dw, int S, long plane) {
+    __shared__ float sums[16][WF_E + 1];
+    const int t = threadIdx.x / WF_E, e = threadIdx.x % WF_E;
+    const long idx = (long)blockIdx.x * WF_E + e;
+    float acc = 0.f;
+    if (idx < plane) {
+        const float* src = slabs + (size_t)t * plane + idx;
+#pragma unroll 8
+        for (int s = 0; s < S; ++s) acc += src[(size_t)s * 16 * plane];
+    }
+    sums[t][e] = acc;
+    __syncthreads();
+    if (t != 0 || idx >= plane) return;
     float m[16];
 #pragma unroll
-    for (int t = 0; t < 16; ++t) m[t] = 0.f;
-    for (int s = 0; s < S; ++s)
-#pragma unroll
-        for (int t = 0; t < 16; ++t) m[t] += slabs[((size_t)s * 16 + t) * plane + idx];
-#pragma unroll
-    for (int t = 0; t < 16; ++t) {
-        const float sc = (((t >> 2) == 1 || (t >> 2) == 2) ? 0.5f : 1.f) * (((t & 3) == 1 || (t & 3) == 2) ? 0.5f : 1.f);
-        m[t] *= sc;
+    for (int k = 0; k < 16; ++k) m[k] = sums[k][e];
+#pragma unroll
+    for (int k = 0; k < 16; ++k) {
+        const float sc = (((k >> 2) == 1 || (k >> 2) == 2) ? 0.5f : 1.f) * (((k & 3) == 1 || (k & 3) == 2) ? 0.5f : 1.f);
+        m[k] *= sc;
     }
     float pr[3][4];
 #pragma unroll
@@ -588,15 +615,17 @@
     return g;
 }
 
-hipError_t wino_transform_tiles(const float* x, float* pack, int n, int h, int w, int c, int mode, hipStream_t st, bool small) {
-    if (c % 32) return hipErrorInvalidValue;
+hipError_t wino_transform_tiles(const float* x, float* pack, int n, int h, int w, int c, int mode, hipStream_t st, bool small, const float* alpha) {
+    if (c % 32 || (alpha && mode != 0)) return hipErrorInvalidValue;
     const WinoGeom g = wino_geom(n, h, w);
     const size_t xb = (size_t)n * h * w * c * 4;
     if (xb >= ((size_t)1 << 31)) return hipErrorInvalidValue;
     const dim3 grid(8 * ((g.MB + 7) / 8) * (small ? 2 : 1), c / 32);
-    if (mode == 0 && small) hipLaunchKernelGGL((wino_tiles_kernel<0, 256>), grid, dim3(256), 0, st, x, pack, h, w, c, g.th, g.tw, g.M, g.MB, (unsigned)xb);
-    else if (mode == 0) hipLaunchKernelGGL((wino_tiles_kernel<0, 512>), grid, dim3(512), 0, st, x, pack, h, w, c, g.th, g.tw, g.M, g.MB, (unsigned)xb);
-    else hipLaunchKernelGGL((wino_tiles_kernel<1, 512>), grid, dim3(512), 0, st, x, pack, h, w, c, g.th, g.tw, g.M, g.MB, (unsigned)xb);
+    if (mode == 0 && small && alpha) hipLaunchKernelGGL((wino_tiles_kernel<0, 256, true>), grid, dim3(256), 0, st, x, alpha, pack, h, w, c, g.th, g.tw, g.M, g.MB, (unsigned)xb);
+    else if (mode == 0 && alpha) hipLaunchKernelGGL((wino_tiles_kernel<0, 512, true>), grid, dim3(512), 0, st, x, alpha, pack, h, w, c, g.th, g.tw, g.M, g.MB, (unsigned)xb);
+    else if (mode == 0 && small) hipLaunchKernelGGL((wino_tiles_kernel<0, 256, false>), grid, dim3(256), 0, st, x, alpha, pack, h, w, c, g.th, g.tw, g.M, g.MB, (unsigned)xb);
+    else if (mode == 0) hipLaunchKernelGGL((wino_tiles_kernel<0, 512, false>), grid, dim3(512), 0, st, x, alpha, pack, h, w, c, g.th, g.tw, g.M, g.MB, (unsigned)xb);
+    else hipLaunchKernelGGL((wino_tiles_kernel<1, 512, false>), grid, dim3(512), 0, st, x, alpha, pack, h, w, c, g.th, g.tw, g.M, g.MB, (unsigned)xb);
     return hipGetLastError();
 }
 
@@ -608,7 +637,7 @@
 }
 
 namespace {
-template <int EPI, int NWN>
+template <int EPI, int NWN, bool LEAN>
 hipError_t wino_mm_launch(const WinoMMParams& p, int NBX, int GRP, int vid0, int vid1, int grid, int tiles, hipStream_t st) {
     constexpr int NW = 4 * NWN;
     const size_t lds = 2 * ((size_t)SLAB_B + NWN * (SLAB_B / 2)) + 2560 + (size_t)NW * 16 * 36 * 4;
@@ -617,7 +646,7 @@
     (void)hipGetDevice(&dev);
     const unsigned bit = 1u << (dev & 31);
     if (!(attr.load(std::memory_order_acquire) & bit)) {
-        hipError_t e = hipFuncSetAttribute(reinterpret_cast<const void*>(wino_mm_kernel<EPI, NWN>), hipFuncAttributeMaxDynamicSharedMemorySize, (int)lds);
+        hipError_t e = hipFuncSetAttribute(reinterpret_cast<const void*>(wino_mm_kernel<EPI, NWN, LEAN>), hipFuncAttributeMaxDynamicSharedMemorySize, (int)lds);
         if (e != hipSuccess) return e;
         attr.fetch_or(bit, std::memory_order_release);
     }
@@ -627,15 +656,31 @@
     const double bytes = frac * ((double)wino_pack_floats(p.g.M, p.K) * 4.0 + 16.0 * p.N * p.K * 4.0 + (double)p.g.n * p.g.h * p.g.w * p.N * 4.0 *
                                  (EPI == EPI_FWD ? (1 + (p.Z ? 1 : 0) + (p.R ? 1 : 0)) : (1 + (p.ADD ? 1 : 0) + (p.RAW ? 1 : 0) + (p.Zin ? 1 : 0))));
     const int h = igemm_prof_begin(sig, (int)((long)tiles * 64 / (p.N / 64)), p.N, 16 * p.K, flops, bytes, st);
-    hipLaunchKernelGGL((wino_mm_kernel<EPI, NWN>), dim3(grid), dim3(256 * NWN), lds, st, p, NBX, GRP, vid0, vid1);
-    igemm_prof_end(h, EPI == EPI_FWD ? (NWN == 2 ? "wino_mm_kernel<0,2>" : "wino_mm_kernel<0,1>") : (NWN == 2 ? "wino_mm_kernel<1,2>" : "wino_mm_kernel<1,1>"), st);
+    hipLaunchKernelGGL((wino_mm_kernel<EPI, NWN, LEAN>), dim3(grid), dim3(256 * NWN), lds, st, p, NBX, GRP, vid0, vid1);
+    static const char* const names[2][2][2] = {{{"wino_mm_kernel<0,1>", "wino_mm_kernel<0,1,1>"}, {"wino_mm_kernel<0,2>", "wino_mm_kernel<0,2,1>"}},
+                                               {{"wino_mm_kernel<1,1>", "wino_mm_kernel<1,1,1>"}, {"wino_mm_kernel<1,2>", "wino_mm_kernel<1,2,1>"}}};
+    igemm_prof_end(h, names[EPI == EPI_FWD ? 0 : 1][NWN - 1][LEAN ? 1 : 0], st);
     return hipGetLastError();
 }
+template <int NWN>
+hipError_t wino_mm_pick(const WinoMMParams& p, int epi, bool lean, int NBX, int GRP, int vid0, int vid1, int grid, int tiles, hipStream_t st) {
+    if (epi == EPI_FWD) return lean ? wino_mm_launch<EPI_FWD, NWN, true>(p, NBX, GRP, vid0, vid1, grid, tiles, st)
+                                    : wino_mm_launch<EPI_FWD, NWN, false>(p, NBX, GRP, vid0, vid1, grid, tiles, st);
+    return lean ? wino_mm_launch<EPI_DGRAD, NWN, true>(p, NBX, GRP, vid0, vid1, grid, tiles, st)
+                : wino_mm_launch<EPI_DGRAD, NWN, false>(p, NBX, GRP, vid0, vid1, grid, tiles, st);
+}
+}
+
+bool wino_lean_enabled() {
+    const char* e = getenv("FTE_WINO_LEAN");
+    return !e || strcmp(e, "0") != 0;
 }
 
 hipError_t wino_mm(const WinoMMParams& p, int epi, hipStream_t st) {
     if (p.K % 64 || p.N % 64 || p.g.MB <= 0) return hipErrorInvalidValue;
     if ((size_t)p.g.n * p.g.h * p.g.w * p.N >= ((size_t)1 << 31)) return hipErrorInvalidValue;
+    if (epi == EPI_FWD ? (!p.Y && !p.Z) : !p.DZ) return hipErrorInvalidValue;
+    const bool lean = wino_lean_enabled() && (epi == EPI_FWD ? (!p.R && !p.Y) : (!p.ADD && !p.RAW));
     const int NB = p.N / 64;
     int NBX = NB < 2 ? NB : 2, GRP = NB / NBX;
     static const int plain = getenv("FTE_WINO_PLAIN_ORDER") ? atoi(getenv("FTE_WINO_PLAIN_ORDER")) : 0;
@@ -663,13 +708,10 @@
     if (halves && L > 0 && 2 * L <= cus && (rounds == 1 || halves == 2)) tail_base = last;
     hipError_t e = hipSuccess;
     if (tail_base > 0) {
-        e = epi == EPI_FWD ? wino_mm_launch<EPI_FWD, 2>(p, NBX, GRP, 0, tail_base, grid, total - (tail_base < nvirt ? L : 0), st)
-                           : wino_mm_launch<EPI_DGRAD, 2>(p, NBX, GRP, 0, tail_base, grid, total - (tail_base < nvirt ? L : 0), st);
+        e = wino_mm_pick<2>(p, epi, lean, NBX, GRP, 0, tail_base, grid, total - (tail_base < nvirt ? L : 0), st);
         if (e != hipSuccess) return e;
     }
-    if (tail_base < nvirt)
-        e = epi == EPI_FWD ? wino_mm_launch<EPI_FWD, 1>(p, NBX, GRP, tail_base, nvirt, 2 * L, L, st)
-                           : wino_mm_launch<EPI_DGRAD, 1>(p, NBX, GRP, tail_base, nvirt, 2 * L, L, st);
+    if (tail_base < nvirt) e = wino_mm_pick<1>(p, epi, lean, NBX, GRP, tail_base, nvirt, 2 * L, L, st);
     return e;
 }
 
@@ -704,7 +746,7 @@
     hipError_t e = hipGetLastError();
     if (e != hipSuccess) return e;
     const long plane = (long)cin * cout;
-    hipLaunchKernelGGL(wino_wgrad_finish_kernel, dim3((unsigned)((plane + 255) / 256)), dim3(256), 0, st, slabs, dw, S, plane);
+    hipLaunchKernelGGL(wino_wgrad_finish_kernel, dim3((unsigned)((plane + WF_E - 1) / WF_E)), dim3(16 * WF_E), 0, st, slabs, dw, S, plane);
     return hipGetLastError();
 }
 
diff --git a/tf_face_toolbox_amd/nets/sphere.py b/tf_face_toolbox_amd/nets/sphere.py
--- a/tf_face_toolbox_amd/nets/sphere.py
+++ b/tf_face_toolbox_amd/nets/sphere.py
@@ -190,6 +190,7 @@
             keep32 = not s16 or l == last
             self.z.append(torch.empty(n, c.hout, c.wout, c.cout, **f32) if keep32 else None)
             self.y.append(torch.empty(n, c.hout, c.wout, c.cout, **f32) if keep32 else None)
+        self.lean = [False] * len(self.convs)
         if s16:
             self.z16 = [torch.empty(n, c.hout, c.wout, c.cout, **i16) for c in self.convs]
         self.emb = torch.empty(n, EMBED, **f32)
@@ -223,6 +224,10 @@
                 if l > 0 and c.stride == 1 and q('fte_conv3x3_algo', n, c.hin, c.win, c.cin, c.cout, 1, 0) == 1 \
                         and q('fte_conv3x3_algo', n, c.hin, c.win, c.cin, c.cout, 1, 2) == 1:
                     self.vpack[l] = torch.empty(q('fte_wino_pack_bytes', n, c.hin, c.win, c.cin) // 4, **f32)
+            for l, c in enumerate(self.convs):
+                if c.second == 1 and self.vpack[l] is not None and self.vpack[l - 1] is not None:
+                    self.lean[l] = True
+                    self.y[l - 1] = None
         for c in self.convs[1:]:
             need = max(need, q('fte_conv3x3_fwd_ws_bytes', n, c.hin, c.win, c.cin, c.cout, c.stride),
                        q('fte_conv3x3_wgrad_ws_bytes', n, c.hin, c.win, c.cin, c.cout, c.stride),
@@ -237,6 +242,12 @@
         self._alloc_head(n)
         self._act_n = n
         self.y16 = None
+
+    def _y_buf(self, l):
+        if self.y[l] is None and not self._storage16():
+            c = self.convs[l]
+            self.y[l] = torch.empty(self._act_n, c.hout, c.wout, c.cout, dtype=torch.float32, device=self.device)
+        return self.y[l]
 
     def _head_width(self):
         return self.sub_centers * self.cpad
@@ -322,9 +333,22 @@
         self._copies_live = copies and keep
         self._s16_live = s16 and keep
         self._vpack_live = keep and not copies
+        lean_live = self._vpack_live and os.environ.get('FTE_WINO_LEAN', '1') != '0'
+        self._lean_live = lean_live
+        nl = len(self.convs)
+        if not lean_live:
+            for l in range(nl):
+                self._y_buf(l)
         if copies:
             self._alloc_copies()
             self._pack_weights(st)
+        def part_pack(l, c, lo, hi, m):
+            vp = self.vpack[l]
+            if m != n:
+                per = ((c.hin + 1) // 2) * ((c.win + 1) // 2) * c.cin * 16
+                vp = vp[lo * per:hi * per] if hi < n else vp[lo * per:]
+            return vp
+
         def layer(l, c, lo, hi, ws, st):
             m = hi - lo
             wv = self.view(c.name + '/weights')
@@ -339,6 +363,13 @@
                     call('fte_conv2d_fwd_s16', self.y16[l - 1][lo:hi], self.w16t[c.name], bv, av, self.y16[l - 2][lo:hi] if c.second == 1 else None,
                          z16, self.y16[l][lo:hi], zz, self.y[l][lo:hi] if self.y[l] is not None else None, m, c.hin, c.win, c.cin, c.cout, 3, c.stride,
                          ws, self.ws_bytes, st)
+            elif lean_live and self.lean[l]:
+                p = self.convs[l - 1]
+                call('fte_conv3x3_fwd_keep_act', self.z[l - 1][lo:hi], self.view(p.name + '/alpha'), wv, bv, av, self.y[l - 2][lo:hi], zz,
+                     self.y[l][lo:hi], m, c.hin, c.win, c.cin, c.cout, c.stride, part_pack(l, c, lo, hi, m), ws, self.ws_bytes, st)
+            elif lean_live and l + 1 < nl and self.lean[l + 1]:
+                call('fte_conv3x3_fwd_keep_act', self.y[l - 1][lo:hi], None, wv, bv, av, None, zz, None,
+                     m, c.hin, c.win, c.cin, c.cout, c.stride, part_pack(l, c, lo, hi, m), ws, self.ws_bytes, st)
             elif l == 0:
                 call('fte_conv3x3_first_fwd', x[lo:hi], wv, bv, av, zz, self.y[0][lo:hi], m, c.hin, c.win, c.cin, c.cout, c.stride, st)
                 if copies:
@@ -346,17 +377,13 @@
             else:
                 res = self.y[l - 2][lo:hi] if c.second == 1 else None
                 if copies:
-                    call('fte_conv2d_fwd16', self.y16[l - 1][lo:hi], self.w16t[c.name], bv, av, res, zz, self.y[l][lo:hi], self.y16[l][lo:hi],
+                    call('fte_conv2d_fwd16', self.y16[l - 1][lo:hi], self.w16t[c.name], bv, av, res, zz, self._y_buf(l)[lo:hi], self.y16[l][lo:hi],
                          m, c.hin, c.win, c.cin, c.cout, 3, c.stride, ws, self.ws_bytes, st)
                 elif keep and self.vpack[l] is not None:
-                    vp = self.vpack[l]
-                    if m != n:
-                        per = ((c.hin + 1) // 2) * ((c.win + 1) // 2) * c.cin * 16
-                        vp = vp[lo * per:hi * per] if hi < n else vp[lo * per:]
-                    call('fte_conv3x3_fwd_keep', self.y[l - 1][lo:hi], wv, bv, av, res, zz, self.y[l][lo:hi],
-                         m, c.hin, c.win, c.cin, c.cout, c.stride, vp, ws, self.ws_bytes, st)
+                    call('fte_conv3x3_fwd_keep', self._y_buf(l - 1)[lo:hi], wv, bv, av, res, zz, self._y_buf(l)[lo:hi],
+                         m, c.hin, c.win, c.cin, c.cout, c.stride, part_pack(l, c, lo, hi, m), ws, self.ws_bytes, st)
                 else:
-                    call('fte_conv3x3_fwd', self.y[l - 1][lo:hi], wv, bv, av, res, zz, self.y[l][lo:hi],
+                    call('fte_conv3x3_fwd', self._y_buf(l - 1)[lo:hi], wv, bv, av, res, zz, self._y_buf(l)[lo:hi],
                          m, c.hin, c.win, c.cin, c.cout, c.stride, ws, self.ws_bytes, st)
 
         split = self._fwd_split(n, copies)
@@ -523,7 +550,7 @@
                 call('fte_conv2d_wgrad16', self.y16[l - 1], dz16_cur, gw, n, c.hin, c.win, c.cin, c.cout, 3, c.stride,
                      wws, self.ws_bytes, wst)
             elif getattr(self, '_vpack_live', False) and self.vpack[l] is not None:
-                call('fte_conv3x3_wgrad_kept', self.y[l - 1], dz_cur, gw, n, c.hin, c.win, c.cin, c.cout, c.stride,
+                call('fte_conv3x3_wgrad_kept', None if getattr(self, '_lean_live', False) and self.lean[l] else self.y[l - 1], dz_cur, gw, n, c.hin, c.win, c.cin, c.cout, c.stride,
                      self.vpack[l], wws, self.ws_bytes, wst)
             else:
                 call('fte_conv3x3_wgrad', self.y[l - 1], dz_cur, gw, n, c.hin, c.win, c.cin, c.cout, c.stride,
```

Result: faster. 15400 images/sec, median of 6 (+1.1%).
